# jirsat/wavenets

Hardware: AMD Instinct MI355X
Metric: audio samples/sec (training step, 16 kHz mu-law) (higher is better)
Workload: dtype f32 (fp16 hi|lo split operands, fp32 accumulate)

## Files before the change

wavenets_amd/csrc/wn_bwd_pair.hip:

```cpp
#include "wn_split16.h"

using namespace wn_split16;

namespace {

constexpr int BP_NK1 = 16;
constexpr int BP_NKR = 4;
constexpr int BP_NKF = 8;
constexpr int BP_NKM = BP_NK1 + BP_NKF;
constexpr int BP_W1 = BP_NK1 * 2 * 2048, BP_W2 = (BP_NKR + BP_NKF) * 2 * 2048;
constexpr int BP_PITCH = 36;
constexpr int BP_STAGE = 32 * BP_PITCH * 4;
constexpr int BP_LDS = BP_W1 + BP_W2 + 8 * BP_STAGE;
constexpr int BP_PF = 4;

__device__ __forceinline__ void bp_store32(const f32x16& v, float* stage, float* dst, int64_t ld, int rows_valid, int lane) {
  const int tl = lane & 31, h = lane >> 5;
#pragma unroll
  for (int rq = 0; rq < 4; ++rq) {
    f32x4 o;
    o.x = v[4 * rq + 0]; o.y = v[4 * rq + 1]; o.z = v[4 * rq + 2]; o.w = v[4 * rq + 3];
    *reinterpret_cast<f32x4*>(stage + tl * BP_PITCH + 8 * rq + 4 * h) = o;
  }
  asm volatile("s_waitcnt lgkmcnt(0)" ::: "memory");
#pragma unroll
  for (int i = 0; i < 4; ++i) {
    const int row = i * 8 + (lane >> 3);
    const int col = (lane & 7) * 4;
    const f32x4 o = *reinterpret_cast<const f32x4*>(stage + row * BP_PITCH + col);
    if (row < rows_valid) *reinterpret_cast<f32x4*>(dst + (int64_t)row * ld + col) = o;
  }
  asm volatile("s_waitcnt lgkmcnt(0)" ::: "memory");
}

}

__global__ __launch_bounds__(512, 2) void wn_bwd_pair_kernel(WnBwdPairArgs a) {
  __shared__ __attribute__((aligned(16))) unsigned char smem[BP_LDS];
  const int tid = threadIdx.x;
  const int lane = tid & 63, wave = tid >> 6;
  const int tl = lane & 31, h = lane >> 5;
  float* stage = reinterpret_cast<float*>(smem + BP_W1 + BP_W2 + wave * BP_STAGE);
  {
    wn_images_to_lds<512, BP_W1 / 16, BP_W2 / 16>(a.wx16, smem, BP_W1 / 16, a.wu16, smem + BP_W1, BP_W2 / 16, tid);
  }
  __syncthreads();
  const h8* w1 = reinterpret_cast<const h8*>(smem) + lane;
  const h8* w2 = reinterpret_cast<const h8*>(smem + BP_W1) + lane;

  float sc1, inv1;
  pow2_scale(a.am_gu_in ? *a.am_gu_in : 0.f, sc1, inv1);
  const float gfmax = a.am_gf ? *a.am_gf : 0.f;

  const int tiles_per_b = (a.T + 31) >> 5;
  const int64_t ntiles = (int64_t)a.B * tiles_per_b;
  struct TileCtx {
    int b, t, rows_valid;
    int64_t row0;
  };
  auto make_ctx = [&](int64_t tile, TileCtx& c) {
    c.b = (int)(tile / tiles_per_b);
    const int t0 = (int)(tile % tiles_per_b) * 32;
    c.t = t0 + tl;
    c.rows_valid = min(32, a.T - t0);
    c.row0 = (int64_t)c.b * a.T + t0;
  };
  auto load_x = [&](const TileCtx& c, int m, f32x4& q0, f32x4& q1, bool& okout) {
    const int seg = m >> 3;
    const int kk = m & 7;
    const int ts = c.t + (seg == 0 ? a.dil : 0);
    const bool ok = c.t < a.T && ts < a.T;
    const float* base = seg == 2 ? a.gf : a.gu_in;
    const float* src = base + ((int64_t)c.b * a.T + (ok ? ts : 0)) * 128 + 4 * h + 16 * kk;
    q0 = ldg4(src);
    q1 = ldg4(src + 8);
    okout = ok;
  };

  float wmax_x = 0.f, wmax_u = 0.f;
  const WnTileWalk walk = wn_tile_walk(ntiles, 8, wave);
  const int64_t tstride = walk.stride, tend = walk.end;
  int64_t tile = walk.first;
  TileCtx cur, nxt;
  f32x4 xr[BP_PF][2];
  bool okr[BP_PF];
  if (tile < tend) {
    make_ctx(tile, cur);
#pragma unroll
    for (int k = 0; k < BP_PF; ++k) load_x(cur, k, xr[k][0], xr[k][1], okr[k]);
  }
  for (; tile < tend; tile += tstride) {
    const bool has_next = tile + tstride < tend;
    if (has_next) make_ctx(tile + tstride, nxt);
    const bool tin = cur.t < a.T;
    const int64_t row = cur.row0 + (tin ? tl : 0);

    f32x4 addc[2][4];
#pragma unroll
    for (int j = 0; j < 2; ++j)
#pragma unroll
      for (int rq = 0; rq < 4; ++rq) addc[j][rq] = ldg4(a.gx_res + row * 64 + 32 * j + 8 * rq + 4 * h);

    f32x16 acc[2];
#pragma unroll
    for (int j = 0; j < 2; ++j)
#pragma unroll
      for (int r = 0; r < 16; ++r) acc[j][r] = 0.f;
    for (int m0 = 0; m0 < BP_NK1; m0 += BP_PF) {
      wn_static_for<BP_PF>([&](auto kc) {
        constexpr int k = decltype(kc)::value;
        h8 bh, bl;
        split8s(xr[k][0], xr[k][1], okr[k] ? sc1 : 0.f, bh, bl);
        __builtin_amdgcn_sched_barrier(0);
        load_x(cur, m0 + k + BP_PF, xr[k][0], xr[k][1], okr[k]);
#pragma unroll
        for (int j = 0; j < 2; ++j) {
          const h8 ah = w1[(((m0 + k) * 2 + j) * 2 + 0) * 64];
          const h8 al = w1[(((m0 + k) * 2 + j) * 2 + 1) * 64];
          mfma3(ah, al, bh, bl, acc[j]);
        }
        __builtin_amdgcn_sched_barrier(0);
      });
    }
    f32x16 gx[2];
    float tmax = 0.f;
#pragma unroll
    for (int j = 0; j < 2; ++j)
#pragma unroll
      for (int rq = 0; rq < 4; ++rq) {
        const float cv[4] = {addc[j][rq].x, addc[j][rq].y, addc[j][rq].z, addc[j][rq].w};
#pragma unroll
        for (int e = 0; e < 4; ++e) {
          const float v = tin ? acc[j][4 * rq + e] * inv1 + cv[e] : 0.f;
          gx[j][4 * rq + e] = v;
          tmax = fmaxf(tmax, fabsf(v));
        }
      }
    f32x4 sg[2][4], zz[2][4];
#pragma unroll
    for (int j = 0; j < 2; ++j)
#pragma unroll
      for (int rq = 0; rq < 4; ++rq) {
        sg[j][rq] = ldg4(a.ag + row * 64 + 32 * j + 8 * rq + 4 * h);
        zz[j][rq] = ldg4(a.z + row * a.ldz + 32 * j + 8 * rq + 4 * h);
      }
    if (cur.rows_valid > 0) {
      bp_store32(gx[0], stage, a.gx_out + cur.row0 * 64, 64, cur.rows_valid, lane);
      bp_store32(gx[1], stage, a.gx_out + cur.row0 * 64 + 32, 64, cur.rows_valid, lane);
    }
    wmax_x = fmaxf(wmax_x, tmax);
#pragma unroll
    for (int o = 32; o > 0; o >>= 1) tmax = fmaxf(tmax, __shfl_xor(tmax, o));
    float sc2, inv2;
    pow2_scale(fmaxf(tmax, gfmax), sc2, inv2);

#pragma unroll
    for (int j = 0; j < 2; ++j)
#pragma unroll
      for (int r = 0; r < 16; ++r) acc[j][r] = 0.f;
    wn_static_for<BP_NKR>([&](auto sc) {
      constexpr int ks = decltype(sc)::value;
      constexpr int jz = ks / 2, r0 = 8 * (ks % 2);
      f32x4 q0, q1;
      q0.x = gx[jz][r0 + 0]; q0.y = gx[jz][r0 + 1]; q0.z = gx[jz][r0 + 2]; q0.w = gx[jz][r0 + 3];
      q1.x = gx[jz][r0 + 4]; q1.y = gx[jz][r0 + 5]; q1.z = gx[jz][r0 + 6]; q1.w = gx[jz][r0 + 7];
      h8 bh, bl;
      split8s(q0, q1, sc2, bh, bl);
#pragma unroll
      for (int j = 0; j < 2; ++j) {
        const h8 ah = w2[((ks * 2 + j) * 2 + 0) * 64];
        const h8 al = w2[((ks * 2 + j) * 2 + 1) * 64];
        mfma3(ah, al, bh, bl, acc[j]);
      }
    });
    for (int m0 = BP_NK1; m0 < BP_NKM; m0 += BP_PF) {
      wn_static_for<BP_PF>([&](auto kc) {
        constexpr int k = decltype(kc)::value;
        h8 bh, bl;
        split8s(xr[k][0], xr[k][1], okr[k] ? sc2 : 0.f, bh, bl);
        __builtin_amdgcn_sched_barrier(0);
        const int mn = m0 + k + BP_PF;
        if (mn < BP_NKM) load_x(cur, mn, xr[k][0], xr[k][1], okr[k]);
        else if (has_next) load_x(nxt, mn - BP_NKM, xr[k][0], xr[k][1], okr[k]);
        const int ks2 = BP_NKR + (m0 + k - BP_NK1);
#pragma unroll
        for (int j = 0; j < 2; ++j) {
          const h8 ah = w2[((ks2 * 2 + j) * 2 + 0) * 64];
          const h8 al = w2[((ks2 * 2 + j) * 2 + 1) * 64];
          mfma3(ah, al, bh, bl, acc[j]);
        }
        __builtin_amdgcn_sched_barrier(0);
      });
    }
#pragma unroll
    for (int part = 0; part < 2; ++part)
#pragma unroll
      for (int j = 0; j < 2; ++j) {
        f32x16 o;
#pragma unroll
        for (int rq = 0; rq < 4; ++rq) {
          const float gv[4] = {sg[j][rq].x, sg[j][rq].y, sg[j][rq].z, sg[j][rq].w};
          const float zv[4] = {zz[j][rq].x, zz[j][rq].y, zz[j][rq].z, zz[j][rq].w};
#pragma unroll
          for (int e = 0; e < 4; ++e) {
            const float dz = acc[j][4 * rq + e] * inv2;
            const float v = tin ? (part == 0 ? wn_gate_bwd_f(dz, gv[e], zv[e]) : wn_gate_bwd_g(dz, gv[e], zv[e])) : 0.f;
            o[4 * rq + e] = v;
            wmax_u = fmaxf(wmax_u, fabsf(v));
          }
        }
        if (cur.rows_valid > 0) bp_store32(o, stage, a.gu_out + cur.row0 * 128 + 64 * part + 32 * j, 128, cur.rows_valid, lane);
      }
    if (has_next) cur = nxt;
  }
#pragma unroll
  for (int o = 32; o > 0; o >>= 1) {
    wmax_x = fmaxf(wmax_x, __shfl_xor(wmax_x, o));
    wmax_u = fmaxf(wmax_u, __shfl_xor(wmax_u, o));
  }
  if (lane == 0) {
    if (a.am_gx) wn_absmax_publish(a.am_gx, wmax_x);
    if (a.am_gu) wn_absmax_publish(a.am_gu, wmax_u);
  }
}

int wn_bwd_pair_supported(int R, int D, int KS, int F0) { return (R == 64 && D == 64 && KS == 2 && F0 == 128) ? 1 : 0; }

int wn_launch_bwd_pair(const WnBwdPairArgs& a, hipStream_t s) {
  const int64_t tiles = (int64_t)a.B * ((a.T + 31) / 32);
  if (tiles <= 0) return WN_OK;
  int64_t gx = (tiles + 7) / 8;
  if (gx > 256) gx = 256;
  hipLaunchKernelGGL(wn_bwd_pair_kernel, dim3((unsigned)gx), dim3(512), 0, s, a);
  WN_HIP_CHECK(hipGetLastError());
  return WN_OK;
}
```

wavenets_amd/csrc/wn_common.h:

```cpp
#pragma once
#include <hip/hip_runtime.h>
#include <stdint.h>

#include "../../include/wn_hip.h"

typedef float f32x16 __attribute__((ext_vector_type(16)));
typedef float f32x4 __attribute__((ext_vector_type(4)));

enum WnEpilogue : int {
  WN_EPI_PLAIN = 0,
  WN_EPI_DACT = 1,
  WN_EPI_GATE_BWD = 2,
  WN_EPI_GATE_FWD = 3,
};

__device__ __forceinline__ f32x16 wn_mfma(float a, float b, f32x16 c) {
  return __builtin_amdgcn_mfma_f32_32x32x2f32(a, b, c, 0, 0, 0);
}

__device__ __forceinline__ int wn_drow(int r, int h) { return (r & 3) + 8 * (r >> 2) + 4 * h; }

__device__ __forceinline__ float wn_sigmoid(float x) { return 1.0f / (1.0f + expf(-x)); }

__device__ __forceinline__ float wn_sigmoid_fast(float x) {
  return __builtin_amdgcn_rcpf(1.0f + __builtin_amdgcn_exp2f(-1.4426950408889634f * x));
}
__device__ __forceinline__ float wn_tanh_fast(float x) {
  return __builtin_fmaf(-2.0f, __builtin_amdgcn_rcpf(1.0f + __builtin_amdgcn_exp2f(2.8853900817779268f * x)), 1.0f);
}

__device__ __forceinline__ float wn_act(float x, int act) {
  switch (act) {
    case WN_ACT_RELU: return x > 0.f ? x : 0.f;
    case WN_ACT_LEAKY_RELU: return x >= 0.f ? x : 0.2f * x;
    case WN_ACT_TANH: return tanhf(x);
    case WN_ACT_SIGMOID: return wn_sigmoid(x);
    case WN_ACT_ELU: return x > 0.f ? x : expm1f(x);
    default: return x;
  }
}

__device__ __forceinline__ float wn_dact_from_y(float y, int act) {
  switch (act) {
    case WN_ACT_RELU: return y > 0.f ? 1.f : 0.f;
    case WN_ACT_LEAKY_RELU: return y >= 0.f ? 1.f : 0.2f;
    case WN_ACT_TANH: return 1.f - y * y;
    case WN_ACT_SIGMOID: return y * (1.f - y);
    case WN_ACT_ELU: return y > 0.f ? 1.f : y + 1.f;
    default: return 1.f;
  }
}

__host__ __device__ __forceinline__ size_t wn_frag_floats(int I, int KK) {
  return (size_t)((KK + 7) / 8) * ((I + 31) / 32) * 256;
}

#ifdef __cplusplus
#include <type_traits>
template <int N, class F>
__device__ __forceinline__ void wn_static_for(F&& f) {
  if constexpr (N > 0) {
    wn_static_for<N - 1>(f);
    f(std::integral_constant<int, N - 1>{});
  }
}
#endif

#define WN_HIP_CHECK(expr)                                   \
  do {                                                       \
    hipError_t _e = (expr);                                  \
    if (_e != hipSuccess) {                                  \
      wn_set_error("%s:%d: %s -> %s", __FILE__, __LINE__, #expr, hipGetErrorString(_e)); \
      return WN_E_HIP;                                       \
    }                                                        \
  } while (0)

__device__ __forceinline__ void wn_gate_bwd(float dz, float g, float z, float& duf, float& dug) {
  const float a = g > 1e-30f ? z / g : 0.f;
  duf = dz * g * (1.f - a * a);
  dug = dz * z * (1.f - g);
}

__device__ __forceinline__ float wn_gate_bwd_f(float dz, float g, float z) {
  const float a = g > 1e-30f ? z / g : 0.f;
  return dz * g * (1.f - a * a);
}
__device__ __forceinline__ float wn_gate_bwd_g(float dz, float g, float z) { return dz * z * (1.f - g); }

__device__ __forceinline__ void wn_absmax_publish(float* slot, float v) {
  if (v > 0.f && v < 3.0e38f && v > *reinterpret_cast<volatile float*>(slot))
    atomicMax(reinterpret_cast<int*>(slot), __float_as_int(v));
}

__device__ __forceinline__ void wn_absmax_publish_any(float* slot, float v) {
  if (v > 0.f && v > *reinterpret_cast<volatile float*>(slot))
    atomicMax(reinterpret_cast<int*>(slot), __float_as_int(v));
}

__device__ __forceinline__ float wn_absmax_acc(float wmax, float a, float b, float c, float d) {
  const unsigned m0 = max(__float_as_uint(a) & 0x7fffffffu, __float_as_uint(b) & 0x7fffffffu);
  const unsigned m1 = max(__float_as_uint(c) & 0x7fffffffu, __float_as_uint(d) & 0x7fffffffu);
  return __uint_as_float(max(__float_as_uint(wmax), max(m0, m1)));
}
__device__ __forceinline__ float wn_wave_absmax_bits(float wmax) {
  unsigned m = __float_as_uint(wmax);
#pragma unroll
  for (int o = 32; o > 0; o >>= 1) m = max(m, (unsigned)__shfl_xor((int)m, o));
  const float v = __uint_as_float(m);
  return v < 3.0e38f ? v : 3.0e38f;
}

template <int THREADS, int MAX1, int MAX2 = 0>
__device__ __forceinline__ void wn_images_to_lds(const void* src1, void* dst1, int n16_1, const void* src2, void* dst2, int n16_2,
                                                 int tid) {
  constexpr int K1 = (MAX1 + THREADS - 1) / THREADS, K2 = (MAX2 + THREADS - 1) / THREADS;
  const f32x4* s1 = reinterpret_cast<const f32x4*>(src1);
  const f32x4* s2 = reinterpret_cast<const f32x4*>(src2);
  f32x4 v1[K1 > 0 ? K1 : 1], v2[K2 > 0 ? K2 : 1];
#pragma unroll
  for (int k = 0; k < K1; ++k) { const int i = tid + k * THREADS; if (i < n16_1) v1[k] = s1[i]; }
#pragma unroll
  for (int k = 0; k < K2; ++k) { const int i = tid + k * THREADS; if (i < n16_2) v2[k] = s2[i]; }
  __builtin_amdgcn_sched_barrier(0);
  f32x4* d1 = reinterpret_cast<f32x4*>(dst1);
  f32x4* d2 = reinterpret_cast<f32x4*>(dst2);
#pragma unroll
  for (int k = 0; k < K1; ++k) { const int i = tid + k * THREADS; if (i < n16_1) d1[i] = v1[k]; }
#pragma unroll
  for (int k = 0; k < K2; ++k) { const int i = tid + k * THREADS; if (i < n16_2) d2[i] = v2[k]; }
}

#define WN_KERAS_EPS 1e-7f

#define WN_RANGE_LIMIT 30000.0f

__device__ __forceinline__ void wn_guard_publish_over(float* slot, float wmax) {
  const unsigned m = __float_as_uint(wmax);
  if (m >= __float_as_uint(WN_RANGE_LIMIT)) {
    const float v = __uint_as_float(m);
    atomicMax(reinterpret_cast<int*>(slot), __float_as_int(v < 3.0e38f ? v : 3.0e38f));
  }
}

static inline int wn_blocks(int64_t n, int per = 256, int cap = 4096) {
  int64_t b = (n + per - 1) / per;
  if (b > cap) b = cap;
  if (b < 1) b = 1;
  return (int)b;
}

void wn_set_error(const char* fmt, ...);
int wn_debug_get(int key);

struct WnTileWalk { int64_t first, end, stride; };
__device__ __forceinline__ WnTileWalk wn_tile_walk(int64_t ntiles, int waves, int wave) {
  WnTileWalk w;
  if ((gridDim.x & 7u) == 0u) {
    const int64_t n8 = (ntiles + 7) >> 3;
    const int64_t x = blockIdx.x & 7u;
    w.first = x * n8 + (int64_t)(blockIdx.x >> 3) * waves + wave;
    w.end = (x + 1) * n8 < ntiles ? (x + 1) * n8 : ntiles;
    w.stride = (int64_t)(gridDim.x >> 3) * waves;
  } else {
    w.first = (int64_t)blockIdx.x * waves + wave;
    w.end = ntiles;
    w.stride = (int64_t)gridDim.x * waves;
  }
  return w;
}
```

wavenets_amd/csrc/wn_elem.hip:

```cpp
#include <algorithm>

#include "wn_kernels.h"
#include "wn_sample.h"

__global__ void wn_add_kernel(const float* a, const float* b, float* out, int64_t n) {
  for (int64_t i = (int64_t)blockIdx.x * blockDim.x + threadIdx.x; i < n;
       i += (int64_t)gridDim.x * blockDim.x)
    out[i] = a[i] + b[i];
}
int wn_launch_add(const float* a, const float* b, float* out, int64_t n, hipStream_t s) {
  if (n <= 0) return WN_OK;
  hipLaunchKernelGGL(wn_add_kernel, dim3(wn_blocks(n)), dim3(256), 0, s, a, b, out, n);
  WN_HIP_CHECK(hipGetLastError());
  return WN_OK;
}

__global__ void wn_fill_kernel(float* p, float v, int64_t n) {
  for (int64_t i = (int64_t)blockIdx.x * blockDim.x + threadIdx.x; i < n;
       i += (int64_t)gridDim.x * blockDim.x)
    p[i] = v;
}
int wn_launch_fill(float* p, float v, int64_t n, hipStream_t s) {
  if (n <= 0) return WN_OK;
  hipLaunchKernelGGL(wn_fill_kernel, dim3(wn_blocks(n)), dim3(256), 0, s, p, v, n);
// ... 307 lines not shown
__global__ void wn_dact_mul_kernel(const float* g, const float* y, float* out, int64_t n, int act) {
  for (int64_t i = (int64_t)blockIdx.x * blockDim.x + threadIdx.x; i < n;
       i += (int64_t)gridDim.x * blockDim.x)
    out[i] = g[i] * wn_dact_from_y(y[i], act);
}
int wn_launch_dact_mul(const float* g, const float* y, float* out, int64_t n, int act, hipStream_t s) {
  if (n <= 0) return WN_OK;
  hipLaunchKernelGGL(wn_dact_mul_kernel, dim3(wn_blocks(n)), dim3(256), 0, s, g, y, out, n, act);
  WN_HIP_CHECK(hipGetLastError());
  return WN_OK;
}

__device__ __forceinline__ uint32_t wn_hash32(uint32_t x) {
  x ^= x >> 16; x *= 0x7feb352dU; x ^= x >> 15; x *= 0x846ca68bU; x ^= x >> 16;
  return x;
}
__device__ __forceinline__ bool wn_drop_keep(int64_t idx, uint32_t key, float rate) {
  const uint32_t lo = (uint32_t)idx, hi = (uint32_t)((uint64_t)idx >> 32);
  const uint32_t hsh = wn_hash32(lo ^ wn_hash32(hi + key));
  return (float)(hsh >> 8) * (1.0f / 16777216.0f) >= rate;
}
__global__ void wn_dropout_kernel(const float* x, const float* g_res, float* out, int64_t n, float rate, float scale,
                                  uint32_t key, float* absmax_out) {
  float m = 0.f;
  for (int64_t i = (int64_t)blockIdx.x * blockDim.x + threadIdx.x; i < n; i += (int64_t)gridDim.x * blockDim.x) {
    float v = wn_drop_keep(i, key, rate) ? x[i] * scale : 0.f;
    if (g_res) v += g_res[i];
    out[i] = v;
    m = fmaxf(m, fabsf(v));
  }
  if (absmax_out) {
    m = wn_wave_max(m);
    if ((threadIdx.x & 63) == 0) wn_absmax_publish(absmax_out, m);
  }
}
uint32_t wn_dropout_key(uint64_t seed, int block, uint64_t step) {
  uint32_t k = (uint32_t)seed * 0x9E3779B9U + (uint32_t)(seed >> 32);
  k ^= (uint32_t)block * 0x85EBCA6BU + 0x1234567U;
  k ^= (uint32_t)step * 0xC2B2AE35U + (uint32_t)(step >> 32) * 0x27D4EB2FU;
  return k;
}
int wn_launch_dropout(const float* x, const float* g_res, float* out, int64_t n, float rate, uint32_t key,
                      float* absmax_out, hipStream_t s) {
  if (n <= 0) return WN_OK;
  hipLaunchKernelGGL(wn_dropout_kernel, dim3(wn_blocks(n)), dim3(256), 0, s, x, g_res, out, n, rate, 1.0f / (1.0f - rate),
                     key, absmax_out);
  WN_HIP_CHECK(hipGetLastError());
  return WN_OK;
}

__global__ void wn_cond_scatter_kernel(const float* tmp, const float* params, int64_t b_off0, int64_t b_stride, int B,
                                       int N, int D2, float* cb) {
  const int64_t total = (int64_t)N * B * D2;
  for (int64_t i = (int64_t)blockIdx.x * blockDim.x + threadIdx.x; i < total; i += (int64_t)gridDim.x * blockDim.x) {
    const int n = (int)(i % D2);
    const int u = (int)((i / D2) % B);
    const int b = (int)(i / ((int64_t)D2 * B));
    cb[i] = tmp[((int64_t)u * N + b) * D2 + n] + params[b_off0 + (int64_t)b * b_stride + n];
  }
}
__global__ void wn_cond_gather_kernel(const float* slab, int64_t P, int spb, int64_t bd_off0, int64_t bd_stride, int B,
                                      int N, int D2, float* dcb) {
  const int64_t total = (int64_t)B * N * D2;
  for (int64_t i = (int64_t)blockIdx.x * blockDim.x + threadIdx.x; i < total; i += (int64_t)gridDim.x * blockDim.x) {
    const int n = (int)(i % D2);
    const int b = (int)((i / D2) % N);
    const int u = (int)(i / ((int64_t)D2 * N));
    float acc = 0.f;
    for (int sp = 0; sp < spb; ++sp) acc += slab[(int64_t)(u * spb + sp) * P + bd_off0 + (int64_t)b * bd_stride + n];
    dcb[i] = acc;
  }
}
__global__ void wn_cond_wgrad_kernel(const float* m, const float* dcb, int B, int Cc, int N, int D2, float* grads,
                                     int64_t w_off0, int64_t w_stride, int64_t b_off0, int64_t b_stride) {
  const int64_t total = (int64_t)N * (Cc + 1) * D2;
  for (int64_t i = (int64_t)blockIdx.x * blockDim.x + threadIdx.x; i < total; i += (int64_t)gridDim.x * blockDim.x) {
    const int n = (int)(i % D2);
    const int c = (int)((i / D2) % (Cc + 1));
    const int b = (int)(i / ((int64_t)D2 * (Cc + 1)));
    float acc = 0.f;
    for (int u = 0; u < B; ++u) {
      const float g = dcb[((int64_t)u * N + b) * D2 + n];
      acc += c < Cc ? m[(int64_t)u * Cc + c] * g : g;
    }
    if (c < Cc) grads[w_off0 + (int64_t)b * w_stride + (int64_t)c * D2 + n] = acc;
    else grads[b_off0 + (int64_t)b * b_stride + n] = acc;
  }
}
int wn_launch_cond_scatter(const float* tmp, const float* params, int64_t b_off0, int64_t b_stride, int B, int N, int D2,
                           float* cb, hipStream_t s) {
  const int64_t total = (int64_t)N * B * D2;
  hipLaunchKernelGGL(wn_cond_scatter_kernel, dim3((unsigned)std::min<int64_t>((total + 255) / 256, 1024)), dim3(256), 0, s, tmp,
                     params, b_off0, b_stride, B, N, D2, cb);
  WN_HIP_CHECK(hipGetLastError());
  return WN_OK;
}
int wn_launch_cond_gather(const float* slab, int64_t P, int spb, int64_t bd_off0, int64_t bd_stride, int B, int N, int D2,
                          float* dcb, hipStream_t s) {
  const int64_t total = (int64_t)B * N * D2;
  hipLaunchKernelGGL(wn_cond_gather_kernel, dim3((unsigned)std::min<int64_t>((total + 255) / 256, 1024)), dim3(256), 0, s, slab, P,
                     spb, bd_off0, bd_stride, B, N, D2, dcb);
  WN_HIP_CHECK(hipGetLastError());
  return WN_OK;
}
int wn_launch_cond_wgrad(const float* m, const float* dcb, int B, int Cc, int N, int D2, float* grads, int64_t w_off0,
                         int64_t w_stride, int64_t b_off0, int64_t b_stride, hipStream_t s) {
  const int64_t total = (int64_t)N * (Cc + 1) * D2;
  hipLaunchKernelGGL(wn_cond_wgrad_kernel, dim3((unsigned)std::min<int64_t>((total + 255) / 256, 1024)), dim3(256), 0, s, m, dcb, B,
                     Cc, N, D2, grads, w_off0, w_stride, b_off0, b_stride);
  WN_HIP_CHECK(hipGetLastError());
  return WN_OK;
}

__global__ __launch_bounds__(256) void wn_inconv_fwd_kernel(const float* x, const float* w, const float* bias, int B, int T,
                                                            int R, int KS, float* y, float* absmax_out) {
  const int q = R / 4;
  const int64_t total = (int64_t)B * T * q;
  float wmax = 0.f;
  for (int64_t i = (int64_t)blockIdx.x * blockDim.x + threadIdx.x; i < total; i += (int64_t)gridDim.x * blockDim.x) {
    const int c = (int)(i % q) * 4;
    const int64_t row = i / q;
    const int t = (int)(row % T);
    float a0 = 0.f, a1 = 0.f, a2 = 0.f, a3 = 0.f;
    for (int tap = 0; tap < KS; ++tap) {
      const int ts = t - (KS - 1 - tap);
      const float xv = ts >= 0 ? x[row - (KS - 1 - tap)] : 0.f;
      const f32x4 wv = *reinterpret_cast<const f32x4*>(w + (int64_t)tap * R + c);
      a0 = fmaf(wv.x, xv, a0); a1 = fmaf(wv.y, xv, a1); a2 = fmaf(wv.z, xv, a2); a3 = fmaf(wv.w, xv, a3);
    }
    const f32x4 bv = *reinterpret_cast<const f32x4*>(bias + c);
    const f32x4 o = f32x4{a0 + bv.x, a1 + bv.y, a2 + bv.z, a3 + bv.w};
    *reinterpret_cast<f32x4*>(y + row * R + c) = o;
    wmax = fmaxf(wmax, fmaxf(fmaxf(fabsf(o.x), fabsf(o.y)), fmaxf(fabsf(o.z), fabsf(o.w))));
  }
  if (absmax_out) {
    __shared__ float wm[4];
    if (!(wmax < 3.0e38f)) wmax = 3.0e38f;
    wmax = wn_wave_max(wmax);
    if ((threadIdx.x & 63) == 0) wm[threadIdx.x >> 6] = wmax;
    __syncthreads();
    if (threadIdx.x == 0) wn_absmax_publish_any(absmax_out, fmaxf(fmaxf(wm[0], wm[1]), fmaxf(wm[2], wm[3])));
  }
}
int wn_launch_inconv_fwd(const float* x, const float* w, const float* bias, int B, int T, int R, int KS, float* y,
                         float* absmax_out, hipStream_t s) {
  const int64_t total = (int64_t)B * T * (R / 4);
  if (total <= 0) return WN_OK;
  hipLaunchKernelGGL(wn_inconv_fwd_kernel, dim3((unsigned)std::min<int64_t>((total + 255) / 256, 1024)), dim3(256), 0, s, x, w, bias,
                     B, T, R, KS, y, absmax_out);
  WN_HIP_CHECK(hipGetLastError());
  return WN_OK;
}

__global__ __launch_bounds__(256) void wn_sgemm_small32_kernel(const float* A, int64_t sai, int64_t sak, const float* B, int64_t sbk,
                                                               int64_t sbj, float* C, int ldc, int M, int N, int K,
                                                               int64_t za, int64_t zb, int64_t zc, const float* bias, int act,
                                                               int zk) {
  constexpr int KC = 128;
  __shared__ float As[KC][32 + 1], Bs[KC][32 + 1];
  A += (int64_t)blockIdx.z * za; B += (int64_t)blockIdx.z * zb; C += (int64_t)blockIdx.z * zc;
  if (zk > 0) K = max(0, min(K - (int)blockIdx.z * zk, zk));
  const int i0 = blockIdx.y * 32, j0 = blockIdx.x * 32;
  const int tx = threadIdx.x & 31, ty = threadIdx.x >> 5;
  float acc[4] = {0.f, 0.f, 0.f, 0.f};
  for (int k0 = 0; k0 < K; k0 += KC) {
    float ra[16], rb[16];
#pragma unroll
    for (int q = 0; q < 16; ++q) {
      const int e = threadIdx.x + 256 * q;
      const int ka = sak == 1 ? e % KC : e / 32, ia = sak == 1 ? e / KC : e % 32;
      ra[q] = (i0 + ia < M && k0 + ka < K) ? A[(int64_t)(i0 + ia) * sai + (int64_t)(k0 + ka) * sak] : 0.f;
      const int kb = sbk == 1 ? e % KC : e / 32, jb = sbk == 1 ? e / KC : e % 32;
      rb[q] = (j0 + jb < N && k0 + kb < K) ? B[(int64_t)(k0 + kb) * sbk + (int64_t)(j0 + jb) * sbj] : 0.f;
    }
    if (k0 > 0) __syncthreads();
#pragma unroll
    for (int q = 0; q < 16; ++q) {
      const int e = threadIdx.x + 256 * q;
      const int ka = sak == 1 ? e % KC : e / 32, ia = sak == 1 ? e / KC : e % 32;
      As[ka][ia] = ra[q];
      const int kb = sbk == 1 ? e % KC : e / 32, jb = sbk == 1 ? e / KC : e % 32;
      Bs[kb][jb] = rb[q];
    }
    __syncthreads();
#pragma unroll 8
    for (int k = 0; k < KC; ++k) {
      const float bv = Bs[k][tx];
#pragma unroll
      for (int a = 0; a < 4; ++a) acc[a] = fmaf(As[k][ty + 8 * a], bv, acc[a]);
    }
  }
#pragma unroll
  for (int a = 0; a < 4; ++a) {
    const int i = i0 + ty + 8 * a, j = j0 + tx;
    if (i < M && j < N) {
      float v = acc[a];
      if (bias) v = wn_act(v + bias[j], act);
      C[(int64_t)i * ldc + j] = v;
    }
  }
}
int wn_launch_sgemm_small(const float* A, int64_t sai, int64_t sak, const float* B, int64_t sbk, int64_t sbj, float* C, int ldc,
                          int M, int N, int K, hipStream_t s) {
  if (M <= 0 || N <= 0) return WN_OK;
  hipLaunchKernelGGL(wn_sgemm_small32_kernel, dim3((N + 31) / 32, (M + 31) / 32), dim3(256), 0, s, A, sai, sak, B, sbk, sbj, C,
                     ldc, M, N, K, (int64_t)0, (int64_t)0, (int64_t)0, (const float*)nullptr, 0, 0);
  WN_HIP_CHECK(hipGetLastError());
  return WN_OK;
}

int wn_launch_sgemm_small_batched(const float* A, int64_t sai, int64_t sak, int64_t za, const float* B, int64_t sbk, int64_t sbj,
                                  int64_t zb, float* C, int ldc, int64_t zc, int M, int N, int K, int nz, const float* bias,
                                  int act, hipStream_t s, int zk) {
  if (M <= 0 || N <= 0 || nz <= 0) return WN_OK;
  if (nz > 65535) { wn_set_error("sgemm_small_batched: too many products"); return WN_E_UNSUPPORTED; }
  hipLaunchKernelGGL(wn_sgemm_small32_kernel, dim3((N + 31) / 32, (M + 31) / 32, nz), dim3(256), 0, s, A, sai, sak, B, sbk, sbj, C,
                     ldc, M, N, K, za, zb, zc, bias, act, zk);
  WN_HIP_CHECK(hipGetLastError());
  return WN_OK;
}

__global__ void wn_skip_gather_kernel(const float* params, int64_t ws_off0, int64_t ws_stride, const float* bsum, int N, int D,
                                      int S, float* wsall) {
  for (int64_t i = (int64_t)blockIdx.x * blockDim.x + threadIdx.x; i < (int64_t)(N * D + 1) * S; i += (int64_t)gridDim.x * blockDim.x) {
    const int k = (int)(i / S), sidx = (int)(i % S);
    wsall[i] = k < N * D ? params[ws_off0 + (int64_t)(k / D) * ws_stride + (int64_t)(k % D) * S + sidx] : bsum[sidx];
  }
}
__global__ void wn_vec_add_kernel(const float* a, const float* b, int n, float* out) {
  const int i = blockIdx.x * blockDim.x + threadIdx.x;
  if (i < n) out[i] = a[i] + b[i];
}
int wn_launch_skip_fold(const float* params, int64_t ws_off0, int64_t ws_stride, int64_t wf0_off, int64_t bf0_off,
                        const float* bsum, int N, int D, int S, int F0, float* V, float* bfold, float* wsall, hipStream_t s) {
  const int64_t total = (int64_t)(N * D + 1) * S;
  hipLaunchKernelGGL(wn_skip_gather_kernel, dim3((unsigned)std::min<int64_t>((total + 255) / 256, 2048)), dim3(256), 0, s, params,
                     ws_off0, ws_stride, bsum, N, D, S, wsall);
  WN_HIP_CHECK(hipGetLastError());
  int rc = wn_launch_sgemm_small(wsall, S, 1, params + wf0_off, F0, 1, V, F0, N * D + 1, F0, S, s);
  if (rc) return rc;
  hipLaunchKernelGGL(wn_vec_add_kernel, dim3((F0 + 255) / 256), dim3(256), 0, s, V + (int64_t)N * D * F0, params + bf0_off, F0, bfold);
  WN_HIP_CHECK(hipGetLastError());
  return WN_OK;
}

__global__ void wn_skip_scatter_kernel(const float* Y, const float* colsum, int64_t ws_off0, int64_t ws_stride, int64_t bs_off0,
                                       int64_t bs_stride, int64_t bf0_off, int N, int D, int S, int F0, float* grads) {
  const int64_t n_ws = (int64_t)N * D * S, n_bs = (int64_t)N * S;
  const int64_t total = n_ws + n_bs + F0;
  for (int64_t i = (int64_t)blockIdx.x * blockDim.x + threadIdx.x; i < total; i += (int64_t)gridDim.x * blockDim.x) {
    if (i < n_ws) {
      const int k = (int)(i / S), sidx = (int)(i % S);
      grads[ws_off0 + (int64_t)(k / D) * ws_stride + (int64_t)(k % D) * S + sidx] = Y[i];
    } else if (i < n_ws + n_bs) {
      const int64_t j = i - n_ws;
      grads[bs_off0 + (j / S) * bs_stride + (j % S)] = Y[n_ws + (j % S)];
    } else {
      grads[bf0_off + (i - n_ws - n_bs)] = colsum[i - n_ws - n_bs];
    }
  }
}
int wn_launch_skip_scatter(const float* Y, const float* colsum, int64_t ws_off0, int64_t ws_stride, int64_t bs_off0,
                           int64_t bs_stride, int64_t bf0_off, int N, int D, int S, int F0, float* grads, hipStream_t s) {
  const int64_t total = (int64_t)N * D * S + (int64_t)N * S + F0;
  hipLaunchKernelGGL(wn_skip_scatter_kernel, dim3((unsigned)std::min<int64_t>((total + 255) / 256, 4096)), dim3(256), 0, s, Y, colsum,
                     ws_off0, ws_stride, bs_off0, bs_stride, bf0_off, N, D, S, F0, grads);
  WN_HIP_CHECK(hipGetLastError());
  return WN_OK;
}

__global__ void wn_guard_flag_kernel(const float* absmax, float limit, int enabled, float* out) {
  const float m = absmax ? *absmax : 0.f;
  out[0] = (enabled && !(m < limit)) ? 1.0f : 0.0f;
}
__global__ void wn_guard_accumulate_kernel(const float* src, float* dst) {
  const unsigned a = __float_as_uint(src[0]) & 0x7fffffffu, b = __float_as_uint(dst[0]) & 0x7fffffffu;
  dst[0] = __uint_as_float(a > b ? a : b);
}
int wn_launch_guard_accumulate(const float* src, float* dst, hipStream_t s) {
  hipLaunchKernelGGL(wn_guard_accumulate_kernel, dim3(1), dim3(1), 0, s, src, dst);
  WN_HIP_CHECK(hipGetLastError());
  return WN_OK;
}
int wn_launch_guard_flag(const float* absmax, float limit, int enabled, float* out, hipStream_t s) {
  hipLaunchKernelGGL(wn_guard_flag_kernel, dim3(1), dim3(1), 0, s, absmax, limit, enabled, out);
  WN_HIP_CHECK(hipGetLastError());
  return WN_OK;
}

template <int KS>
__global__ __launch_bounds__(256) void wn_inconv_wgrad_kernel(const float* x, const float* g, int T, int R, int spb,
                                                              float* slab, int64_t P, int64_t w_off, int64_t b_off) {
  __shared__ float red[256 * (KS + 1) * 4];
  const int split = blockIdx.x, ub = split / spb, sp = split % spb;
  int len = (T + spb - 1) / spb;
  const int r0 = sp * len, r1 = min(T, r0 + len);
  const int ng = R / 4, nrl = 256 / ng;
  const int cg = threadIdx.x % ng, rl = threadIdx.x / ng;
  float acc[KS + 1][4];
#pragma unroll
  for (int i = 0; i <= KS; ++i)
#pragma unroll
    for (int e = 0; e < 4; ++e) acc[i][e] = 0.f;
  const float* xb = x + (int64_t)ub * T;
  const float* gb = g + (int64_t)ub * T * R + 4 * cg;
  for (int t = r0 + rl; t < r1; t += nrl) {
    const f32x4 gv = *reinterpret_cast<const f32x4*>(gb + (int64_t)t * R);
    const float ge[4] = {gv.x, gv.y, gv.z, gv.w};
#pragma unroll
    for (int tap = 0; tap < KS; ++tap) {
      const int ts = t - (KS - 1 - tap);
      const float xv = ts >= 0 ? xb[ts] : 0.f;
#pragma unroll
      for (int e = 0; e < 4; ++e) acc[tap][e] = fmaf(xv, ge[e], acc[tap][e]);
    }
#pragma unroll
    for (int e = 0; e < 4; ++e) acc[KS][e] += ge[e];
  }
#pragma unroll
  for (int i = 0; i <= KS; ++i)
#pragma unroll
    for (int e = 0; e < 4; ++e) red[(i * 4 + e) * 256 + rl * ng + cg] = acc[i][e];
  __syncthreads();
  float* row = slab + (int64_t)split * P;
  for (int o = threadIdx.x; o < (KS + 1) * R; o += 256) {
    const int i = o / R, c = o % R;
    float sum = 0.f;
    for (int l = 0; l < nrl; ++l) sum += red[(i * 4 + (c & 3)) * 256 + l * ng + (c >> 2)];
    if (i < KS) row[w_off + (int64_t)i * R + c] = sum;
    else row[b_off + c] = sum;
  }
}

int wn_inconv_wgrad_supported(int R, int KS) { return (R % 4 == 0 && R >= 4 && R <= 1024 && 256 % (R / 4) == 0 && (KS == 2 || KS == 3)) ? 1 : 0; }

int wn_launch_inconv_wgrad(const float* x, const float* g, int B, int T, int R, int KS, int splits_per_b, float* slab,
                           int64_t P, int64_t w_off, int64_t b_off, hipStream_t s) {
  if (!wn_inconv_wgrad_supported(R, KS)) { wn_set_error("inconv_wgrad: unsupported shape R=%d KS=%d", R, KS); return WN_E_UNSUPPORTED; }
  const dim3 grid((unsigned)(B * splits_per_b));
  if (KS == 2) hipLaunchKernelGGL(wn_inconv_wgrad_kernel<2>, grid, dim3(256), 0, s, x, g, T, R, splits_per_b, slab, P, w_off, b_off);
  else hipLaunchKernelGGL(wn_inconv_wgrad_kernel<3>, grid, dim3(256), 0, s, x, g, T, R, splits_per_b, slab, P, w_off, b_off);
  WN_HIP_CHECK(hipGetLastError());
  return WN_OK;
}
```

wavenets_amd/csrc/wn_forward.hip:

```cpp
#include "wn_plan_internal.h"

namespace {

__global__ void wn_ring_capture_kernel(const float* src, int B, int T, int C, int nslots, float* ring) {
  const int64_t n = (int64_t)nslots * B * C;
  for (int64_t i = (int64_t)blockIdx.x * blockDim.x + threadIdx.x; i < n; i += (int64_t)gridDim.x * blockDim.x) {
    const int c = (int)(i % C);
    const int b = (int)((i / C) % B);
    const int k = (int)(i / ((int64_t)C * B));
    const int t = T - nslots + k;
    if (t >= 0) ring[((int64_t)(t % nslots) * B + b) * C + c] = src[((int64_t)b * T + t) * C + c];
  }
}

__global__ void wn_shift_split_kernel(const float* x_full, int B, int T, float* inputs, float* y_true) {
  const int64_t n = (int64_t)B * T;
  for (int64_t i = (int64_t)blockIdx.x * blockDim.x + threadIdx.x; i < n; i += (int64_t)gridDim.x * blockDim.x) {
    const int64_t b = i / T, t = i % T;
    inputs[i] = x_full[b * (T + 1) + t];
    y_true[i] = x_full[b * (T + 1) + t + 1];
  }
}

}

namespace wnp {

BlockPtrs block_ptrs(const wn_plan* p, int b, const float* params, const float* fragbase, int B, int T) {
  BlockPtrs k;
  memset(&k, 0, sizeof(k));
  const BlockInfo& bi = p->blocks[b];
  k.B = B; k.T = T; k.KS = p->KS; k.R = p->R; k.D = p->D; k.S = p->S; k.Cin = p->R; k.depth = p->LPB;
  k.act = p->c.activation; k.residual = p->c.use_residual;
  for (int i = 0; i < p->LPB; ++i) {
    const ConvInfo& c = bi.dil[i];
    k.dil[i] = c.dil;
    k.Wd[i] = params + p->tensors[c.kernel_t].off;
    k.bd[i] = params + p->tensors[c.bias_t].off;
    k.Fd[i] = fragbase + c.fragF; k.Fd_stride[i] = c.fragF_stride;
    k.Bd[i] = fragbase + c.fragB; k.Bd_stride[i] = c.fragB_stride;
  }
  k.br = params + p->tensors[bi.conv1.bias_t].off;
  k.Fr = fragbase + bi.conv1.fragF; k.Br_ = fragbase + bi.conv1.fragB;
  if (bi.has_skip) { k.bs = params + p->tensors[bi.conv_skip.bias_t].off; k.Bs = fragbase + bi.conv_skip.fragB; }
  k.Cc = 0; k.cond = nullptr; k.cb = nullptr;
  k.fused = p->fused_ok;
  if (p->fused16_ok && p->LPB == 1) { k.F16d = fragbase + bi.dil.back().frag16; k.F16r = fragbase + bi.conv1.frag16; }
  if (bi.f16gate >= 0) { k.F16g = fragbase + bi.f16gate; k.F16r = fragbase + bi.conv1.frag16; }
  if (bi.f16nat >= 0) k.F16n = fragbase + bi.f16nat;
  if (bi.g16u >= 0 && p->LPB == 1) k.G16u = fragbase + bi.g16u;
  if (bi.g16uf >= 0) k.G16uf = fragbase + bi.g16uf;
  if (p->LPB == 1 && bi.dil[0].frag16B >= 0) k.G16x = fragbase + bi.dil[0].frag16B;
  return k;
}

void deep16_ptrs(const wn_plan* p, int b, const float* fragbase, BlockPtrs& k) {
  if (!deep16(p)) return;
  const BlockInfo& bi = p->blocks[b];
  k.F16d = fragbase + bi.dil.back().frag16; k.F16r = fragbase + bi.conv1.frag16;
  for (int i = 0; i < p->LPB; ++i) {
    const ConvInfo& c = bi.dil[i];
    if (bi.d16F[i] >= 0) { k.F16i[i] = fragbase + bi.d16F[i]; k.JTi[i] = std::max(2, ceil32(c.cout)); }
    if (bi.d16B[i] >= 0) { k.G16i[i] = fragbase + bi.d16B[i]; k.JTb[i] = std::max(2, ceil32(c.cin)); }
  }
  if (bi.g16u >= 0) { k.G16u = fragbase + bi.g16u; k.JTu = std::max(2, ceil32(p->D)); }
}

int ring_capture(const float* src, int B, int T, int C, int nslots, float* ring, hipStream_t s) {
  const int64_t n = (int64_t)nslots * B * C;
  hipLaunchKernelGGL(wn_ring_capture_kernel, dim3((unsigned)std::min<int64_t>((n + 255) / 256, 4096)), dim3(256), 0, s,
                     src, B, T, C, nslots, ring);
  WN_HIP_CHECK(hipGetLastError());
  return WN_OK;
}

int forward_core(wn_plan* p, const float* params, const float* x, bool prep, const float* cond, int B,
                 int T, bool training, float* ws, const WsLayout& L, hipStream_t s, const GenRings* rings, LossFuse* lf) {
  int rc = ensure_device_tables(p);
  if (rc) return rc;
  const int64_t rows = (int64_t)B * T;
  float* fragbase = ws + L.frag;
  if (prep) {
    rc = wn_launch_prep_table(p->d_prep, (int)p->prep.size(), params, fragbase, s);
    if (rc) return rc;
  }
  wn_exec& exs = wnp::ex(p);
  const bool fold = fold_ok(p);
  const bool fork_prep = prep && fold && p->c.use_skip && wn_debug_get(9) == 0;
  bool prep_forked = false;
  auto fold_prep = [&](hipStream_t sp) -> int {
    const bool fp_prof = prep && fold && exs.foldprep_used + 2 <= (int)exs.foldprep_ev.size();
    if (fp_prof) (void)hipEventRecord(exs.foldprep_ev[exs.foldprep_used], sp);
    if (prep && p->c.use_skip) {
      const ConvInfo& c0 = p->blocks[0].has_skip ? p->blocks[0].conv_skip : p->blocks[0].conv1;
      WnVecSumArgs v;
      v.base = params; v.off0 = p->tensors[c0.bias_t].off;
      v.stride = p->N > 1 ? (p->tensors[(p->blocks[1].has_skip ? p->blocks[1].conv_skip : p->blocks[1].conv1).bias_t].off - v.off0) : 0;
      v.count = p->N; v.len = p->Sh; v.out = ws + L.bias_sum;
      const int r = wn_launch_vecsum(v, sp);
      if (r) return r;
    }
    if (fold && prep) {
      const BlockInfo& b0 = p->blocks[0];
      const int64_t wst = p->N > 1 ? p->tensors[p->blocks[1].conv_skip.kernel_t].off - p->tensors[b0.conv_skip.kernel_t].off : 0;
      int r = wn_launch_skip_fold(params, p->tensors[b0.conv_skip.kernel_t].off, wst, p->tensors[p->finals[0].kernel_t].off,
                                  p->tensors[p->finals[0].bias_t].off, ws + L.bias_sum, p->N, p->D, p->S, p->fold_F0, ws + L.vfold,
                                  ws + L.bfold, ws + L.wsall, sp);
      if (r) return r;
      r = wn_launch_prep_table(p->d_prep2, (int)p->prep2.size(), ws, fragbase, sp, 64);
      if (r) return r;
    }
    if (fp_prof) { (void)hipEventRecord(exs.foldprep_ev[exs.foldprep_used + 1], sp); exs.foldprep_used += 2; }
    return WN_OK;
  };
  if (!fork_prep) {
    rc = fold_prep(s);
    if (rc) return rc;
  }
  const float* m = cond;
  if (p->c.cond_inputs > 0) {
    if (!cond) { wn_set_error("Conditioning must be provided."); return WN_E_INVALID; }
    int mc = p->c.cond_inputs;
    for (size_t j = 0; j < p->mapping.size(); ++j) {
      const ConvInfo& c = p->mapping[j];
      if (cond_small(p))
        rc = wn_launch_sgemm_small_batched(m, mc, 1, 0, params + p->tensors[c.kernel_t].off, c.cout, 1, 0, ws + L.M[j], c.cout, 0,
                                           B, c.cout, mc, 1, params + p->tensors[c.bias_t].off, p->c.mapping_activation, s);
      else
      rc = Gemm(1, B, c.cout, ceil32(c.cout)).seg(m, mc, mc, 0, fragbase + c.fragF)
               .bias(params + p->tensors[c.bias_t].off).act(p->c.mapping_activation).run(ws + L.M[j], c.cout, s);
      if (rc) return rc;
      m = ws + L.M[j]; mc = c.cout;
    }
    if (p->frag_condF >= 0) {
      const int D2 = 2 * p->D;
      const ConvInfo& c0 = p->blocks[0].conv_cond;
      const int64_t bst = p->N > 1 ? p->tensors[p->blocks[1].conv_cond.bias_t].off - p->tensors[c0.bias_t].off : 0;
      if (cond_small(p)) {
        const int64_t wst = p->N > 1 ? p->tensors[p->blocks[1].conv_cond.kernel_t].off - p->tensors[c0.kernel_t].off : 0;
        rc = wn_launch_sgemm_small_batched(m, p->Cc, 1, 0, params + p->tensors[c0.kernel_t].off, D2, 1, wst, ws + L.cbt, p->N * D2, D2,
                                           B, D2, p->Cc, p->N, nullptr, 0, s);
      } else
      rc = Gemm(1, B, p->N * D2, ceil32(p->N * D2)).seg(m, p->Cc, p->Cc, 0, fragbase + p->frag_condF).run(ws + L.cbt, p->N * D2, s);
      if (rc) return rc;
      rc = wn_launch_cond_scatter(ws + L.cbt, params, p->tensors[c0.bias_t].off, bst, B, p->N, D2, ws + L.cb, s);
      if (rc) return rc;
    } else {
    for (int b = 0; b < p->N; ++b) {
      const ConvInfo& c = p->blocks[b].conv_cond;
      rc = Gemm(1, B, 2 * p->D, ceil32(2 * p->D)).seg(m, p->Cc, p->Cc, 0, fragbase + c.fragF)
               .bias(params + p->tensors[c.bias_t].off).run(ws + L.cb + (int64_t)b * B * 2 * p->D, 2 * p->D, s);
      if (rc) return rc;
    }
    }
  }
  float* const fam = ws + L.fwd_absmax;
  WN_HIP_CHECK(hipMemsetAsync(fam, 0, sizeof(float), s));
  {
    if (p->R % 4 == 0 && wn_debug_get(1) != 1) {
      rc = wn_launch_inconv_fwd(x, params + p->tensors[p->causal.kernel_t].off, params + p->tensors[p->causal.bias_t].off, B, T,
                                p->R, p->KS, ws + L.H[0], fam, s);
    } else {
      Gemm g(B, T, p->R, ceil32(p->R));
      for (int t = 0; t < p->KS; ++t)
        g.seg(x, 1, 1, (p->KS - 1 - t), fragbase + p->causal.fragF + t * p->causal.fragF_stride);
      rc = g.bias(params + p->tensors[p->causal.bias_t].off).run(ws + L.H[0], p->R, s);
    }
    if (rc) return rc;
    if (rings) {
      rc = ring_capture(x, B, T, 1, p->KS, rings->xin, s);
      if (!rc) rc = ring_capture(ws + L.H[0], B, T, p->R, rings->nslots[0], rings->h[0], s);
      if (rc) return rc;
    }
  }
  if (p->Dp != p->D) {
    rc = wn_launch_fill(ws + L.Z, 0.f, rows * p->N * p->Dp, s);
    if (rc) return rc;
  }
  const bool prof_chain = wnp::ex(p).prof_on && !rings && p->LPB == 1 && p->c.cond_inputs == 0 && p->R == p->D &&
                          !(training && wnp::ex(p).drop_rate > 0.f) && block_ptrs(p, 0, params, fragbase, B, T).fused;
  const bool stack_prof = !rings && wnp::ex(p).stack_used + 2 <= (int)wnp::ex(p).stack_ev.size();
  if (stack_prof) (void)hipEventRecord(wnp::ex(p).stack_ev[wnp::ex(p).stack_used], s);
  if (fork_prep) {
    if (!exs.side) {
      WN_HIP_CHECK(hipStreamCreateWithFlags(&exs.side, hipStreamNonBlocking));
      WN_HIP_CHECK(hipEventCreateWithFlags(&exs.ev_fork, hipEventDisableTiming));
      WN_HIP_CHECK(hipEventCreateWithFlags(&exs.ev_join, hipEventDisableTiming));
    }
    if (!exs.ev_ffork) {
      WN_HIP_CHECK(hipEventCreateWithFlags(&exs.ev_ffork, hipEventDisableTiming));
      WN_HIP_CHECK(hipEventCreateWithFlags(&exs.ev_fjoin, hipEventDisableTiming));
    }
    WN_HIP_CHECK(hipEventRecord(exs.ev_ffork, s));
    WN_HIP_CHECK(hipStreamWaitEvent(exs.side, exs.ev_ffork, 0));
    rc = fold_prep(exs.side);
    if (rc) return rc;
    WN_HIP_CHECK(hipEventRecord(exs.ev_fjoin, exs.side));
    prep_forked = true;
  }
  for (int b = 0; b < p->N; ++b) {
    BlockPtrs k = block_ptrs(p, b, params, fragbase, B, T);
    if (training && !rings) deep16_ptrs(p, b, fragbase, k);
    if (p->c.cond_inputs > 0) k.cb = ws + L.cb + (int64_t)b * B * 2 * p->D;
    BlockBufs f;
    memset(&f, 0, sizeof(f));
    const int hi = training ? b : (b & 1), ho = training ? b + 1 : ((b + 1) & 1);
    f.x = ws + L.H[hi];
    if (training && wnp::ex(p).drop_rate > 0.f) {
      rc = wn_launch_dropout(ws + L.H[hi], nullptr, ws + L.XD[b], rows * p->R, wnp::ex(p).drop_rate,
                             wn_dropout_key(wnp::ex(p).drop_seed, b, wnp::ex(p).drop_step), nullptr, s);
      if (rc) return rc;
      f.x = ws + L.XD[b];
      f.res = ws + L.H[hi];
    }
    for (int i = 0; i + 1 < p->LPB; ++i) f.P[i] = ws + L.P[b][i];
    f.U = ws + L.U;
    f.AG = training ? ws + L.AG[b] : nullptr;
    f.Z = ws + L.Z + (int64_t)b * rows * p->Dp; f.ldz = p->Dp;
    f.O = nullptr;
    f.x_out = ws + L.H[ho];
    f.fwd_absmax = fam;
    const bool prof = wnp::ex(p).prof_on && wnp::ex(p).prof_used + 2 <= (int)wnp::ex(p).prof_ev.size();
    const bool ev0 = prof && (!prof_chain || b == 0), ev1 = prof && (!prof_chain || b == p->N - 1);
    if (ev0) (void)hipEventRecord(wnp::ex(p).prof_ev[wnp::ex(p).prof_used], s);
    rc = block_forward(k, f, s);
    if (rc) return rc;
    if (ev1) {
      (void)hipEventRecord(wnp::ex(p).prof_ev[wnp::ex(p).prof_used + 1], s);
      wnp::ex(p).prof_cnt[wnp::ex(p).prof_used / 2] = prof_chain ? p->N : 1;
      wnp::ex(p).prof_used += 2;
    }
    if (rings && b + 1 < p->N) {
      rc = ring_capture(f.x_out, B, T, p->R, rings->nslots[b + 1], rings->h[b + 1], s);
      if (rc) return rc;
    }
    if (rings)
      for (int i = 0; i + 1 < p->LPB; ++i) {
        rc = ring_capture(f.P[i], B, T, p->D, rings->nslots_p[b][i], rings->hp[b][i], s);
        if (rc) return rc;
      }
  }
  if (prep_forked) WN_HIP_CHECK(hipStreamWaitEvent(s, exs.ev_fjoin, 0));
  const float* hin;
  size_t first_final = 0;
  if (fold) {
    const ConvInfo& c0 = p->finals[0];
    if (p->Dp == p->D && wn_gemm_planes16s_supported(c0.cout, p->D, p->N, p->Dp, c0.cout) &&
        (int64_t)rows * p->Dp * 4 < ((int64_t)1 << 32) && (int64_t)rows * c0.cout * 4 < ((int64_t)1 << 32)) {
      WnGemmPlanesArgs ga;
      memset(&ga, 0, sizeof(ga));
      ga.z = ws + L.Z; ga.plane_stride = rows * p->Dp; ga.ld = p->Dp; ga.plane_k = p->D; ga.nplanes = p->N;
      ga.w16 = fragbase + p->frag16_foldF; ga.bias = ws + L.bfold; ga.act = p->c.activation;
      ga.y = ws + L.HA[0]; ga.ldy = c0.cout; ga.N = c0.cout; ga.B = B; ga.T = T; ga.absmax_out = fam;
      rc = wn_launch_gemm_planes16s(ga, s);
    } else
    rc = Gemm(B, T, c0.cout, ceil32(c0.cout)).seg_planes(ws + L.Z, p->Dp, rows * p->Dp, p->N * p->Dp, nullptr)
             .w16(fragbase + p->frag16_foldF).bias(ws + L.bfold).act(p->c.activation).absmax_fwd(fam)
             .run(ws + L.HA[0], c0.cout, s);
    if (rc) return rc;
    hin = ws + L.HA[0];
    first_final = 1;
  } else if (p->c.use_skip) {
    rc = Gemm(B, T, p->Sh, ceil32(p->Sh)).seg_planes(ws + L.Z, p->Dp, rows * p->Dp, p->N * p->Dp, fragbase + p->frag_skipF)
             .w16(p->frag16_skipF >= 0 ? fragbase + p->frag16_skipF : nullptr)
             .bias(ws + L.bias_sum).absmax_fwd(fam).run(ws + L.skipsum, p->Sh, s);
    if (rc) return rc;
    hin = ws + L.skipsum;
  } else {
    hin = ws + L.H[training ? p->N : (p->N & 1)];
  }
  if (stack_prof) { (void)hipEventRecord(wnp::ex(p).stack_ev[wnp::ex(p).stack_used + 1], s); wnp::ex(p).stack_used += 2; }
  int hc = fold ? p->finals[0].cout : p->Hin;
  for (size_t i = first_final; i < p->finals.size(); ++i) {
    const ConvInfo& c = p->finals[i];
    const bool last = (i + 1 == p->finals.size());
    float* dst = last ? ws + L.logits : ws + L.HA[i];
    if (last && lf && loss_fusable(p, rows) && wn_gemm_planes16s_supported(c.cout, hc, 1, hc, c.cout) &&
        (int64_t)rows * hc * 4 < ((int64_t)1 << 32)) {
      WnGemmPlanesArgs ga;
      memset(&ga, 0, sizeof(ga));
      ga.z = hin; ga.plane_stride = 0; ga.ld = hc; ga.plane_k = hc; ga.nplanes = 1;
      ga.w16 = fragbase + c.frag16; ga.bias = params + p->tensors[c.bias_t].off; ga.act = WN_ACT_LINEAR;
      ga.y = lf->g_logits; ga.ldy = c.cout; ga.N = c.cout; ga.B = B; ga.T = T; ga.absmax_out = lf->absmax_out;
      ga.cat_loss = 1; ga.target = lf->target; ga.gscale = lf->gscale; ga.loss_rows = lf->loss_rows;
      ga.sample_out = lf->sample_out; ga.inv_lv = lf->inv_lv; ga.seed = lf->seed; ga.offset = lf->offset;
      rc = wn_launch_gemm_planes16s(ga, s);
      if (rc) return rc;
      lf->done = true;
      break;
    }
    if (c.frag16 >= 0 && wn_debug_get(1) != 1 && wn_gemm_planes16s_supported(c.cout, hc, 1, hc, c.cout) &&
        (int64_t)rows * hc * 4 < ((int64_t)1 << 32)) {
      WnGemmPlanesArgs ga;
      memset(&ga, 0, sizeof(ga));
      ga.z = hin; ga.plane_stride = 0; ga.ld = hc; ga.plane_k = hc; ga.nplanes = 1;
      ga.w16 = fragbase + c.frag16; ga.bias = params + p->tensors[c.bias_t].off; ga.act = last ? WN_ACT_LINEAR : p->c.activation;
      ga.y = dst; ga.ldy = c.cout; ga.N = c.cout; ga.B = B; ga.T = T; ga.absmax_out = last ? nullptr : fam;
      rc = wn_launch_gemm_planes16s(ga, s);
      if (rc) return rc;
      hin = dst; hc = c.cout;
      continue;
    }
    rc = Gemm(B, T, c.cout, ceil32(c.cout)).seg(hin, hc, hc, 0, fragbase + c.fragF)
             .w16(c.frag16 >= 0 ? fragbase + c.frag16 : nullptr)
             .bias(params + p->tensors[c.bias_t].off).act(last ? WN_ACT_LINEAR : p->c.activation)
             .absmax_fwd(last ? nullptr : fam).run(dst, c.cout, s);
    if (rc) return rc;
    hin = dst; hc = c.cout;
  }
  return WN_OK;
}

int shift_split(const float* x_full, int B, int T, float* inputs, float* y_true, hipStream_t s) {
  const int64_t rows = (int64_t)B * T;
  hipLaunchKernelGGL(wn_shift_split_kernel, dim3((unsigned)std::min<int64_t>((rows + 255) / 256, 4096)), dim3(256), 0, s,
                     x_full, B, T, inputs, y_true);
  WN_HIP_CHECK(hipGetLastError());
  return WN_OK;
}

bool loss_fusable(const wn_plan* p, int64_t rows) {
  if (p->c.head != WN_HEAD_CATEGORICAL || p->Cout != 256 || wn_debug_get(1) == 1 || p->finals.empty()) return false;
  const ConvInfo& c = p->finals.back();
  return c.frag16 >= 0 && c.cout == 256 && rows > 0;
}

int loss_stage(wn_plan* p, int B, int T, int global_batch, bool want_grad, float* ws, const WsLayout& L,
               float* loss_out, float* absmax_out, hipStream_t s, bool fused_done) {
  const int64_t rows = (int64_t)B * T;
  const float gscale = 1.0f / (float)global_batch;
  int rc;
  if (fused_done) return wn_launch_sum(ws + L.loss_rows, rows, gscale, loss_out, ws + L.sum_scratch, s);
  float* g_logits = want_grad ? ws + L.GF.back() : nullptr;
  if (p->c.head == WN_HEAD_CATEGORICAL) {
    rc = wn_launch_quantize(ws + L.yt, reinterpret_cast<int32_t*>(ws + L.target), rows, p->c.bits, s);
    if (rc) return rc;
    float* so = nullptr;
    if (want_grad && wnp::ex(p).step_sample && !wnp::ex(p).step_sample_det && p->Cout <= 256) { so = wnp::ex(p).step_sample; wnp::ex(p).step_sample = nullptr; }
    rc = wn_launch_cat_loss(ws + L.logits, reinterpret_cast<const int32_t*>(ws + L.target), rows, p->Cout,
                            gscale, ws + L.loss_rows, g_logits, absmax_out, s, so, p->c.bits, wnp::ex(p).step_sample_seed,
                            wnp::ex(p).step_sample_off);
  } else {
    rc = wn_launch_mix_loss(ws + L.logits, ws + L.yt, rows, p->c.num_mixtures, p->c.bits,
                            p->c.head == WN_HEAD_LOGISTIC ? 1 : 2, gscale, ws + L.loss_rows, g_logits, absmax_out, s);
  }
  if (rc) return rc;
  return wn_launch_sum(ws + L.loss_rows, rows, gscale, loss_out, ws + L.sum_scratch, s);
}

}

using namespace wnp;

extern "C" int wn_forward(wn_plan* p, const float* params, const float* x, const float* cond, int32_t B,
                          int32_t T, float* out, float* logits_out, float* workspace, int64_t ws_floats,
                          void* stream) {
  if (!p || !params || !x || !workspace || B < 1 || T < 1) { wn_set_error("forward: bad arguments"); return WN_E_INVALID; }
  hipStream_t s = (hipStream_t)stream;
  const WsLayout L = make_layout(p, B, T, false);
  if (ws_floats < L.total) { wn_set_error("forward: workspace too small (%lld < %lld floats)", (long long)ws_floats, (long long)L.total); return WN_E_INVALID; }
  int rc = forward_core(p, params, x, true, cond, B, T, false, workspace, L, s);
  if (rc) return rc;
  const int64_t rows = (int64_t)B * T;
  if (logits_out) WN_HIP_CHECK(hipMemcpyAsync(logits_out, workspace + L.logits, rows * p->Cout * sizeof(float), hipMemcpyDeviceToDevice, s));
  if (out) {
    if (p->c.head == WN_HEAD_CATEGORICAL) return wn_launch_softmax(workspace + L.logits, out, rows, p->Cout, s);
    WN_HIP_CHECK(hipMemcpyAsync(out, workspace + L.logits, rows * p->Cout * sizeof(float), hipMemcpyDeviceToDevice, s));
  }
  return WN_OK;
}

extern "C" int wn_forward_training(wn_plan* p, const float* params, const float* x, const float* cond, int32_t B,
                                   int32_t T, float* out, float* logits_out, float* workspace, int64_t ws_floats,
                                   void* stream) {
  if (!p || !params || !x || !workspace || B < 1 || T < 1) { wn_set_error("forward_training: bad arguments"); return WN_E_INVALID; }
  hipStream_t s = (hipStream_t)stream;
  const WsLayout L = make_layout(p, B, T, true);
  if (ws_floats < L.total) { wn_set_error("forward_training: workspace too small (%lld < %lld floats)", (long long)ws_floats, (long long)L.total); return WN_E_INVALID; }
  int rc = forward_core(p, params, x, true, cond, B, T, true, workspace, L, s);
  if (rc) return rc;
  const int64_t rows = (int64_t)B * T;
  if (logits_out) WN_HIP_CHECK(hipMemcpyAsync(logits_out, workspace + L.logits, rows * p->Cout * sizeof(float), hipMemcpyDeviceToDevice, s));
  if (out) {
    if (p->c.head == WN_HEAD_CATEGORICAL) return wn_launch_softmax(workspace + L.logits, out, rows, p->Cout, s);
    WN_HIP_CHECK(hipMemcpyAsync(out, workspace + L.logits, rows * p->Cout * sizeof(float), hipMemcpyDeviceToDevice, s));
  }
  return WN_OK;
}

extern "C" int wn_eval_loss(wn_plan* p, const float* params, const float* x_full, const float* cond,
                            int32_t B, int32_t T, int32_t global_batch, float* loss_out, float* pred_out,
                            float* workspace, int64_t ws_floats, void* stream) {
  if (!p || !params || !x_full || !workspace || !loss_out || B < 1 || T < 1) { wn_set_error("eval_loss: bad arguments"); return WN_E_INVALID; }
  hipStream_t s = (hipStream_t)stream;
  const WsLayout L = make_layout(p, B, T, false);
  if (ws_floats < L.total) { wn_set_error("eval_loss: workspace too small"); return WN_E_INVALID; }
  const int64_t rows = (int64_t)B * T;
  float* inputs = workspace + L.probs;
  { const int rcs = shift_split(x_full, B, T, inputs, workspace + L.yt, s); if (rcs) return rcs; }
  int rc = forward_core(p, params, inputs, true, cond, B, T, false, workspace, L, s);
  if (rc) return rc;
  rc = loss_stage(p, B, T, global_batch > 0 ? global_batch : B, false, workspace, L, loss_out, nullptr, s);
  if (rc) return rc;
  rc = wn_launch_guard_flag(workspace + L.fwd_absmax, WN_RANGE_LIMIT, wn_debug_get(1) != 1, loss_out + 2, s);
  if (rc) return rc;
  if (pred_out) {
    if (p->c.head == WN_HEAD_CATEGORICAL) return wn_launch_softmax(workspace + L.logits, pred_out, rows, p->Cout, s);
    WN_HIP_CHECK(hipMemcpyAsync(pred_out, workspace + L.logits, rows * p->Cout * sizeof(float), hipMemcpyDeviceToDevice, s));
  }
  return WN_OK;
}
```

wavenets_amd/csrc/wn_gemm.hip:

```cpp
#include "wn_split16.h"

using namespace wn_split16;

__device__ __forceinline__ void wn_prep16_body(const WnPrepDesc& d, const float* params, float* ws,
                                               int64_t start, int64_t stride) {
  const int JI = (d.I + 31) / 32;
  const int nks = (d.KK + 15) / 16;
  const int64_t total = (int64_t)nks * JI * 64 * 8;
  const float* src = params + d.src_off;
  __half* dst = reinterpret_cast<__half*>(ws + d.dst_off);
  for (int64_t idx = start; idx < total; idx += stride) {
    const int jj = idx & 7;
    const int lane = (idx >> 3) & 63;
    const int64_t blk = idx >> 9;
    const int j = blk % JI;
    const int ks = blk / JI;
    const int i = 32 * j + (lane & 31);
    const int kk = 16 * ks + 8 * (jj >> 2) + 4 * (lane >> 5) + (jj & 3);
    float v = 0.f;
    if (i < d.I && kk < d.KK) v = d.transpose ? src[(int64_t)kk * d.ld + i] : src[(int64_t)i * d.ld + kk];
    const __half hi = __float2half_rn(v);
    const __half lo = __float2half_rn(v - __half2float(hi));
    const int64_t base = (((int64_t)(ks + d.q_off) * d.JT + (j + d.j_off)) * 2) * 512 + lane * 8 + jj;
    dst[base] = hi;
// ... 409 lines not shown
        for (int i = 0; i < WG_TM; ++i) av[i][e] = px[(int64_t)e * a.ldx + 32 * i];
#pragma unroll
        for (int j = 0; j < WG_TN; ++j) bv[j][e] = pg[(int64_t)e * a.ldg + 32 * j];
      }
      return;
    }
#pragma unroll
    for (int e = 0; e < 8; ++e) {
      const int t = tb + e;
      const int ts = t - a.shift;
      const bool tv = t < r1;
      const bool xv = tv && ts >= 0 && ts < a.T;
#pragma unroll
      for (int i = 0; i < WG_TM; ++i) av[i][e] = (xv && kin[i]) ? px[(int64_t)e * a.ldx + 32 * i] : 0.f;
#pragma unroll
      for (int j = 0; j < WG_TN; ++j) bv[j][e] = (tv && nin[j]) ? pg[(int64_t)e * a.ldg + 32 * j] : 0.f;
    }
  };
  auto compute_chunk = [&](const float (&av)[WG_TM][8], const float (&bv)[WG_TN][8]) {
    h8 ah[WG_TM], al[WG_TM];
#pragma unroll
    for (int i = 0; i < WG_TM; ++i) split8(av[i], ah[i], al[i]);
#pragma unroll
    for (int j = 0; j < WG_TN; ++j) {
      h8 bh, bl;
      float sv[8];
#pragma unroll
      for (int e = 0; e < 8; ++e) {
        bsum[j] += bv[j][e];
        sv[e] = bv[j][e] * gsc;
      }
      split8(sv, bh, bl);
#pragma unroll
      for (int i = 0; i < WG_TM; ++i) {
        mfma3(ah[i], al[i], bh, bl, acc[i][j]);
      }
    }
  };
  {
    float av0[WG_TM][8], bv0[WG_TN][8], av1[WG_TM][8], bv1[WG_TN][8];
    int tt = r0;
    if (tt < r1) load_chunk(tt, av0, bv0);
    for (; tt < r1; tt += 32) {
      if (tt + 16 < r1) load_chunk(tt + 16, av1, bv1);
      compute_chunk(av0, bv0);
      if (tt + 16 < r1) {
        if (tt + 32 < r1) load_chunk(tt + 32, av0, bv0);
        compute_chunk(av1, bv1);
      }
    }
  }

#pragma unroll
  for (int i = 0; i < WG_TM; ++i)
#pragma unroll
    for (int j = 0; j < WG_TN; ++j) {
      const int n = n0 + 32 * j + tl;
#pragma unroll
      for (int r = 0; r < 16; ++r) {
        const int k = k0 + 32 * i + wn_drow(r, h);
        if (k < a.K && n < a.N) a.out[(int64_t)k * a.out_ld + n] = acc[i][j][r] * inv_gsc;
      }
    }
  if (a.bias) {
#pragma unroll
    for (int j = 0; j < WG_TN; ++j) {
      const float tot = bsum[j] + __shfl_xor(bsum[j], 32);
      const int n = n0 + 32 * j + tl;
      if (h == 0 && n < a.N) a.bias[n] = tot;
    }
  }
}

__global__ __launch_bounds__(256, 2) void wn_wgrad_kernel(WnWgradArgs a, int nkb, int nnb) {
  const int wave = threadIdx.x >> 6;
  const int nsplit = a.B * a.splits_per_b;
  const int split = blockIdx.x * 4 + wave;
  if (split >= nsplit) return;
  const int kb = blockIdx.y / nnb, nb = blockIdx.y % nnb;
  const int sp = split % a.splits_per_b;
  int len = (a.T + a.splits_per_b - 1) / a.splits_per_b;
  len = (len + 1) & ~1;
  WnWgUnit u;
  u.x = a.x; u.ldx = a.ldx; u.K = a.K; u.shift = a.shift; u.g = a.g; u.ldg = a.ldg; u.N = a.N;
  u.T = a.T; u.b = split / a.splits_per_b; u.r0 = sp * len; u.r1 = min(a.T, u.r0 + len);
  u.k0 = kb * 32 * WG_TM; u.n0 = nb * 32 * WG_TN;
  u.out = a.slab + (int64_t)split * a.K * a.N; u.out_ld = a.N;
  u.bias = (a.slab_bias && kb == 0) ? a.slab_bias + (int64_t)split * a.N : nullptr;
  wn_wgrad_body(u);
}

template <bool F16>
__global__ __launch_bounds__(256, 2) void wn_wgrad_batched_kernel(const WnWgJob* jobs, float* ws, float* slab,
                                                                  int64_t P, int B, int T, int splits_per_b) {
  const int wave = threadIdx.x >> 6;
  const int nsplit = B * splits_per_b;
  const int split = blockIdx.x * 4 + wave;
  if (split >= nsplit) return;
  const WnWgJob j = jobs[blockIdx.y];
  const int sp = split % splits_per_b;
  int len = (T + splits_per_b - 1) / splits_per_b;
  len = (len + 1) & ~1;
  WnWgUnit u;
  u.x = ws + j.x_off; u.ldx = j.ldx; u.K = j.K; u.shift = j.shift; u.g = ws + j.g_off; u.ldg = j.ldg; u.N = j.N;
  u.T = T; u.b = split / splits_per_b; u.r0 = sp * len; u.r1 = min(T, u.r0 + len);
  u.k0 = j.k0; u.n0 = j.n0;
  float* row = slab + (int64_t)split * P;
  u.out = row + j.out_off; u.out_ld = j.N;
  u.bias = j.bias_off >= 0 ? row + j.bias_off : nullptr;
  if constexpr (F16) {
    float gsc = 1.0f, inv = 1.0f;
    if (j.gmax_off >= 0) pow2_scale(ws[j.gmax_off], gsc, inv);
    wn_wgrad_body16(u, gsc, inv);
  } else {
    wn_wgrad_body(u);
  }
}

int wn_launch_wgrad_batched(const WnWgJob* d_jobs, int njobs, float* ws, float* slab, int64_t P, int B, int T,
                            int splits_per_b, hipStream_t s, bool exact_fp32) {
  if (njobs <= 0) return WN_OK;
  const int nsplit = B * splits_per_b;
  if (exact_fp32 || wn_debug_get(1) == 1 || wn_debug_get(3) == 1)
    hipLaunchKernelGGL(wn_wgrad_batched_kernel<false>, dim3((nsplit + 3) / 4, njobs), dim3(256), 0, s, d_jobs, ws, slab, P,
                       B, T, splits_per_b);
  else
    hipLaunchKernelGGL(wn_wgrad_batched_kernel<true>, dim3((nsplit + 3) / 4, njobs), dim3(256), 0, s, d_jobs, ws, slab, P,
                       B, T, splits_per_b);
  WN_HIP_CHECK(hipGetLastError());
  return WN_OK;
}

__global__ void wn_reduce_table_kernel(const float* slab, int nsplit, int64_t P, float* out,
                                       const WnTensorDesc* table) {
  const WnTensorDesc d = table[blockIdx.y];
  for (int64_t i = (int64_t)blockIdx.x * blockDim.x + threadIdx.x; i < d.len;
       i += (int64_t)gridDim.x * blockDim.x) {
    float acc = 0.f;
    const float* col = slab + d.off + i;
    int s = 0;
    for (; s + 8 <= nsplit; s += 8) {
      float v[8];
#pragma unroll
      for (int e = 0; e < 8; ++e) v[e] = col[(int64_t)(s + e) * P];
#pragma unroll
      for (int e = 0; e < 8; ++e) acc += v[e];
    }
    for (; s < nsplit; ++s) acc += col[(int64_t)s * P];
    out[d.off + i] = acc;
  }
}

struct WnBlkFirst { int v[257]; };
__global__ __launch_bounds__(256) void wn_reduce_flat_kernel(const float* slab, int nsplit, int64_t P, float* out,
                                                             const WnTensorDesc* table, WnBlkFirst bf, int n) {
  int lo = 0, hi = n;
  while (hi - lo > 1) {
    const int mid = (lo + hi) >> 1;
    if (bf.v[mid] <= (int)blockIdx.x) lo = mid; else hi = mid;
  }
  const WnTensorDesc d = table[lo];
  const int64_t i = (int64_t)((int)blockIdx.x - bf.v[lo]) * 256 + threadIdx.x;
  if (i >= d.len) return;
  float acc = 0.f;
  const float* col = slab + d.off + i;
  int s = 0;
  for (; s + 16 <= nsplit; s += 16) {
    float v[16];
#pragma unroll
    for (int e = 0; e < 16; ++e) v[e] = col[(int64_t)(s + e) * P];
#pragma unroll
    for (int e = 0; e < 16; ++e) acc += v[e];
  }
  for (; s < nsplit; ++s) acc += col[(int64_t)s * P];
  out[d.off + i] = acc;
}

int wn_launch_reduce_table(const float* slab, int nsplit, int64_t P, float* out, const WnTensorDesc* d_table,
                           int n, hipStream_t s, const WnTensorDesc* h_table) {
  if (n <= 0) return WN_OK;
  if (h_table && n <= 256) {
    WnBlkFirst bf;
    int64_t nblk = 0;
    for (int t = 0; t < n; ++t) { bf.v[t] = (int)nblk; nblk += (h_table[t].len + 255) / 256; }
    for (int t = n; t <= 256; ++t) bf.v[t] = (int)nblk;
    if (nblk <= 0) return WN_OK;
    if (nblk < (int64_t)1 << 30) {
      hipLaunchKernelGGL(wn_reduce_flat_kernel, dim3((unsigned)nblk), dim3(256), 0, s, slab, nsplit, P, out, d_table, bf, n);
      WN_HIP_CHECK(hipGetLastError());
      return WN_OK;
    }
  }
  hipLaunchKernelGGL(wn_reduce_table_kernel, dim3(64, n), dim3(256), 0, s, slab, nsplit, P, out, d_table);
  WN_HIP_CHECK(hipGetLastError());
  return WN_OK;
}

int wn_wgrad_tile_k() { return 32 * WG_TM; }
int wn_wgrad_tile_n() { return 32 * WG_TN; }

int wn_wgrad_choose_splits(int B, int T, int K, int N) {
  const int jobs = ((K + 32 * WG_TM - 1) / (32 * WG_TM)) * ((N + 32 * WG_TN - 1) / (32 * WG_TN));
  int want = (1024 + jobs - 1) / jobs;
  int per_b = (want + B - 1) / B;
  const int max_per_b = (T + 255) / 256;
  if (per_b > max_per_b) per_b = max_per_b;
  if (per_b < 1) per_b = 1;
  return per_b;
}

int wn_launch_wgrad(const WnWgradArgs& a, hipStream_t s) {
  if (a.K <= 0 || a.N <= 0 || a.B <= 0 || a.T <= 0) return WN_OK;
  const int nkb = (a.K + 32 * WG_TM - 1) / (32 * WG_TM);
  const int nnb = (a.N + 32 * WG_TN - 1) / (32 * WG_TN);
  const int nsplit = a.B * a.splits_per_b;
  dim3 grid((nsplit + 3) / 4, nkb * nnb);
  hipLaunchKernelGGL(wn_wgrad_kernel, grid, dim3(256), 0, s, a, nkb, nnb);
  WN_HIP_CHECK(hipGetLastError());
  return WN_OK;
}

#define WN_RED_GROUP 16
__global__ void wn_reduce_stageA_kernel(float* slab, int nsplit, int64_t total) {
  const int g = blockIdx.y;
  const int s0 = g * WN_RED_GROUP;
  const int s1 = min(nsplit, s0 + WN_RED_GROUP);
  for (int64_t i = (int64_t)blockIdx.x * blockDim.x + threadIdx.x; i < total;
       i += (int64_t)gridDim.x * blockDim.x) {
    float acc = 0.f;
    for (int s = s0; s < s1; ++s) acc += slab[(int64_t)s * total + i];
    slab[(int64_t)s0 * total + i] = acc;
  }
}

__global__ void wn_reduce_kernel(WnReduceArgs a, int stride) {
  const int64_t total = (int64_t)a.K * a.N;
  for (int64_t i = (int64_t)blockIdx.x * blockDim.x + threadIdx.x; i < total;
       i += (int64_t)gridDim.x * blockDim.x) {
    float acc = 0.f;
    for (int s = 0; s < a.nsplit; s += stride) acc += a.slab[(int64_t)s * total + i];
    const int k = (int)(i / a.N), n = (int)(i % a.N);
    float* dst = a.out + (int64_t)(k / a.seg_len) * a.seg_stride + (int64_t)(k % a.seg_len) * a.N + n;
    for (int r = 0; r < a.replicate; ++r) {
      float* d = dst + (int64_t)r * a.rep_stride;
      *d = a.accumulate ? (*d + acc) : acc;
    }
  }
}

int wn_launch_reduce(const WnReduceArgs& a, hipStream_t s) {
  const int64_t total = (int64_t)a.K * a.N;
  if (total <= 0) return WN_OK;
  int blocks = (int)((total + 255) / 256);
  if (blocks > 2048) blocks = 2048;
  int stride = 1;
  if (a.nsplit > 2 * WN_RED_GROUP) {
    const int groups = (a.nsplit + WN_RED_GROUP - 1) / WN_RED_GROUP;
    hipLaunchKernelGGL(wn_reduce_stageA_kernel, dim3(blocks, groups), dim3(256), 0, s,
                       const_cast<float*>(a.slab), a.nsplit, total);
    stride = WN_RED_GROUP;
  }
  hipLaunchKernelGGL(wn_reduce_kernel, dim3(blocks), dim3(256), 0, s, a, stride);
  WN_HIP_CHECK(hipGetLastError());
  return WN_OK;
}
```

wavenets_amd/csrc/wn_kernels.h:

```cpp
#pragma once
#include "wn_common.h"

struct WnTensorDesc { int64_t off; int64_t len; };

struct WnPrepDesc {
  int64_t src_off;
  int64_t dst_off;
  int32_t I;
  int32_t KK;
  int32_t ld;
  int32_t transpose;
  int32_t q_off;
  int32_t j_off;
  int32_t JT;
  int32_t kind;
};
int wn_launch_prep_table(const WnPrepDesc* d_table, int n, const float* params, float* ws,
                         hipStream_t s, int gx = 16);
int wn_launch_prep_one(WnPrepDesc d, const float* params, float* ws, hipStream_t s);
struct WnVecSumArgs { const float* base; int64_t off0; int64_t stride; int32_t count; int32_t len; float* out; };
int wn_launch_vecsum(WnVecSumArgs a, hipStream_t s);

#define WN_MAXSEG 4
struct WnSeg {
  const float* x;
  const float* frag;
  int32_t ldx;
  int32_t K;
  int32_t shift;
  int32_t vec;
  int32_t plane_k;
  int64_t plane_stride;
};
struct WnGemmArgs {
  WnSeg seg[WN_MAXSEG];
  int32_t nseg;
  int32_t B, T;
  int32_t N;
  int32_t JTtot;
  const float* bias;
  const float* rowbias;
  int32_t ld_rowbias;
  const float* addc;
  int32_t ld_addc;
  int32_t act;
  int32_t epi;
  const float* aux;
  int32_t ld_aux;
  const float* aux2;
  int32_t ld_aux2;
  float* y;
  int32_t ldy;
  int32_t vec_out;
  float* y2;
  int32_t ld_y2;
  int32_t absmax_any;
};
int wn_launch_gemm_rows(const WnGemmArgs& a, hipStream_t s);
int wn_gemm_rows16_ok(const WnGemmArgs& a);
int wn_launch_gemm_rows16(const WnGemmArgs& a, const float* w16, const float* absmax_in0,
                          const float* absmax_in1, float* absmax_out, hipStream_t s);

struct WnGemmPlanesArgs {
  const float* z;
  int64_t plane_stride;
  int32_t ld, plane_k, nplanes;
  const float* w16;
  const float* bias;
  int32_t act;
  float* y; int32_t ldy;
  int32_t N;
  int32_t B, T;
  float* absmax_out;
  int32_t bwd;
  const float* absmax_in;
  const float* aux; int32_t ld_aux;
  int32_t nshift; int32_t shift[4];
  int32_t cat_loss;
  const int32_t* target;
  float gscale;
  float* loss_rows;
  float* sample_out;
  float inv_lv;
  uint64_t seed, offset;
};
int wn_gemm_planes16s_supported(int N, int plane_k, int nplanes, int ld, int ldy);
int wn_gemm_taps16s_supported(int N, int plane_k, int ntaps, int ld, int ldy);
int wn_launch_gemm_planes16s(const WnGemmPlanesArgs& a, hipStream_t s);

struct WnWgradArgs {
  const float* x; int32_t ldx; int32_t K; int32_t shift;
  const float* g; int32_t ldg; int32_t N;
  int32_t B, T;
  int32_t splits_per_b;
  float* slab;
  float* slab_bias;
};
int wn_wgrad_choose_splits(int B, int T, int K, int N);
int wn_launch_wgrad(const WnWgradArgs& a, hipStream_t s);
struct WnWgJob {
  int64_t x_off, g_off, out_off, bias_off;
  int64_t gmax_off;
  int32_t ldx, ldg, K, N, shift, k0, n0, pad_;
};
struct WnWgLayer {
  int64_t x_off, du_off, z_off, go_off;
  int64_t dwd_off, dbd_off, dwr_off, dbr_off;
  int64_t gmax_u_off, gmax_h_off;
  int32_t dilation, ldz;
};
int wn_wgrad_layer_supported(int R, int D, int KS);
int wn_launch_wgrad_layers(const WnWgLayer* d_layers, int nlayers, int R, float* ws, float* slab, int64_t P, int B,
                           int T, int splits_per_b, hipStream_t s, int inner = 0);
struct WnWgPair {
  int64_t x_off, g_off;
  int64_t w_off, b_off;
  int64_t gmax_off;
  int32_t shift;
  union { int32_t pad_; int32_t nseg; };
  union { int64_t g2_off; int64_t seg_stride; };
  int64_t w2_off, b2_off, gmax2_off;
};
int wn_wgrad_pair_kind(int K, int N);
int wn_launch_wgrad_pairs(int kind, const WnWgPair* d_jobs, int njobs, float* ws, float* slab, int64_t P, int B, int T,
                          int splits_per_b, hipStream_t s);
int wn_wgrad_tr_kind(int K, int N, int taps);
int wn_launch_wgrad_tr(int kind, const WnWgPair* d_jobs, int njobs, float* ws, float* slab, int64_t P, int B, int T,
                       int splits_per_b, hipStream_t s, float* slab2 = nullptr, int64_t P2 = 0);
struct WnBwdPairArgs {
  const float* gu_in;
  const float* gx_res;
  const float* gf;
  const float* ag;
  const float* z; int32_t ldz;
  float* gx_out;
  float* gu_out;
  const float* wx16;
  const float* wu16;
  const float* am_gu_in; const float* am_gf;
  float* am_gx; float* am_gu;
  int32_t B, T, dil;
};
int wn_bwd_pair_supported(int R, int D, int KS, int F0);
int wn_launch_bwd_pair(const WnBwdPairArgs& a, hipStream_t s);
int wn_bwd_s128_supported(int R, int D, int KS, int F0);
int wn_launch_bwd_s128(const WnBwdPairArgs& a, hipStream_t s);
int wn_wgrad_skip_supported(int D, int S, int KZ);
int wn_launch_wgrad_skip(const float* z, int ldz, const float* g, int ldg, int64_t rows, int KZ, int S, int D,
                         int nsplit, float* slab, int64_t P, int64_t w_off0, int64_t w_stride, int64_t b_off0,
                         int64_t b_stride, int nblocks, const float* gmax, hipStream_t s);
int wn_wgrad_tile_k();
int wn_wgrad_tile_n();
int wn_launch_wgrad_batched(const WnWgJob* d_jobs, int njobs, float* ws, float* slab, int64_t P, int B, int T,
                            int splits_per_b, hipStream_t s, bool exact_fp32 = false);
int wn_launch_reduce_table(const float* slab, int nsplit, int64_t P, float* out, const WnTensorDesc* d_table,
                           int n, hipStream_t s, const WnTensorDesc* h_table = nullptr);
struct WnReduceArgs {
  const float* slab; int32_t nsplit; int32_t K; int32_t N;
  float* out; int32_t seg_len; int64_t seg_stride; int32_t accumulate;
  int32_t replicate; int64_t rep_stride;
};
int wn_launch_reduce(const WnReduceArgs& a, hipStream_t s);

struct WnLayerFwdArgs {
  const float* x;
  const float* frag_d;
  const float* frag_r;
  const float* bias_d;
  const float* bias_r;
  const float* cb;
  float* x_out;
  float* o_out;
  float* z_out; int32_t ldz;
  float* ag_out;
  const float* res;
  const float* xt[3];
  int32_t B, T, R, D, KS, dilation, residual;
  float* absmax_out;
};
int wn_layer_fwd_supported(int R, int D, int KS);
int wn_layer_fwd_f16_supported(int R, int D, int KS);
int wn_launch_layer_fwd_f16(const WnLayerFwdArgs& a, hipStream_t s);
size_t wn_frag16_floats(int I, int KK);
int wn_layer_fwd_s128_supported(int R, int D, int KS);
int wn_launch_layer_fwd_s128(const WnLayerFwdArgs& a, hipStream_t s);
int wn_launch_layer_fwd(const WnLayerFwdArgs& a, hipStream_t s);
int wn_gen_block128_supported(int R, int D, int KS);
int wn_launch_gen_block128(const WnLayerFwdArgs& a, hipStream_t s);

struct WnGenBlock {
  int64_t ring_off;
  int64_t w16d_off;
  int64_t w16r_off;
  int64_t bias_d_off;
  int64_t bias_r_off;
  int64_t cb_off;
  int32_t nslots, dilation;
};
struct WnGenStepArgs {
  const float* params;
  float* ws;
  const WnGenBlock* blocks;
  const float* xin;
  const float* causal_w;
  const float* causal_b;
  int64_t zrow_off;
  int64_t hrow_off;
  int64_t skip_w16_off;
  int64_t skip_bias_off;
  int64_t skiprow_off;
  int32_t skip_tiles, skip_ld;
  int32_t skip_act, pad1_;
  int64_t u0_off;
  int64_t tau;
  int32_t B, nblocks, residual;
  int32_t ntiles;
  unsigned long long* ts;
  int64_t bias_r_off0, bias_r_stride;
  WnGenBlock blk0[3];
  float* guard;
};
struct WnGen128Args {
  const float* params;
  float* ws;
  const WnGenBlock* blocks;
  int64_t zrow_off;
  int64_t hrow_off;
  int64_t tau;
  int32_t B, nblocks, residual;
  float* guard;
  int64_t skip_w16_off, skip_bias_off, skiprow_off;
  int32_t skip_act;
  const float* xin; const float* causal_w; const float* causal_b;
  int32_t ntiles; uint32_t epoch; int64_t relay_off; unsigned* tmo;
  unsigned long long* ts;
  int32_t mute_block;
};
int wn_launch_gen_chain128(const WnGen128Args& a, hipStream_t s);
int wn_launch_gen_relay128(const WnGen128Args& a, hipStream_t s);
int64_t wn_gen_relay128_floats(int B, int nblocks);
struct WnEmit { float* out; int length; int step; float* xin_slot; };
#define WN_EMIT_NONE (WnEmit{nullptr, 0, 0, nullptr})
struct WnSampleCtl {
  float T, inv_T;
  int32_t top_k;
  float top_p;
  __host__ __device__ bool on() const { return T != 1.0f || top_k > 0 || top_p > 0.f; }
};
#define WN_SAMPLE_CTL_OFF (WnSampleCtl{1.0f, 1.0f, 0, 0.f})
#define WN_GEN_HEAD_MAX 4
struct WnGenHeadArgs {
  const float* params;
  float* ws;
  int64_t in_off;
  int64_t out_off;
  int64_t w16_off[WN_GEN_HEAD_MAX];
  int64_t bias_off[WN_GEN_HEAD_MAX];
  int32_t K[WN_GEN_HEAD_MAX], N[WN_GEN_HEAD_MAX], act[WN_GEN_HEAD_MAX];
  int32_t in_ld, nlayers, B;
  int64_t f32_w_off, f32_bias_off;
  int32_t f32_K, f32_N;
  int32_t tail, mix_M, mix_kind;
  float inv_lv;
  uint64_t seed, offset;
  float* samp;
  WnEmit em;
  float* guard;
  WnSampleCtl ctl;
};
int wn_launch_gen_head(const WnGenHeadArgs& a, hipStream_t s);
int wn_gen_blocks_supported(int R, int D, int KS);
int wn_gen_chain_max_blocks();
int64_t wn_gen_u0_floats(int B, int nblocks, int D);
int wn_gen_skip_fusable(int S);
int wn_launch_gen_blocks(const WnGenStepArgs& a, int R, int KS, int what, hipStream_t s);
int wn_launch_gen_head_pre(const WnGenHeadArgs& a, const WnGenStepArgs& g, int R, int KS, hipStream_t s);

int wn_launch_add(const float* a, const float* b, float* out, int64_t n, hipStream_t s);
int wn_launch_fill(float* p, float v, int64_t n, hipStream_t s);
int wn_launch_dact_mul(const float* g, const float* y, float* out, int64_t n, int act, hipStream_t s);
uint32_t wn_dropout_key(uint64_t seed, int block, uint64_t step);
int wn_launch_dropout(const float* x, const float* g_res, float* out, int64_t n, float rate, uint32_t key,
                      float* absmax_out, hipStream_t s);
int wn_launch_gate(const float* u, int64_t rows, int D, float* ag, float* z, int ldz, hipStream_t s);
int wn_launch_cond_scatter(const float* tmp, const float* params, int64_t b_off0, int64_t b_stride, int B, int N, int D2,
                           float* cb, hipStream_t s);
int wn_launch_cond_gather(const float* slab, int64_t P, int spb, int64_t bd_off0, int64_t bd_stride, int B, int N, int D2,
                          float* dcb, hipStream_t s);
int wn_launch_cond_wgrad(const float* m, const float* dcb, int B, int Cc, int N, int D2, float* grads, int64_t w_off0,
                         int64_t w_stride, int64_t b_off0, int64_t b_stride, hipStream_t s);
int wn_launch_skip_fold(const float* params, int64_t ws_off0, int64_t ws_stride, int64_t wf0_off, int64_t bf0_off,
                        const float* bsum, int N, int D, int S, int F0, float* V, float* bfold, float* wsall, hipStream_t s);
int wn_launch_sgemm_small(const float* A, int64_t sai, int64_t sak, const float* B, int64_t sbk, int64_t sbj, float* C, int ldc,
                          int M, int N, int K, hipStream_t s);
int wn_launch_sgemm_small_batched(const float* A, int64_t sai, int64_t sak, int64_t za, const float* B, int64_t sbk, int64_t sbj,
                                  int64_t zb, float* C, int ldc, int64_t zc, int M, int N, int K, int nz, const float* bias,
                                  int act, hipStream_t s, int zk = 0);
int wn_launch_skip_scatter(const float* Y, const float* colsum, int64_t ws_off0, int64_t ws_stride, int64_t bs_off0,
                           int64_t bs_stride, int64_t bf0_off, int N, int D, int S, int F0, float* grads, hipStream_t s);
int wn_inconv_wgrad_supported(int R, int KS);
int wn_launch_inconv_wgrad(const float* x, const float* g, int B, int T, int R, int KS, int splits_per_b, float* slab,
                           int64_t P, int64_t w_off, int64_t b_off, hipStream_t s);
int wn_launch_inconv_fwd(const float* x, const float* w, const float* bias, int B, int T, int R, int KS, float* y,
                         float* absmax_out, hipStream_t s);
int wn_launch_guard_flag(const float* absmax, float limit, int enabled, float* out, hipStream_t s);
int wn_launch_guard_accumulate(const float* src, float* dst, hipStream_t s);
int wn_launch_batch_reduce(const float* slab, int B, int splits, int N, float* out, hipStream_t s);
int64_t wn_colsum_scratch_floats(int B, int C);
int wn_launch_colsum_per_batch(const float* g, int B, int T, int C, float* out, float* scratch, hipStream_t s);
int wn_launch_quantize(const float* x, int32_t* idx, int64_t n, int bits, hipStream_t s);
int wn_launch_dequantize(const int32_t* idx, float* x, int64_t n, int bits, hipStream_t s);
int wn_launch_mulaw(const float* x, float* y, int64_t n, hipStream_t s);
int wn_launch_inv_mulaw(const float* y, float* x, int64_t n, hipStream_t s);

int wn_launch_softmax(const float* logits, float* probs, int64_t rows, int C, hipStream_t s);
int wn_launch_cat_loss(const float* logits, const int32_t* target, int64_t rows, int C,
                       float gscale, float* loss_rows, float* g_logits, float* absmax_out, hipStream_t s,
                       float* sample_out = nullptr, int bits = 8, uint64_t seed = 0, uint64_t offset = 0);
int wn_launch_cat_loss_probs(const float* probs, const int32_t* target, int64_t rows, int C,
                             float* loss_rows, hipStream_t s);
int wn_launch_mix_loss(const float* pred, const float* y, int64_t rows, int M, int bits, int kind,
                       float gscale, float* loss_rows, float* g_pred, float* absmax_out, hipStream_t s);
int wn_launch_sum(const float* v, int64_t n, float scale, float* out, float* scratch, hipStream_t s);
int wn_launch_sqdiff_sum(const float* a, const float* b, int64_t n, float scale, float* out, float* scratch, hipStream_t s);

int wn_launch_sample_det(const float* pred, int64_t rows, int C, int M, int bits, float* out, hipStream_t s,
                         WnEmit em = WN_EMIT_NONE);
int wn_launch_sample_rand(const float* pred, int64_t rows, int C, int M, int bits, int kind, uint64_t seed, uint64_t offset,
                          float* out, hipStream_t s, WnSampleCtl ctl = WN_SAMPLE_CTL_OFF, WnEmit em = WN_EMIT_NONE);
int wn_sample_from_logits_supported(int C);
int wn_launch_sample_rand_cat_logits(const float* logits, int64_t rows, int C, int bits, uint64_t seed, uint64_t offset,
                                     float* out, hipStream_t s, WnSampleCtl ctl = WN_SAMPLE_CTL_OFF, WnEmit em = WN_EMIT_NONE);
int wn_sample_top_k_max_classes();

int wn_launch_sumsq(const float* g, const WnTensorDesc* d_table, int n, float* norms2, hipStream_t s);
int wn_launch_clip(float* g, const WnTensorDesc* d_table, int n, float clipnorm, float* norms2, hipStream_t s);
int wn_launch_axpy_table(float* y, const float* x, const WnTensorDesc* d_table, int n, float coef,
                         hipStream_t s);
int wn_launch_adam(float* p, const float* g, float* m, float* v, const WnTensorDesc* d_table, int n,
                   const float* norms2, float clipnorm, float alpha, float beta1, float beta2,
                   float eps, const float* skip_flag, hipStream_t s);
int wn_launch_adam_ema(float* p, const float* g, float* m, float* v, float* a, const WnTensorDesc* d_table, int n,
                       const float* norms2, float clipnorm, float alpha, float beta1, float beta2,
                       float eps, float momentum, int first, int overwrite, const float* skip_flag, hipStream_t s);
```

wavenets_amd/csrc/wn_layer16.hip:

```cpp
#include "wn_split16.h"

using namespace wn_split16;

template <int R32, int D32, int KS>
struct WnL16 {
  static constexpr int R = 32 * R32, D = 32 * D32, JU = 2 * D32;
  static constexpr int KS1 = KS * R / 16;
  static constexpr int KS2 = D / 16;
  static constexpr int WD_BYTES = KS1 * JU * 2048;
  static constexpr int WR_BYTES = KS2 * R32 * 2048;
  static constexpr int CMAX = (R > D ? R : D);
  static constexpr int PITCH = CMAX + 4;
  static constexpr int STAGE_BYTES = 32 * PITCH * 4;
  static constexpr int WAVES = 8;
  static constexpr int BIAS_BYTES = (2 * D + R) * 4;
  static constexpr int LDS_BYTES = WD_BYTES + WR_BYTES + WAVES * STAGE_BYTES + BIAS_BYTES;
};

typedef unsigned u32x4 __attribute__((ext_vector_type(4)));
template <int C32, int PITCH>
__device__ __forceinline__ void wn_store_tile(const f32x16 (&v)[C32], float* stage, float* dst, int ld, int rows_valid, int lane) {
  const int tl = lane & 31, h = lane >> 5;
#pragma unroll
  for (int j = 0; j < C32; ++j)
#pragma unroll
    for (int rq = 0; rq < 4; ++rq) {
      f32x4 o;
      o.x = v[j][4 * rq + 0]; o.y = v[j][4 * rq + 1]; o.z = v[j][4 * rq + 2]; o.w = v[j][4 * rq + 3];
      *reinterpret_cast<f32x4*>(stage + tl * PITCH + 32 * j + 8 * rq + 4 * h) = o;
    }
  asm volatile("s_waitcnt lgkmcnt(0)" ::: "memory");
  constexpr int LPR = C32 * 8;
  constexpr int RPI = 64 / LPR;
  const __amdgpu_buffer_rsrc_t rs = __builtin_amdgcn_make_buffer_rsrc(dst, 0, rows_valid * ld * 4, 0x00020000);
#pragma unroll
  for (int i = 0; i < 32 / RPI; ++i) {
    const int row = i * RPI + lane / LPR;
    const int col = (lane % LPR) * 4;
    const f32x4 o = *reinterpret_cast<const f32x4*>(stage + row * PITCH + col);
    __builtin_amdgcn_raw_buffer_store_b128(__builtin_bit_cast(u32x4, o), rs, (row * ld + col) * 4, 0, 0);
  }
  asm volatile("" ::: "memory");
}

template <int R32, int D32, int KS, int FAST>
__global__ __launch_bounds__(512, 2) void wn_layer_fwd_f16_kernel(WnLayerFwdArgs a_in) {
  WnLayerFwdArgs a = a_in;
  if constexpr (FAST > 0) {
    a.xt[0] = a.xt[1] = a.xt[2] = nullptr; a.res = nullptr; a.o_out = nullptr; a.residual = 1;
    if constexpr (FAST != 3) a.cb = nullptr;
    if constexpr (FAST == 1) a.ag_out = nullptr;
  }
  using G = WnL16<R32, D32, KS>;
  constexpr int R = G::R, D = G::D, JU = G::JU, KS1 = G::KS1, KS2 = G::KS2, PITCH = G::PITCH;
  constexpr int QR = R / 8;
  __shared__ __attribute__((aligned(16))) unsigned char smem[G::LDS_BYTES];
  const int tid = threadIdx.x;
  const int lane = tid & 63, wave = __builtin_amdgcn_readfirstlane(tid >> 6);
  const int tl = lane & 31, h = lane >> 5;

  {
    float* sb = reinterpret_cast<float*>(smem + G::WD_BYTES + G::WR_BYTES + G::WAVES * G::STAGE_BYTES);
    static_assert(2 * D + R <= 512, "one bias element per thread");
    const float bval = tid < 2 * D ? a.bias_d[tid] : (tid < 2 * D + R ? a.bias_r[tid - 2 * D] : 0.f);
    wn_images_to_lds<512, G::WD_BYTES / 16, G::WR_BYTES / 16>(a.frag_d, smem, G::WD_BYTES / 16, a.frag_r, smem + G::WD_BYTES,
                                                               G::WR_BYTES / 16, tid);
    if (tid < 2 * D + R) sb[tid] = bval;
  }
  __syncthreads();
  const float* lbias_d = reinterpret_cast<const float*>(smem + G::WD_BYTES + G::WR_BYTES + G::WAVES * G::STAGE_BYTES);
  const float* lbias_r = lbias_d + 2 * D;
  const h8* wd = reinterpret_cast<const h8*>(smem) + lane;
  const h8* wr = reinterpret_cast<const h8*>(smem + G::WD_BYTES) + lane;
  float* stage = reinterpret_cast<float*>(smem + G::WD_BYTES + G::WR_BYTES + wave * G::STAGE_BYTES);

  const int tiles_per_b = (a.T + 31) >> 5;
  const int64_t ntiles = (int64_t)a.B * tiles_per_b;
  float wmax = 0.f;
  const WnTileWalk walk = wn_tile_walk(ntiles, G::WAVES, wave);

  struct Tile {
    int b, rows_valid;
    bool tin, xvalid[KS];
    int64_t row0;
    const float* xrow[KS];
  };
  auto tile_at = [&](int64_t tile) {
    Tile s;
    s.b = (int)(tile / tiles_per_b);
    const int t0 = (int)(tile % tiles_per_b) * 32;
    const int t = t0 + tl;
    s.tin = t < a.T;
    s.rows_valid = min(32, a.T - t0);
    s.row0 = (int64_t)s.b * a.T + t0;
#pragma unroll
    for (int tap = 0; tap < KS; ++tap) {
      const int ts = a.xt[tap] ? t : t - (KS - 1 - tap) * a.dilation;
      s.xvalid[tap] = s.tin && ts >= 0;
      s.xrow[tap] = (a.xt[tap] ? a.xt[tap] : a.x) + ((int64_t)s.b * a.T + (s.xvalid[tap] ? ts : 0)) * R + 4 * h;
    }
    return s;
  };
  f32x4 xq[KS][QR];
  f32x4 cbv = {0.f, 0.f, 0.f, 0.f};
  auto request_tap = [&](const Tile& s, auto tapc) {
    constexpr int tap = decltype(tapc)::value;
#pragma unroll
    for (int q = 0; q < QR; ++q) xq[tap][q] = *reinterpret_cast<const f32x4*>(s.xrow[tap] + 8 * q);
  };
  auto request_cb = [&](const Tile& s) {
    if (a.cb && 4 * lane < 2 * D) cbv = *reinterpret_cast<const f32x4*>(a.cb + (int64_t)s.b * 2 * D + 4 * lane);
  };

  constexpr bool ROT = FAST >= 2;
  Tile cur, nxt;
  auto do_tile = [&](int64_t tile, auto nextc, auto firstc) __attribute__((always_inline)) {
    constexpr bool has_next = ROT && decltype(nextc)::value;
    constexpr bool first = !ROT || decltype(firstc)::value;
    asm volatile("; tile body %0" ::"n"(2 * (int)has_next + (int)first) : "memory");
    if constexpr (first) {
      cur = tile_at(tile);
      wn_static_for<KS>([&](auto tapc) { request_tap(cur, tapc); });
      request_cb(cur);
    }
    if constexpr (has_next) nxt = tile_at(tile + walk.stride);
    const bool tin = cur.tin;
    const int rows_valid = cur.rows_valid;
    const int64_t row0 = cur.row0;
    __builtin_amdgcn_sched_barrier(0);
    f32x16 u[JU];
#pragma unroll
    for (int j = 0; j < JU; ++j)
#pragma unroll
      for (int rq = 0; rq < 4; ++rq) {
        const f32x4 bv = *reinterpret_cast<const f32x4*>(lbias_d + 32 * j + 8 * rq + 4 * h);
        u[j][4 * rq + 0] = bv.x; u[j][4 * rq + 1] = bv.y; u[j][4 * rq + 2] = bv.z; u[j][4 * rq + 3] = bv.w;
      }
    if (a.cb) {
      f32x4* cbl = reinterpret_cast<f32x4*>(stage);
      if (4 * lane < 2 * D) cbl[lane] = cbv;
      if constexpr (ROT) {
        if constexpr (has_next) request_cb(nxt);
      }
#pragma unroll
      for (int j = 0; j < JU; ++j)
#pragma unroll
        for (int rq = 0; rq < 4; ++rq) {
          const f32x4 cv = cbl[8 * j + 2 * rq + h];
          u[j][4 * rq + 0] += cv.x; u[j][4 * rq + 1] += cv.y; u[j][4 * rq + 2] += cv.z; u[j][4 * rq + 3] += cv.w;
        }
    }

    {
      constexpr int NB = KS1 * JU;
      h8 fr[3][2];
#pragma unroll
      for (int i = 0; i < 2; ++i) { fr[i][0] = wd[(i * 2 + 0) * 64]; fr[i][1] = wd[(i * 2 + 1) * 64]; }
      h8 bh, bl;
      wn_static_for<NB>([&](auto bc) {
        constexpr int blk = decltype(bc)::value;
        constexpr int ks = blk / JU, j = blk % JU;
        if constexpr (j == 0) {
          constexpr int tap = ks / (R / 16), kk = ks % (R / 16);
          f32x4 q0 = xq[tap][2 * kk], q1 = xq[tap][2 * kk + 1];
          if (!cur.xvalid[tap]) { q0 = f32x4{0.f, 0.f, 0.f, 0.f}; q1 = q0; }
          split8(q0, q1, bh, bl);
        }
        if constexpr (blk + 2 < NB) {
          fr[(blk + 2) % 3][0] = wd[((blk + 2) * 2 + 0) * 64];
          fr[(blk + 2) % 3][1] = wd[((blk + 2) * 2 + 1) * 64];
        }
        mfma3(fr[blk % 3][0], fr[blk % 3][1], bh, bl, u[j]);
        __builtin_amdgcn_sched_barrier(0);
        if constexpr (has_next && j == 0 && (ks + 1) % (R / 16) == 0 && ks / (R / 16) < KS - 1) {
          request_tap(nxt, std::integral_constant<int, ks / (R / 16)>{});
          __builtin_amdgcn_sched_barrier(0);
        }
      });
    }

    if (a.ag_out) {
#pragma unroll
      for (int j = 0; j < D32; ++j)
#pragma unroll
        for (int r = 0; r < 16; ++r) {
          u[j + D32][r] = wn_sigmoid_fast(u[j + D32][r]);
          u[j][r] = wn_tanh_fast(u[j][r]) * u[j + D32][r];
        }
      {
        f32x16 gv[D32];
#pragma unroll
        for (int j = 0; j < D32; ++j) gv[j] = u[j + D32];
        wn_store_tile<D32, PITCH>(gv, stage, a.ag_out + row0 * D, D, rows_valid, lane);
      }
    } else {
#pragma unroll
      for (int j = 0; j < D32; ++j)
#pragma unroll
        for (int r = 0; r < 16; ++r) u[j][r] = wn_tanh_fast(u[j][r]) * wn_sigmoid_fast(u[j + D32][r]);
    }
    if (a.z_out) {
      f32x16 zv[D32];
#pragma unroll
      for (int j = 0; j < D32; ++j) zv[j] = u[j];
      wn_store_tile<D32, PITCH>(zv, stage, a.z_out + row0 * a.ldz, a.ldz, rows_valid, lane);
    }

    f32x16 o[R32];
#pragma unroll
    for (int j = 0; j < R32; ++j)
#pragma unroll
      for (int rq = 0; rq < 4; ++rq) {
        const f32x4 bv = *reinterpret_cast<const f32x4*>(lbias_r + 32 * j + 8 * rq + 4 * h);
        o[j][4 * rq + 0] = bv.x; o[j][4 * rq + 1] = bv.y; o[j][4 * rq + 2] = bv.z; o[j][4 * rq + 3] = bv.w;
      }
    {
      constexpr int NB = KS2 * R32;
      h8 fr[3][2];
#pragma unroll
      for (int i = 0; i < 2 && i < NB; ++i) { fr[i][0] = wr[(i * 2 + 0) * 64]; fr[i][1] = wr[(i * 2 + 1) * 64]; }
      h8 bh, bl;
      wn_static_for<NB>([&](auto bc) {
        constexpr int blk = decltype(bc)::value;
        constexpr int ks = blk / R32, j = blk % R32;
        if constexpr (j == 0) {
          constexpr int jz = ks / 2, r0 = 8 * (ks % 2);
          f32x4 q0, q1;
          q0.x = u[jz][r0 + 0]; q0.y = u[jz][r0 + 1]; q0.z = u[jz][r0 + 2]; q0.w = u[jz][r0 + 3];
          q1.x = u[jz][r0 + 4]; q1.y = u[jz][r0 + 5]; q1.z = u[jz][r0 + 6]; q1.w = u[jz][r0 + 7];
          split8(q0, q1, bh, bl);
        }
        if constexpr (blk + 2 < NB) {
          fr[(blk + 2) % 3][0] = wr[((blk + 2) * 2 + 0) * 64];
          fr[(blk + 2) % 3][1] = wr[((blk + 2) * 2 + 1) * 64];
        }
        mfma3(fr[blk % 3][0], fr[blk % 3][1], bh, bl, o[j]);
        __builtin_amdgcn_sched_barrier(0);
      });
    }

    if (a.o_out) wn_store_tile<R32, PITCH>(o, stage, a.o_out + row0 * R, R, rows_valid, lane);
    if (a.residual) {
#pragma unroll
      for (int j = 0; j < R32; ++j)
#pragma unroll
        for (int rq = 0; rq < 4; ++rq) {
          f32x4 xr;
          if (a.res) xr = tin ? *reinterpret_cast<const f32x4*>(a.res + (row0 + tl) * R + 32 * j + 8 * rq + 4 * h)
                              : f32x4{0.f, 0.f, 0.f, 0.f};
          else xr = xq[KS - 1][j * 4 + rq];
          o[j][4 * rq + 0] += xr.x; o[j][4 * rq + 1] += xr.y; o[j][4 * rq + 2] += xr.z; o[j][4 * rq + 3] += xr.w;
        }
    }
    if constexpr (has_next) {
      __builtin_amdgcn_sched_barrier(0);
      request_tap(nxt, std::integral_constant<int, KS - 1>{});
      __builtin_amdgcn_sched_barrier(0);
    }
    if (tin) {
#pragma unroll
      for (int j = 0; j < R32; ++j)
#pragma unroll
        for (int r = 0; r < 16; ++r) wmax = fmaxf(wmax, fabsf(o[j][r]));
    }
    wn_store_tile<R32, PITCH>(o, stage, a.x_out + row0 * R, R, rows_valid, lane);
    if constexpr (has_next) cur = nxt;
  };
  using Next = std::true_type;
  using Last = std::false_type;
  using First = std::true_type;
  using Later = std::false_type;
  if constexpr (ROT) {
    if (walk.first < walk.end) {
// ... 50 lines not shown
```

wavenets_amd/csrc/wn_loss.hip:

```cpp
#include <algorithm>

#include "wn_kernels.h"
#include "wn_sample.h"

__global__ __launch_bounds__(256) void wn_softmax_kernel(const float* logits, float* probs,
                                                         int64_t rows, int C) {
  const int lane = threadIdx.x & 63;
  const int64_t row = (int64_t)blockIdx.x * 4 + (threadIdx.x >> 6);
  if (row >= rows) return;
  WnSoftmaxLoop(logits + row * C, C, lane).each([&](int j, float q) { probs[row * C + j] = q; });
}
int wn_launch_softmax(const float* logits, float* probs, int64_t rows, int C, hipStream_t s) {
  if (rows <= 0) return WN_OK;
  hipLaunchKernelGGL(wn_softmax_kernel, dim3((unsigned)((rows + 3) / 4)), dim3(256), 0, s, logits,
                     probs, rows, C);
  WN_HIP_CHECK(hipGetLastError());
  return WN_OK;
}

__global__ __launch_bounds__(256) void wn_cat_loss256_kernel(const float* logits, const int32_t* target,
                                                             int64_t rows, int C, float gscale,
                                                             float* loss_rows, float* g_logits, float* absmax_out,
                                                             float* sample_out, float inv_lv, uint64_t seed, uint64_t offset) {
  __shared__ float qs[4][256];
// ... 32 lines not shown
  }
}

__global__ __launch_bounds__(256) void wn_cat_loss_kernel(const float* logits, const int32_t* target,
                                                          int64_t rows, int C, float gscale,
                                                          float* loss_rows, float* g_logits, float* absmax_out) {
  const int lane = threadIdx.x & 63;
  const int64_t row = (int64_t)blockIdx.x * 4 + (threadIdx.x >> 6);
  if (row >= rows) return;
  float gmax = 0.f;
  wn_cat_ce_row(WnSoftmaxLoop(logits + row * C, C, lane), target[row], gscale, loss_rows + row, g_logits, row * C, gmax);
  if (g_logits && absmax_out) {
    gmax = wn_wave_max(gmax);
    if (lane == 0) wn_absmax_publish(absmax_out, gmax);
  }
}
int wn_launch_cat_loss(const float* logits, const int32_t* target, int64_t rows, int C,
                       float gscale, float* loss_rows, float* g_logits, float* absmax_out, hipStream_t s,
                       float* sample_out, int bits, uint64_t seed, uint64_t offset) {
  if (rows <= 0) return WN_OK;
  if (sample_out && C > 256) { wn_set_error("cat_loss: the in-kernel sample draw needs <= 256 classes"); return WN_E_UNSUPPORTED; }
  const float inv_lv = sample_out ? 1.0f / (float)(1 << (bits - 1)) : 0.f;
  if (C <= 256) {
    const int64_t wgs = std::min<int64_t>((rows + 3) / 4, 256 * 8);
    hipLaunchKernelGGL(wn_cat_loss256_kernel, dim3((unsigned)wgs), dim3(256), 0, s, logits, target, rows, C, gscale,
                       loss_rows, g_logits, absmax_out, sample_out, inv_lv, seed, offset);
  } else {
    hipLaunchKernelGGL(wn_cat_loss_kernel, dim3((unsigned)((rows + 3) / 4)), dim3(256), 0, s, logits,
                       target, rows, C, gscale, loss_rows, g_logits, absmax_out);
  }
  WN_HIP_CHECK(hipGetLastError());
  return WN_OK;
}

__global__ __launch_bounds__(256) void wn_cat_loss_probs_kernel(const float* probs,
                                                                const int32_t* target, int64_t rows,
                                                                int C, float* loss_rows) {
  const int lane = threadIdx.x & 63;
  const int64_t row = (int64_t)blockIdx.x * 4 + (threadIdx.x >> 6);
  if (row >= rows) return;
  const float* q = probs + row * C;
  float S = 0.f;
  for (int j = lane; j < C; j += 64) S += wn_ce_clip(q[j]);
  S = wn_wave_sum(S);
  const float pt = wn_ce_clip(q[wn_ce_target(target[row], C)]);
  if (lane == 0) loss_rows[row] = wn_ce_loss(pt, S);
}
int wn_launch_cat_loss_probs(const float* probs, const int32_t* target, int64_t rows, int C,
                             float* loss_rows, hipStream_t s) {
  if (rows <= 0) return WN_OK;
  hipLaunchKernelGGL(wn_cat_loss_probs_kernel, dim3((unsigned)((rows + 3) / 4)), dim3(256), 0, s,
                     probs, target, rows, C, loss_rows);
  WN_HIP_CHECK(hipGetLastError());
  return WN_OK;
}

#define WN_MAXMIX 32
__device__ __forceinline__ double wn_sigmoid_d(double x) { return 1.0 / (1.0 + exp(-x)); }
__device__ __forceinline__ double wn_dsigmoid_d(double x) { return wn_sigmoid_d(x) * wn_sigmoid_d(-x); }
__device__ __forceinline__ bool wn_logistic_bin(double a, double b, double& hi, double& lo) {
  const bool up = a + b > 0.0;
  hi = up ? -b : a;
  lo = up ? -a : b;
  return up;
}
__global__ void wn_mix_loss_kernel(const float* pred, const float* y, int64_t rows, int M, int bits,
                                   int kind, float gscale, float* loss_rows, float* g_pred, float* absmax_out) {
  const int64_t row = (int64_t)blockIdx.x * blockDim.x + threadIdx.x;
  if (row >= rows) return;
  const float* p = pred + row * 3 * M;
  const double yy = (double)y[row];
  double w[WN_MAXMIX], comp[WN_MAXMIX];
  double wm = -INFINITY;
  for (int k = 0; k < M; ++k) wm = fmax(wm, (double)p[k]);
  double wz = 0.0;
  for (int k = 0; k < M; ++k) { w[k] = exp((double)p[k] - wm); wz += w[k]; }
  const double winv = 1.0 / wz;
  const double halfbit = 0.5 / (double)(1 << bits);
  const double sqrt2pi = sqrt(2.0 * 3.14159265359);
  double lik = 0.0;
  for (int k = 0; k < M; ++k) {
    w[k] *= winv;
    const double mu = (double)p[M + k];
    const double ls = fmax((double)p[2 * M + k], -7.0);
    if (kind == 1) {
      const double inv = exp(-ls);
      double hi, lo;
      wn_logistic_bin((yy - mu + halfbit) * inv, (yy - mu - halfbit) * inv, hi, lo);
      comp[k] = wn_sigmoid_d(hi) - wn_sigmoid_d(lo);
    } else {
      const double sc = exp(ls);
      const double xx = fmin((yy - mu) / sc, 1e8);
      comp[k] = exp(-0.5 * xx * xx) / (sc * sqrt2pi);
    }
    lik += w[k] * comp[k];
  }
  loss_rows[row] = (float)(-log(lik));
  if (!g_pred) return;
  float* g = g_pred + row * 3 * M;
  const double dl = -(double)gscale / lik;
  for (int k = 0; k < M; ++k) {
    const double mu = (double)p[M + k];
    const double lsr = (double)p[2 * M + k];
    const double ls = fmax(lsr, -7.0);
    const double lsmask = lsr >= -7.0 ? 1.0 : 0.0;
    g[k] = (float)(dl * (w[k] * comp[k] - w[k] * lik));
    if (kind == 1) {
      const double inv = exp(-ls);
      double hi, lo;
      const bool up = wn_logistic_bin((yy - mu + halfbit) * inv, (yy - mu - halfbit) * inv, hi, lo);
      const double dhi = wn_dsigmoid_d(hi), dlo = wn_dsigmoid_d(lo);
      g[M + k] = (float)(dl * (-w[k] * inv * (up ? dlo - dhi : dhi - dlo)));
      g[2 * M + k] = (float)(dl * lsmask * (-w[k] * (hi * dhi - lo * dlo)));
    } else {
      const double sc = exp(ls);
      const double xr = (yy - mu) / sc;
      const double xx = fmin(xr, 1e8);
      const double xmask = xr <= 1e8 ? 1.0 : 0.0;
      const double pdf = comp[k];
      g[M + k] = (float)(dl * w[k] * pdf * xx / sc * xmask);
      g[2 * M + k] = (float)(dl * lsmask * w[k] * pdf * (xx * xx * xmask - 1.0));
    }
  }
  if (absmax_out) {
    float gmax = 0.f;
    for (int k = 0; k < 3 * M; ++k) gmax = fmaxf(gmax, fabsf(g[k]));
    wn_absmax_publish(absmax_out, gmax);
  }
}
int wn_launch_mix_loss(const float* pred, const float* y, int64_t rows, int M, int bits, int kind,
                       float gscale, float* loss_rows, float* g_pred, float* absmax_out, hipStream_t s) {
  if (rows <= 0) return WN_OK;
  if (M < 1 || M > WN_MAXMIX) { wn_set_error("mix_loss: num_mixtures %d unsupported (max %d)", M, WN_MAXMIX); return WN_E_UNSUPPORTED; }
  hipLaunchKernelGGL(wn_mix_loss_kernel, dim3((unsigned)((rows + 255) / 256)), dim3(256), 0, s, pred,
                     y, rows, M, bits, kind, gscale, loss_rows, g_pred, absmax_out);
  WN_HIP_CHECK(hipGetLastError());
  return WN_OK;
}

__global__ void wn_sum_stage1(const float* v, int64_t n, double* scratch) {
  __shared__ double sm[256];
  double acc = 0.0;
  for (int64_t i = (int64_t)blockIdx.x * blockDim.x + threadIdx.x; i < n;
       i += (int64_t)gridDim.x * blockDim.x)
    acc += (double)v[i];
  sm[threadIdx.x] = acc;
  __syncthreads();
  for (int o = 128; o > 0; o >>= 1) {
    if (threadIdx.x < o) sm[threadIdx.x] += sm[threadIdx.x + o];
    __syncthreads();
  }
  if (threadIdx.x == 0) scratch[blockIdx.x] = sm[0];
}
__global__ void wn_sum_stage2(const double* scratch, int nb, float scale, float* out) {
  __shared__ double sm[256];
  double acc = 0.0;
  for (int i = threadIdx.x; i < nb; i += blockDim.x) acc += scratch[i];
  sm[threadIdx.x] = acc;
  __syncthreads();
  for (int o = 128; o > 0; o >>= 1) {
    if (threadIdx.x < o) sm[threadIdx.x] += sm[threadIdx.x + o];
    __syncthreads();
  }
  if (threadIdx.x == 0) out[0] = (float)(sm[0] * (double)scale);
}
int wn_launch_sum(const float* v, int64_t n, float scale, float* out, float* scratch, hipStream_t s) {
  int nb = wn_blocks(n, 256, 1024);
  hipLaunchKernelGGL(wn_sum_stage1, dim3(nb), dim3(256), 0, s, v, n, reinterpret_cast<double*>(scratch));
  hipLaunchKernelGGL(wn_sum_stage2, dim3(1), dim3(256), 0, s, reinterpret_cast<const double*>(scratch), nb, scale, out);
  WN_HIP_CHECK(hipGetLastError());
  return WN_OK;
}

__global__ void wn_sqdiff_stage1(const float* a, const float* b, int64_t n, double* scratch) {
  __shared__ double sm[256];
  double acc = 0.0;
  for (int64_t i = (int64_t)blockIdx.x * blockDim.x + threadIdx.x; i < n;
       i += (int64_t)gridDim.x * blockDim.x) {
    const float d = a[i] - b[i];
    acc += (double)(d * d);
  }
  sm[threadIdx.x] = acc;
  __syncthreads();
  for (int o = 128; o > 0; o >>= 1) {
    if (threadIdx.x < o) sm[threadIdx.x] += sm[threadIdx.x + o];
    __syncthreads();
  }
  if (threadIdx.x == 0) scratch[blockIdx.x] = sm[0];
}
int wn_launch_sqdiff_sum(const float* a, const float* b, int64_t n, float scale, float* out, float* scratch, hipStream_t s) {
  int nb = wn_blocks(n, 256, 1024);
  hipLaunchKernelGGL(wn_sqdiff_stage1, dim3(nb), dim3(256), 0, s, a, b, n, reinterpret_cast<double*>(scratch));
  hipLaunchKernelGGL(wn_sum_stage2, dim3(1), dim3(256), 0, s, reinterpret_cast<const double*>(scratch), nb, scale, out);
  WN_HIP_CHECK(hipGetLastError());
  return WN_OK;
}
```

wavenets_amd/csrc/wn_plan_internal.h:

```cpp
#pragma once
#include <math.h>
#include <stdlib.h>
#include <string.h>

#include <algorithm>
#include <mutex>
#include <vector>

#include "../../include/wn_hip.h"
#include "wn_kernels.h"

namespace wnp {

inline int64_t align64(int64_t v) { return (v + 63) & ~(int64_t)63; }
inline int ceil32(int v) { return (v + 31) / 32; }
inline int ceil8(int v) { return (v + 7) / 8 * 8; }

struct TensorInfo {
  int64_t off, len;
  int ndim;
  int64_t shape[3];
  int is_kernel;
};

// ... 182 lines not shown
  int64_t sum_scratch;
  std::vector<int64_t> M;
  int64_t cb;
  int64_t dcb, g_m0, g_m1;
  int64_t cbt;
  int64_t total;
};

inline bool al16(const void* p) { return (((uintptr_t)p) & 15) == 0; }

struct Gemm {
  WnGemmArgs a;
  const float* w16_ = nullptr;
  const float* am0_ = nullptr;
  const float* am1_ = nullptr;
  float* amo_ = nullptr;
  Gemm& w16(const float* img) { w16_ = img; return *this; }
  Gemm& absmax(const float* in0, const float* in1, float* out) { am0_ = in0; am1_ = in1; amo_ = out; return *this; }
  Gemm& absmax_fwd(float* out) { amo_ = out; a.absmax_any = out ? 1 : 0; return *this; }
  Gemm(int B, int T, int N, int JTtot) {
    memset(&a, 0, sizeof(a));
    a.B = B; a.T = T; a.N = N; a.JTtot = JTtot; a.act = WN_ACT_LINEAR; a.epi = WN_EPI_PLAIN;
  }
  Gemm& seg(const float* x, int ldx, int K, int shift, const float* frag) {
    WnSeg& s = a.seg[a.nseg++];
    s.x = x; s.ldx = ldx; s.K = K; s.shift = shift; s.frag = frag;
    s.vec = (ldx % 4 == 0 && K % 4 == 0 && al16(x)) ? 1 : 0;
    s.plane_k = 0; s.plane_stride = 0;
    return *this;
  }
  Gemm& seg_planes(const float* x, int plane_k, int64_t plane_stride, int K, const float* frag) {
    seg(x, plane_k, K, 0, frag);
    WnSeg& s = a.seg[a.nseg - 1];
    s.plane_k = plane_k; s.plane_stride = plane_stride;
    s.vec = (plane_k % 4 == 0 && plane_stride % 4 == 0 && al16(x)) ? 1 : 0;
    return *this;
  }
  Gemm& bias(const float* b) { a.bias = b; return *this; }
  Gemm& rowbias(const float* b, int ld) { a.rowbias = b; a.ld_rowbias = ld; return *this; }
  Gemm& addc(const float* c, int ld) { a.addc = c; a.ld_addc = ld; return *this; }
  Gemm& act(int act) { a.act = act; return *this; }
  Gemm& dact(const float* ysaved, int ld, int act) { a.epi = WN_EPI_DACT; a.aux = ysaved; a.ld_aux = ld; a.act = act; return *this; }
  Gemm& gate_bwd(const float* g, int ldg, const float* z, int ldz) {
    a.epi = WN_EPI_GATE_BWD; a.aux = g; a.ld_aux = ldg; a.aux2 = z; a.ld_aux2 = ldz;
    return *this;
  }
  Gemm& gate_fwd(float* sig, int ld) { a.epi = WN_EPI_GATE_FWD; a.y2 = sig; a.ld_y2 = ld; return *this; }
  int run(float* y, int ldy, hipStream_t s) {
    a.y = y; a.ldy = ldy;
    bool v = (a.N % 4 == 0) && (ldy % 4 == 0) && al16(y);
    if (a.bias) v = v && al16(a.bias);
    if (a.addc) v = v && (a.ld_addc % 4 == 0) && al16(a.addc);
    if (a.aux) v = v && (a.ld_aux % 4 == 0) && al16(a.aux);
    if (a.aux2) v = v && (a.ld_aux2 % 4 == 0) && al16(a.aux2);
    if (a.y2) v = v && (a.ld_y2 % 4 == 0) && al16(a.y2);
    a.vec_out = v ? 1 : 0;
    if (w16_ && wn_debug_get(1) != 1 && wn_gemm_rows16_ok(a)) return wn_launch_gemm_rows16(a, w16_, am0_, am1_, amo_, s);
    if (a.epi == WN_EPI_GATE_FWD) { wn_set_error("gate-forward contraction needs the split-precision kernel (alignment / shape)"); return WN_E_UNSUPPORTED; }
    for (int i = 0; i < a.nseg; ++i)
      if (!a.seg[i].frag) { wn_set_error("contraction without an fp32 weight image needs the split-precision kernel"); return WN_E_UNSUPPORTED; }
    return wn_launch_gemm_rows(a, s);
  }
};

struct BlockPtrs {
  int B, T, KS, R, D, S, Cin, depth, act, residual;
  int dil[16];
  const float* Wd[16]; const float* bd[16];
  const float* br; const float* bs; const float* bc;
  const float* Fd[16]; const float* Bd[16]; int64_t Fd_stride[16], Bd_stride[16];
  const float* Fr; const float* Br_;
  const float* Fs; const float* Bs;
  const float* Fc; const float* Bc;
  int Cc;
  const float* cond;
  const float* cb;
  bool fused;
  const float* F16d; const float* F16r;
  const float* G16u; const float* G16x;
  const float* G16uf;
  const float* F16g;
  const float* F16n;
  const float* F16i[16]; const float* G16i[16];
  int JTi[16], JTb[16], JTu;
};

struct BlockBufs {
  const float* x;
  float* P[16];
  float* U;
  float* AG;
  float* Z; int ldz;
  float* O;
  float* x_out;
  const float* xt[3];
  const float* res;
  bool pre_done;
  float* fwd_absmax;
};

struct BlockGrads {
  const float* g_xout;
  const float* g_skip;
  float* g_o_tmp;
  float* g_u;
  float* g_p;
  float* g_pi[16];
  float* g_x;
  float* g_cond;
  float* dWd[16]; float* dbd[16];
  float* dWr; float* dbr; float* dWs; float* dbs; float* dWc; float* dbc;
  float* dcb;
  float* slab;
  bool defer;
  const float* am_gxout; const float* am_gskip;
  float* am_gu; float* am_gx;
  float* am_gp[16];
  const float* g_fold; int fold_F0; const float* am_gfold;
  float drop_rate; uint32_t drop_key; float* g_xd;
};

struct GenRings {
  float* xin;
  std::vector<float*> h;
  std::vector<int> nslots;
  std::vector<std::vector<float*>> hp;
  std::vector<std::vector<int>> nslots_p;
};

inline bool m16(int v) { return v > 0 && v % 16 == 0; }
inline bool m32(int v) { return v >= 64 && v % 32 == 0; }

int ensure_device_tables(wn_plan* p);
WsLayout make_layout(const wn_plan* p, int B, int T, bool training);
bool deep16(const wn_plan* p);
bool cond_small(const wn_plan* p);
bool fold_ok(const wn_plan* p);
bool head_pairs_ok(const wn_plan* p);
TrainPaths train_paths(const wn_plan* p);
TrainPaths train_paths(const wn_plan* p, const wn_exec& e, const WsLayout& L, int64_t rows);
int64_t slab_need(int B, int T, int K, int N);
int wgrad(const float* x, int ldx, int K, int shift, const float* g, int ldg, int N, int B, int T,
          float* dW, float* db, float* per_batch, float* slab, hipStream_t s);
int block_forward(const BlockPtrs& k, const BlockBufs& f, hipStream_t s);
int block_backward(const BlockPtrs& k, const BlockBufs& f, const BlockGrads& g, hipStream_t s);
struct LossFuse {
  const int32_t* target; float gscale; float* loss_rows; float* g_logits; float* absmax_out;
  float* sample_out; float inv_lv; uint64_t seed, offset;
  bool done;
};
bool loss_fusable(const wn_plan* p, int64_t rows);
BlockPtrs block_ptrs(const wn_plan* p, int b, const float* params, const float* fragbase, int B, int T);
void deep16_ptrs(const wn_plan* p, int b, const float* fragbase, BlockPtrs& k);
int forward_core(wn_plan* p, const float* params, const float* x, bool prep, const float* cond, int B,
                 int T, bool training, float* ws, const WsLayout& L, hipStream_t s, const GenRings* rings = nullptr,
                 LossFuse* lf = nullptr);
int shift_split(const float* x_full, int B, int T, float* inputs, float* y_true, hipStream_t s);
int loss_stage(wn_plan* p, int B, int T, int global_batch, bool want_grad, float* ws, const WsLayout& L,
               float* loss_out, float* absmax_out, hipStream_t s, bool fused_done = false);

}

int wn_sampling_check(const char* who, const wn_sampling* sp, int head, int classes, WnSampleCtl* ctl);
```

wavenets_amd/csrc/wn_train.hip:

```cpp
#include "wn_plan_internal.h"

namespace {
using namespace wnp;

void add_jobs(std::vector<WnWgJob>& jobs, int64_t x_off, int ldx, int K, int shift, int64_t g_off, int ldg, int N,
              int64_t out_off, int64_t bias_off, int64_t gmax_off) {
  const int tk = wn_wgrad_tile_k(), tn = wn_wgrad_tile_n();
  for (int k0 = 0; k0 < K; k0 += tk)
    for (int n0 = 0; n0 < N; n0 += tn) {
      WnWgJob j;
      memset(&j, 0, sizeof(j));
      j.x_off = x_off; j.g_off = g_off; j.out_off = out_off; j.bias_off = (k0 == 0) ? bias_off : -1;
      j.gmax_off = gmax_off;
      j.ldx = ldx; j.ldg = ldg; j.K = K; j.N = N; j.shift = shift; j.k0 = k0; j.n0 = n0;
      jobs.push_back(j);
    }
}

int ensure_schedule(const wn_plan* p, wn_exec& e, const WsLayout& L, int B, int T, const TrainPaths& tp) {
  WgSchedule& g = e.wg;
  if (g.valid && g.B == B && g.T == T && g.bsplits == L.bsplits && g.paths == tp) return WN_OK;
  const bool layerk = tp.layerk(), pairk = tp.pairk(), fold = tp.fold;
  std::vector<WnWgLayer> wgl, wgli;
  std::vector<WnWgPair> pairs[3];
// ... 40 lines not shown
      w.gmax_u_off = am_GU(b); w.gmax_h_off = p->S == 0 ? am_skip : am_GH(b + 1);
      w.dilation = c.dil;
      wgl.push_back(w);
    } else if (pairk) {
      const int64_t xoff = tp.drop ? L.XD[b] : L.H[b];
      {
        WnWgPair w;
        memset(&w, 0, sizeof(w));
        w.x_off = xoff; w.g_off = L.GU[b]; w.shift = c.dil;
        w.w_off = p->tensors[c.kernel_t].off;
        w.b_off = p->tensors[c.bias_t].off;
        w.gmax_off = am_GU(b);
        pairs[1].push_back(w);
      }
      WnWgPair w;
      memset(&w, 0, sizeof(w));
      w.x_off = zoff; w.g_off = p->S == 0 ? L.GO[b] : L.GH[b + 1]; w.shift = 0;
      w.w_off = p->tensors[bi.conv1.kernel_t].off; w.b_off = p->tensors[bi.conv1.bias_t].off;
      w.gmax_off = p->S == 0 ? am_skip : am_GH(b + 1);
      w.g2_off = w.w2_off = w.b2_off = w.gmax2_off = -1;
      if (tp.mfused) {
        w.g2_off = L.GF[0]; w.w2_off = (int64_t)b * p->D * p->fold_F0;
        w.b2_off = b == 0 ? (int64_t)p->N * p->D * p->fold_F0 : -1;
        w.gmax2_off = L.absmax + slot.gf(0);
      }
      pairs[2].push_back(w);
    } else {
    for (int i = 0; i < p->LPB; ++i) {
      const ConvInfo& ci = bi.dil[i];
      const bool lastc = i == p->LPB - 1;
      const int64_t xo = i == 0 ? (tp.drop ? L.XD[b] : L.H[b]) : L.P[b][i - 1];
      const int kc = i == 0 ? p->R : p->D, nc = lastc ? 2 * p->D : p->D;
      for (int t = 0; t < p->KS; ++t)
        add_jobs(jobs, xo, kc, kc, (p->KS - 1 - t) * ci.dil, lastc ? L.GU[b] : L.GP[b][i], nc, nc,
                 p->tensors[ci.kernel_t].off + (int64_t)t * kc * nc,
                 t == p->KS - 1 ? p->tensors[ci.bias_t].off : -1, lastc ? am_GU(b) : am_GP(b, i));
      if (!lastc) { cover(ci.kernel_t); cover(ci.bias_t); }
    }
    add_jobs(jobs, zoff, p->Dp, p->D, 0, p->S == 0 ? L.GO[b] : L.GH[b + 1], p->R, p->R,
             p->tensors[bi.conv1.kernel_t].off, p->tensors[bi.conv1.bias_t].off, p->S == 0 ? am_skip : am_GH(b + 1));
    }
    cover(bi.dil.back().kernel_t); cover(bi.dil.back().bias_t);
    cover(bi.conv1.kernel_t); cover(bi.conv1.bias_t);
    if (bi.has_skip && p->c.use_skip && !fold) {
      if (!tp.skipk)
        add_jobs(jobs, zoff, p->Dp, p->D, 0, L.g_skipsum, p->S, p->S,
                 p->tensors[bi.conv_skip.kernel_t].off, p->tensors[bi.conv_skip.bias_t].off, am_skip);
      cover(bi.conv_skip.kernel_t); cover(bi.conv_skip.bias_t);
    }
  }
  if (tp.mtr != 0) {
    const int per = 256 / p->D;
    for (int b0 = 0; b0 < p->N; b0 += per) {
      WnWgPair w;
      memset(&w, 0, sizeof(w));
      w.x_off = L.Z + (int64_t)b0 * B * T * p->Dp;
      w.seg_stride = (int64_t)B * T * p->Dp;
      w.nseg = std::min(per, p->N - b0);
      w.g_off = L.GF[0]; w.shift = 0;
      w.w_off = (int64_t)b0 * p->D * p->fold_F0;
      w.b_off = b0 == 0 ? (int64_t)p->N * p->D * p->fold_F0 : -1;
      w.gmax_off = L.absmax + slot.gf(0);
      w.w2_off = w.b2_off = w.gmax2_off = -1;
      pairs[0].push_back(w);
    }
  }
  const int head_first = (int)jobs.size(), cov_head = (int)cov.size();
  for (size_t i = fold ? 1 : 0; i < p->finals.size(); ++i) {
    const ConvInfo& c = p->finals[i];
    const int64_t xin = (i == 0) ? (p->c.use_skip ? L.skipsum : L.H[p->N]) : L.HA[i - 1];
    if (tp.headpairs() && wn_wgrad_pair_kind(c.cin, c.cout) != 0) {
      WnWgPair w;
      memset(&w, 0, sizeof(w));
      w.x_off = xin; w.g_off = L.GF[i]; w.shift = 0;
      w.w_off = p->tensors[c.kernel_t].off; w.b_off = p->tensors[c.bias_t].off;
      w.gmax_off = L.absmax + slot.gf((int)i);
      const int kind = wn_wgrad_pair_kind(c.cin, c.cout);
      hpairs[kind].push_back(w);
      if (kind == 5) {
        w.g_off += 128; w.w_off += 128; w.b_off += 128;
        hpairs[kind].push_back(w);
      }
    } else {
      add_jobs(jobs, xin, c.cin, c.cin, 0, L.GF[i], c.cout, c.cout, p->tensors[c.kernel_t].off,
               p->tensors[c.bias_t].off, L.absmax + slot.gf((int)i));
    }
    cover(c.kernel_t); cover(c.bias_t);
  }
  std::vector<WnWgPair> all;
  int pfirst[3], hfirst[6] = {0, 0, 0, 0, 0, 0};
  for (int kd = 0; kd <= 2; ++kd) { pfirst[kd] = (int)all.size(); all.insert(all.end(), pairs[kd].begin(), pairs[kd].end()); }
  for (int kd = 1; kd <= 5; ++kd) { hfirst[kd] = (int)all.size(); all.insert(all.end(), hpairs[kd].begin(), hpairs[kd].end()); }
  std::vector<WgSpan> spans;
  auto span = [&](WgSpan::Op op, WgSpan::Slab slab, int kind, int first, size_t count) {
    if (count > 0) spans.push_back(WgSpan{op, slab, kind, first, (int)count});
  };
  const int njobs = (int)jobs.size();
  const bool head_own = tp.head_split && (head_first < njobs || tp.headpairs());
  span(WgSpan::INCONV, WgSpan::BATCH, 0, 0, tp.in_split);
  span(WgSpan::JOBS, WgSpan::BATCH, tp.wg == WG_GENERIC_FP32, 0, head_own ? head_first : njobs);
  if (head_own) span(WgSpan::JOBS, WgSpan::HEAD, 0, head_first, njobs - head_first);
  for (int kd = 1; kd <= 5; ++kd) {
    const int trk = kd == 1 ? 3 : (kd == 3 ? 4 : (kd == 5 ? 5 : (kd == 2 ? 2 : 0)));
    if (trk != 0 && tp.pairk()) span(WgSpan::TR, WgSpan::HEAD, trk, hfirst[kd], hpairs[kd].size());
    else span(WgSpan::PAIRS, WgSpan::HEAD, kd, hfirst[kd], hpairs[kd].size());
  }
  const int n_side = (int)spans.size();
  span(WgSpan::TR, WgSpan::BATCH, 1, pfirst[1], pairs[1].size());
  span(WgSpan::TR, WgSpan::BATCH, tp.mfused ? 6 : 2, pfirst[2], pairs[2].size());
  span(WgSpan::LAYERS, WgSpan::BATCH, 0, 0, wgl.size());
  span(WgSpan::LAYERS, WgSpan::BATCH, 1, 0, wgli.size());
  if (tp.mtr != 0) span(WgSpan::TR, WgSpan::MFOLD, tp.mtr, pfirst[0], pairs[0].size());
  else if (tp.fold) span(WgSpan::SKIP, WgSpan::MFOLD, 0, 0, !tp.mfused);
  else span(WgSpan::SKIP, WgSpan::BATCH, 0, 0, tp.skipk);
  g.valid = false;
  int rc = g.jobs.upload(jobs, 1);
  if (!rc) rc = g.cov.upload(cov);
  if (!rc) rc = g.layers.upload(wgl);
  if (!rc) rc = g.inner.upload(wgli);
  if (!rc) rc = g.pairs.upload(all);
  if (rc) return rc;
  g.h_cov.swap(cov); g.spans.swap(spans);
  g.n_side = n_side; g.overlap = layerk || pairk; g.cov_head = head_own ? cov_head : (int)g.h_cov.size();
  g.B = B; g.T = T; g.bsplits = L.bsplits; g.paths = tp;
  g.valid = true;
  return WN_OK;
}

struct TrainCall {
  wn_exec& e;
  wn_plan* p; const float* params; const float* x_full; const float* cond;
  int B, T, global_batch, n_replicas;
  float* grads; float* loss_out; float* pred_out; float* ws; hipStream_t s;
  WsLayout L;
  int64_t rows;
  float* inputs;
  const float* fragbase; float* slab;
  float* am; AbsmaxSlots slot;
  int nf; float* am_gskip;
  const float* mlast = nullptr;
  TrainPaths tp;
  bool cond_batched = false;
  int64_t pm = 0;
  float* am_GF(int i) const { return am + slot.gf(i); }
  float* am_GU(int b) const { return am + slot.gu(b); }
  float* am_GH(int b) const { return am + slot.gh(b); }
  float* am_GP(int b, int i) const { return am + slot.gp(b, i); }
  struct Strided { int64_t off, stride; };
  Strided strided(int t0, int t1) const { return {p->tensors[t0].off, p->N > 1 ? p->tensors[t1].off - p->tensors[t0].off : 0}; }
  Strided skip_w{0, 0}, skip_b{0, 0};

  int forward_and_loss() {
    int rc;
    { const int rcs = shift_split(x_full, B, T, inputs, ws + L.yt, s); if (rcs) return rcs; }
    if (e.phase_on) (void)hipEventRecord(e.phase_ev[0], s);
    WN_HIP_CHECK(hipMemsetAsync(am, 0, L.n_absmax * sizeof(float), s));
    LossFuse lf;
    memset(&lf, 0, sizeof(lf));
    const bool fuse = !pred_out && loss_fusable(p, rows);
    if (fuse) {
      rc = wn_launch_quantize(ws + L.yt, reinterpret_cast<int32_t*>(ws + L.target), rows, p->c.bits, s);
      if (rc) return rc;
      lf.target = reinterpret_cast<const int32_t*>(ws + L.target);
      lf.gscale = 1.0f / (float)global_batch;
      lf.loss_rows = ws + L.loss_rows; lf.g_logits = ws + L.GF.back(); lf.absmax_out = am_GF(nf - 1);
      if (e.step_sample && !e.step_sample_det) {
        lf.sample_out = e.step_sample; lf.inv_lv = 1.0f / (float)(1 << (p->c.bits - 1));
        lf.seed = e.step_sample_seed; lf.offset = e.step_sample_off;
      }
    }
    rc = forward_core(p, params, inputs, true, cond, B, T, true, ws, L, s, nullptr, fuse ? &lf : nullptr);
    if (rc) return rc;
    if (lf.done && lf.sample_out) e.step_sample = nullptr;
    if (e.phase_on) (void)hipEventRecord(e.phase_ev[1], s);
    rc = loss_stage(p, B, T, global_batch, true, ws, L, loss_out, am_GF(nf - 1), s, lf.done);
    if (rc) return rc;
    if (pred_out) {
      if (p->c.head == WN_HEAD_CATEGORICAL) rc = wn_launch_softmax(ws + L.logits, pred_out, rows, p->Cout, s);
      else rc = hipMemcpyAsync(pred_out, ws + L.logits, rows * p->Cout * sizeof(float), hipMemcpyDeviceToDevice, s) == hipSuccess ? WN_OK : WN_E_HIP;
      if (rc) return rc;
    }
    if (e.step_sample) {
      float* so = e.step_sample;
      e.step_sample = nullptr;
      if (p->c.head == WN_HEAD_CATEGORICAL) {
        if (e.step_sample_det) {
          wn_set_error("step sample: deterministic categorical draws go through wn_sample_waveform");
          return WN_E_UNSUPPORTED;
        }
        rc = wn_launch_sample_rand_cat_logits(ws + L.logits, rows, p->Cout, p->c.bits, e.step_sample_seed, e.step_sample_off, so, s);
      } else {
        if (e.step_sample_det) rc = wn_launch_sample_det(ws + L.logits, rows, p->Cout, p->c.num_mixtures, p->c.bits, so, s);
        else rc = wn_launch_sample_rand(ws + L.logits, rows, p->Cout, p->c.num_mixtures, p->c.bits, p->c.head, e.step_sample_seed, e.step_sample_off, so, s);
      }
      if (rc) return rc;
    }
    if (p->c.l2_reg_factor > 0.f) {
      float* norms = ws + L.loss_rows;
      rc = wn_launch_sumsq(params, p->d_kdesc, (int)p->kdesc.size(), norms, s);
      if (rc) return rc;
      rc = wn_launch_sum(norms, (int64_t)p->kdesc.size(), p->c.l2_reg_factor / (float)n_replicas, loss_out + 1, ws + L.sum_scratch, s);
      if (rc) return rc;
    } else {
      rc = wn_launch_fill(loss_out + 1, 0.f, 1, s);
      if (rc) return rc;
    }
    rc = wn_launch_guard_flag(ws + L.fwd_absmax, WN_RANGE_LIMIT * (e.drop_rate > 0.f ? 1.f - e.drop_rate : 1.f),
                              wn_debug_get(1) != 1, loss_out + 2, s);
    if (rc) return rc;
    if (e.phase_on) (void)hipEventRecord(e.phase_ev[2], s);
    return WN_OK;
  }

  int cond_block_bwd(const BlockInfo& bi) {
    const ConvInfo& c = bi.conv_cond;
    int r = wgrad(mlast, p->Cc, p->Cc, 0, ws + L.dcb, 2 * p->D, 2 * p->D, 1, B, grads + p->tensors[c.kernel_t].off,
                  grads + p->tensors[c.bias_t].off, nullptr, slab, s);
    if (r) return r;
    return Gemm(1, B, p->Cc, ceil32(p->Cc)).seg(ws + L.dcb, 2 * p->D, 2 * p->D, 0, fragbase + c.fragB)
        .addc(ws + L.g_m0, p->Cc).run(ws + L.g_m0, p->Cc, s);
  }

  int head_backward() {
    int rc;
    float* head_out = p->c.use_skip ? ws + L.g_skipsum : ws + L.GH[p->N];
    for (int i = (int)p->finals.size() - 1; i >= (tp.fold ? 1 : 0); --i) {
      const ConvInfo& c = p->finals[i];
      float* dst = (i == 0) ? head_out : ws + L.GF[i - 1];
      if (c.frag16B >= 0 && wn_debug_get(1) != 1 && wn_gemm_planes16s_supported(c.cin, c.cout, 1, c.cout, c.cin) &&
          (int64_t)rows * c.cout * 4 < ((int64_t)1 << 32)) {
        WnGemmPlanesArgs ga;
        memset(&ga, 0, sizeof(ga));
        ga.z = ws + L.GF[i]; ga.ld = c.cout; ga.plane_k = c.cout; ga.nplanes = 1;
        ga.w16 = fragbase + c.frag16B; ga.act = p->c.activation;
        ga.y = dst; ga.ldy = c.cin; ga.N = c.cin; ga.B = B; ga.T = T;
        ga.bwd = 1; ga.absmax_in = am_GF(i);
        ga.absmax_out = i > 0 ? am_GF(i - 1) : (p->c.use_skip ? am_gskip : am_GH(p->N));
        if (i > 0) { ga.aux = ws + L.HA[i - 1]; ga.ld_aux = c.cin; }
        rc = wn_launch_gemm_planes16s(ga, s);
        if (rc) return rc;
        continue;
      }
      Gemm gm(B, T, c.cin, ceil32(c.cin));
      gm.seg(ws + L.GF[i], c.cout, c.cout, 0, fragbase + c.fragB);
      if (i > 0) gm.dact(ws + L.HA[i - 1], c.cin, p->c.activation);
      if (c.frag16B >= 0)
        gm.w16(fragbase + c.frag16B).absmax(am_GF(i), nullptr, i > 0 ? am_GF(i - 1) : (p->c.use_skip ? am_gskip : am_GH(p->N)));
      rc = gm.run(dst, c.cin, s);
      if (rc) return rc;
    }
    return WN_OK;
  }

  int chain_backward() {
    int rc;
    const float* g_skip = (p->c.use_skip && !tp.fold) ? ws + L.g_skipsum : nullptr;
    if (p->c.use_skip) {
      rc = wn_launch_fill(ws + L.GH[p->N], 0.f, rows * p->R, s);
      if (rc) return rc;
    }
    const bool pairk = tp.bwd_pairs();
    for (int b = p->N - 1; b >= 0; --b) {
      BlockPtrs k = block_ptrs(p, b, params, fragbase, B, T);
      deep16_ptrs(p, b, fragbase, k);
      const BlockInfo& bi = p->blocks[b];
      if (pairk && b < p->N - 1) {
        const BlockPtrs k1 = block_ptrs(p, b + 1, params, fragbase, B, T);
        WnBwdPairArgs a;
        memset(&a, 0, sizeof(a));
        a.gu_in = ws + L.GU[b + 1]; a.gx_res = ws + L.GH[b + 2]; a.gf = ws + L.GF[0];
        a.ag = ws + L.AG[b]; a.z = ws + L.Z + (int64_t)b * rows * p->Dp; a.ldz = p->Dp;
        a.gx_out = ws + L.GH[b + 1]; a.gu_out = ws + L.GU[b];
        a.wx16 = k1.G16x; a.wu16 = k.G16uf;
        a.am_gu_in = am_GU(b + 1); a.am_gf = am_GF(0); a.am_gx = am_GH(b + 1); a.am_gu = am_GU(b);
        a.B = B; a.T = T; a.dil = k1.dil[0];
        if (!a.wx16 || !a.wu16) { wn_set_error("bwd_pair: weight images missing"); return WN_E_UNSUPPORTED; }
        rc = tp.bwd == BWD_S128 ? wn_launch_bwd_s128(a, s) : wn_launch_bwd_pair(a, s);
        if (rc) return rc;
        if (b == 0) {
          Gemm gm(B, T, p->R, ceil32(p->R));
          for (int t = 0; t < p->KS; ++t)
            gm.seg(ws + L.GU[0], 2 * p->D, 2 * p->D, -(p->KS - 1 - t) * k.dil[0], k.Bd[0] + t * k.Bd_stride[0]);
          if (p->c.use_residual) gm.addc(ws + L.GH[1], p->R);
          gm.w16(k.G16x).absmax(am_GU(0), nullptr, am_GH(0));
          rc = gm.run(ws + L.GH[0], p->R, s);
          if (rc) return rc;
        }
        continue;
      }
      BlockBufs f;
      memset(&f, 0, sizeof(f));
      f.x = tp.drop ? ws + L.XD[b] : ws + L.H[b];
      for (int i = 0; i + 1 < p->LPB; ++i) f.P[i] = ws + L.P[b][i];
      f.AG = ws + L.AG[b];
      f.Z = ws + L.Z + (int64_t)b * rows * p->Dp; f.ldz = p->Dp;
      BlockGrads bg;
      memset(&bg, 0, sizeof(bg));
      bg.defer = true;
      for (int i = 0; i + 1 < p->LPB; ++i) bg.g_pi[i] = ws + L.GP[b][i];
      if (tp.deep16)
        for (int i = 0; i + 1 < p->LPB; ++i) bg.am_gp[i] = am_GP(b, i);
      if (tp.drop) {
        bg.drop_rate = e.drop_rate; bg.drop_key = wn_dropout_key(e.drop_seed, b, e.drop_step); bg.g_xd = ws + L.gxd;
      }
      bg.g_xout = (p->c.use_skip && b == p->N - 1 && p->S == 0) ? nullptr : ws + L.GH[b + 1];
      bg.g_skip = g_skip;
      bg.g_o_tmp = p->S == 0 ? ws + L.GO[b] : nullptr;
      bg.g_u = ws + L.GU[b];
      bg.g_x = pairk ? nullptr : ws + L.GH[b];
      bg.dcb = (bi.has_cond && !cond_batched) ? ws + L.dcb : nullptr;
      bg.slab = slab;
      bg.am_gxout = bg.g_xout ? am_GH(b + 1) : nullptr;
      bg.am_gskip = g_skip ? am_gskip : nullptr;
      bg.am_gu = am_GU(b); bg.am_gx = am_GH(b);
      if (tp.fold) { bg.g_fold = ws + L.GF[0]; bg.fold_F0 = p->fold_F0; bg.am_gfold = am_GF(0); }
      rc = block_backward(k, f, bg, s);
      if (rc) return rc;
      if (p->S == 0 && bg.g_xout == nullptr && g_skip) {
        WN_HIP_CHECK(hipMemcpyAsync(ws + L.GO[b], g_skip, rows * p->R * sizeof(float), hipMemcpyDeviceToDevice, s));
      }
      if (bi.has_cond && !cond_batched) {
        rc = cond_block_bwd(bi);
        if (rc) return rc;
      }
    }
    return WN_OK;
  }

  int fold_weight_gradients() {
    const int F0 = p->fold_F0;
    int rc = wn_launch_reduce_table(ws + L.mslab, B * L.bsplits, pm, ws + L.mtot, p->d_cov_fold, 1, s, &p->h_cov_fold);
    if (rc) return rc;
    const ConvInfo& c0 = p->finals[0];
    const int nd1 = p->N * p->D + 1;
    const float* wf0 = params + p->tensors[c0.kernel_t].off;
    rc = wn_launch_sgemm_small(ws + L.mtot, F0, 1, wf0, 1, F0, ws + L.ytmp, p->S, nd1, p->S, F0, s);
    if (rc) return rc;
    const int nzk = (nd1 + 127) / 128;
    if ((int64_t)nzk * p->S * F0 <= L.slab_floats) {
      rc = wn_launch_sgemm_small_batched(ws + L.wsall, 1, p->S, (int64_t)128 * p->S, ws + L.mtot, F0, 1, (int64_t)128 * F0, slab, F0,
                                         (int64_t)p->S * F0, p->S, F0, nd1, nzk, nullptr, 0, s, 128);
      if (rc) return rc;
      WnVecSumArgs v;
      v.base = slab; v.off0 = 0; v.stride = (int64_t)p->S * F0; v.count = nzk; v.len = p->S * F0;
      v.out = grads + p->tensors[c0.kernel_t].off;
      rc = wn_launch_vecsum(v, s);
    } else
    rc = wgrad(ws + L.wsall, p->S, p->S, 0, ws + L.mtot, F0, F0, 1, nd1, grads + p->tensors[c0.kernel_t].off, nullptr, nullptr,
               slab, s);
    if (rc) return rc;
    return wn_launch_skip_scatter(ws + L.ytmp, ws + L.mtot + (int64_t)p->N * p->D * F0, skip_w.off, skip_w.stride, skip_b.off,
                                  skip_b.stride, p->tensors[c0.bias_t].off, p->N, p->D, p->S, F0, grads, s);
  }

  int cond_weight_gradients() {
    int rc;
    const int D2 = 2 * p->D;
    const BlockInfo& b0 = p->blocks[0]; const BlockInfo& b1 = p->blocks[p->N > 1 ? 1 : 0];
    const Strided db = strided(b0.dil.back().bias_t, b1.dil.back().bias_t);
    const Strided cw = strided(b0.conv_cond.kernel_t, b1.conv_cond.kernel_t), cbi = strided(b0.conv_cond.bias_t, b1.conv_cond.bias_t);
    rc = wn_launch_cond_gather(ws + L.bslab, p->nparams, L.bsplits, db.off, db.stride, B, p->N, D2, ws + L.cbt, s);
    if (rc) return rc;
    if (cond_small(p) && (int64_t)p->N * B * p->Cc <= L.slab_floats) {
      rc = wn_launch_sgemm_small_batched(ws + L.cbt, p->N * D2, 1, D2, params + cw.off, 1, D2, cw.stride,
                                         slab, p->Cc, (int64_t)B * p->Cc, B, p->Cc, D2, p->N, nullptr, 0, s);
      if (rc) return rc;
      WnVecSumArgs v;
      v.base = slab; v.off0 = 0; v.stride = (int64_t)B * p->Cc; v.count = p->N; v.len = B * p->Cc; v.out = ws + L.g_m0;
      rc = wn_launch_vecsum(v, s);
    } else
    rc = Gemm(1, B, p->Cc, ceil32(p->Cc)).seg(ws + L.cbt, p->N * D2, p->N * D2, 0, fragbase + p->frag_condB).run(ws + L.g_m0, p->Cc, s);
    if (rc) return rc;
    return wn_launch_cond_wgrad(mlast, ws + L.cbt, B, p->Cc, p->N, D2, grads, cw.off, cw.stride, cbi.off, cbi.stride, s);
  }

  int launch(const WgSpan& sp, hipStream_t st) {
    const WgSchedule& g = e.wg;
    float* out = ws + L.bslab; int64_t pitch = p->nparams; int splits = L.bsplits;
    if (sp.slab == WgSpan::HEAD) { out = ws + L.hslab - L.head_base; pitch = L.head_span; splits = L.hsplits; }
    if (sp.slab == WgSpan::MFOLD) { out = ws + L.mslab; pitch = pm; }
    switch (sp.op) {
      case WgSpan::INCONV:
        return wn_launch_inconv_wgrad(inputs, ws + L.GH[0], B, T, p->R, p->KS, L.isplits, ws + L.islab, (int64_t)(p->KS + 1) * p->R,
                                      0, (int64_t)p->KS * p->R, st);
      case WgSpan::JOBS: return wn_launch_wgrad_batched(g.jobs.d + sp.first, sp.count, ws, out, pitch, B, T, splits, st, sp.kind != 0);
      case WgSpan::PAIRS: return wn_launch_wgrad_pairs(sp.kind, g.pairs.d + sp.first, sp.count, ws, out, pitch, B, T, splits, st);
      case WgSpan::TR:
        return wn_launch_wgrad_tr(sp.kind, g.pairs.d + sp.first, sp.count, ws, out, pitch, B, T, splits, st,
                                  sp.kind == 6 ? ws + L.mslab : nullptr, sp.kind == 6 ? pm : 0);
      case WgSpan::LAYERS: return wn_launch_wgrad_layers(sp.kind ? g.inner.d : g.layers.d, sp.count, p->R, ws, out, pitch, B, T, splits, st, sp.kind);
      case WgSpan::SKIP:
        if (sp.slab == WgSpan::MFOLD)
          return wn_launch_wgrad_skip(ws + L.Z, p->Dp, ws + L.GF[0], p->fold_F0, rows, p->N * p->D, p->fold_F0, p->D, B * splits, out, pitch,
                                      0, (int64_t)p->D * p->fold_F0, (int64_t)p->N * p->D * p->fold_F0, 0, 1, am_GF(0), st);
        return wn_launch_wgrad_skip(ws + L.Z, p->Dp, ws + L.g_skipsum, p->S, rows, p->N * p->D, p->S, p->D, B * splits, out, pitch,
                                    skip_w.off, skip_w.stride, skip_b.off, skip_b.stride, p->N, am_gskip, st);
    }
    return WN_E_INVALID;
  }

  int weight_gradients() {
    int rc;
    const WgSchedule& g = e.wg;
    if (e.phase_on) (void)hipEventRecord(e.phase_ev[3], s);
    const bool fork = g.overlap && wn_debug_get(9) != 1;
    if (fork && !e.side) {
      WN_HIP_CHECK(hipStreamCreateWithFlags(&e.side, hipStreamNonBlocking));
      WN_HIP_CHECK(hipEventCreateWithFlags(&e.ev_fork, hipEventDisableTiming));
      WN_HIP_CHECK(hipEventCreateWithFlags(&e.ev_join, hipEventDisableTiming));
    }
    struct SideJoin {
      wn_exec& e; hipStream_t s; bool armed;
      ~SideJoin() {
        if (!armed) return;
        if (hipEventRecord(e.ev_join, e.side) != hipSuccess || hipStreamWaitEvent(s, e.ev_join, 0) != hipSuccess)
          (void)hipStreamSynchronize(e.side);
      }
    } side_join{e, s, false};
    if (fork) {
      WN_HIP_CHECK(hipEventRecord(e.ev_fork, s));
      WN_HIP_CHECK(hipStreamWaitEvent(e.side, e.ev_fork, 0));
      side_join.armed = true;
    }
    size_t i = 0;
    for (; i < (size_t)g.n_side; ++i)
      if ((rc = launch(g.spans[i], fork ? e.side : s))) return rc;
    if (fork) WN_HIP_CHECK(hipEventRecord(e.ev_join, e.side));
    for (; i < g.spans.size(); ++i)
      if ((rc = launch(g.spans[i], s))) return rc;
    if (tp.fold && (rc = fold_weight_gradients())) return rc;
    if (fork) { WN_HIP_CHECK(hipStreamWaitEvent(s, e.ev_join, 0)); side_join.armed = false; }
    if (cond_batched && (rc = cond_weight_gradients())) return rc;
    const int cov0 = tp.in_split ? 2 : 0, ncov = (int)g.h_cov.size(), cov1 = g.cov_head;
    rc = wn_launch_reduce_table(ws + L.bslab, B * L.bsplits, p->nparams, grads, g.cov.d + cov0, cov1 - cov0, s, g.h_cov.data() + cov0);
    if (rc) return rc;
    if (tp.in_split && (rc = wn_launch_reduce_table(ws + L.islab, B * L.isplits, (int64_t)(p->KS + 1) * p->R, grads, g.cov.d, 2, s, g.h_cov.data())))
      return rc;
    if (cov1 < ncov && (rc = wn_launch_reduce_table(ws + L.hslab - L.head_base, B * L.hsplits, L.head_span, grads, g.cov.d + cov1, ncov - cov1,
                                                    s, g.h_cov.data() + cov1)))
      return rc;
    if (!p->c.use_skip && p->S > 0) {
      for (const BlockInfo& bi : p->blocks) {
        rc = wn_launch_fill(grads + p->tensors[bi.conv_skip.kernel_t].off, 0.f, p->tensors[bi.conv_skip.kernel_t].len, s);
        if (!rc) rc = wn_launch_fill(grads + p->tensors[bi.conv_skip.bias_t].off, 0.f, p->tensors[bi.conv_skip.bias_t].len, s);
        if (rc) return rc;
      }
    }
    return WN_OK;
  }

  int mapping_backward() {
    int rc;
    if (p->c.cond_inputs > 0) {
      const float* gm_cur = ws + L.g_m0;
      float* gm_other = ws + L.g_m1;
      for (int j = (int)p->mapping.size() - 1; j >= 0; --j) {
        const ConvInfo& c = p->mapping[j];
        const float* yin = (j == 0) ? cond : ws + L.M[j - 1];
        rc = wn_launch_dact_mul(gm_cur, ws + L.M[j], gm_other, (int64_t)B * c.cout, p->c.mapping_activation, s);
        if (rc) return rc;
        if (cond_small(p)) {
          rc = wn_launch_sgemm_small_batched(yin, 1, c.cin, 0, gm_other, c.cout, 1, 0, grads + p->tensors[c.kernel_t].off, c.cout, 0,
                                             c.cin, c.cout, B, 1, nullptr, 0, s);
          if (rc) return rc;
          WnVecSumArgs v;
          v.base = gm_other; v.off0 = 0; v.stride = c.cout; v.count = B; v.len = c.cout; v.out = grads + p->tensors[c.bias_t].off;
          rc = wn_launch_vecsum(v, s);
          if (rc) return rc;
          if (j > 0) {
            float* dst = const_cast<float*>(gm_cur);
            rc = wn_launch_sgemm_small_batched(gm_other, c.cout, 1, 0, params + p->tensors[c.kernel_t].off, 1, c.cout, 0, dst, c.cin, 0,
                                               B, c.cin, c.cout, 1, nullptr, 0, s);
            if (rc) return rc;
          }
          continue;
        }
        rc = wgrad(yin, c.cin, c.cin, 0, gm_other, c.cout, c.cout, 1, B, grads + p->tensors[c.kernel_t].off,
                   grads + p->tensors[c.bias_t].off, nullptr, slab, s);
        if (rc) return rc;
        if (j > 0) {
          float* dst = const_cast<float*>(gm_cur);
          rc = Gemm(1, B, c.cin, ceil32(c.cin)).seg(gm_other, c.cout, c.cout, 0, fragbase + c.fragB).run(dst, c.cin, s);
          if (rc) return rc;
        }
      }
    }
    return WN_OK;
  }

  int backward() {
    int rc;
    fragbase = ws + L.frag;
    slab = ws + L.slab;
    if (p->c.cond_inputs > 0) {
      mlast = p->mapping.empty() ? cond : ws + L.M.back();
      rc = wn_launch_fill(ws + L.g_m0, 0.f, (int64_t)B * p->Cc, s);
      if (rc) return rc;
    }
    cond_batched = p->frag_condB >= 0;
    tp = train_paths(p, e, L, rows);
    pm = (int64_t)p->N * p->D * p->fold_F0 + p->fold_F0;
    if (p->blocks[0].has_skip) {
      const BlockInfo& b0 = p->blocks[0]; const BlockInfo& b1 = p->blocks[p->N > 1 ? 1 : 0];
      skip_w = strided(b0.conv_skip.kernel_t, b1.conv_skip.kernel_t); skip_b = strided(b0.conv_skip.bias_t, b1.conv_skip.bias_t);
    }
    rc = ensure_schedule(p, e, L, B, T, tp);
    if (rc) return rc;
    if ((rc = head_backward())) return rc;
    if ((rc = chain_backward())) return rc;
    if ((rc = weight_gradients())) return rc;
    if ((rc = mapping_backward())) return rc;
    if (p->c.l2_reg_factor > 0.f) {
      rc = wn_launch_axpy_table(grads, params, p->d_kdesc, (int)p->kdesc.size(), 2.0f * p->c.l2_reg_factor / (float)n_replicas, s);
      if (rc) return rc;
    }
    if (e.phase_on) {
      (void)hipEventRecord(e.phase_ev[4], s);
    }

    return WN_OK;
  }
};

}

extern "C" int wn_plan_set_train_phases(wn_plan* p, int32_t phases) {
  if (!p || phases < 1 || phases > 3) { wn_set_error("set_train_phases: 1 (forward + loss), 2 (backward), 3 (both)"); return WN_E_INVALID; }
  wnp::ex(p).train_phases = phases;
  return WN_OK;
}

extern "C" int wn_train_fwd_bwd(wn_plan* p, const float* params, const float* x_full, const float* cond,
                                int32_t B, int32_t T, int32_t global_batch, int32_t n_replicas, float* grads,
                                float* loss_out, float* pred_out, float* workspace, int64_t ws_floats,
                                void* stream) {
  if (!p || !params || !x_full || !workspace || !loss_out || !grads || B < 1 || T < 1) { wn_set_error("train_fwd_bwd: bad arguments"); return WN_E_INVALID; }
  TrainCall c{wnp::ex(p)};
  c.p = p; c.params = params; c.x_full = x_full; c.cond = cond; c.B = B; c.T = T;
  c.global_batch = global_batch > 0 ? global_batch : B;
  c.n_replicas = n_replicas > 0 ? n_replicas : 1;
  c.grads = grads; c.loss_out = loss_out; c.pred_out = pred_out; c.ws = workspace; c.s = (hipStream_t)stream;
  c.L = make_layout(p, B, T, true);
  if (ws_floats < c.L.total) { wn_set_error("train_fwd_bwd: workspace too small (%lld < %lld floats)", (long long)ws_floats, (long long)c.L.total); return WN_E_INVALID; }
  c.rows = (int64_t)B * T;
  c.inputs = workspace + c.L.probs;
  c.am = workspace + c.L.absmax;
  c.nf = (int)p->finals.size();
  c.slot = AbsmaxSlots{c.nf, p->N, p->LPB};
  c.am_gskip = c.am + c.slot.gskip();
  const int phases = c.e.train_phases;
  int rc = WN_OK;
  if (phases & 1) rc = c.forward_and_loss();
  if (!rc && (phases & 2)) rc = c.backward();
  return rc;
}

extern "C" int wn_adam_step_guarded(wn_plan* p, float* params, const float* grads, float* m, float* v, int64_t step,
                                    float lr, float beta1, float beta2, float eps, float clipnorm, float* scratch,
                                    const float* skip_flag, void* stream) {
  if (!p || !params || !grads || !m || !v || !scratch || step < 1) { wn_set_error("adam_step: bad arguments"); return WN_E_INVALID; }
  hipStream_t s = (hipStream_t)stream;
  int rc = ensure_device_tables(p);
  if (rc) return rc;
  const int n = (int)p->tdesc.size();
  if (clipnorm > 0.f) {
    rc = wn_launch_sumsq(grads, p->d_tdesc, n, scratch, s);
    if (rc) return rc;
  }
  const double alpha = (double)lr * sqrt(1.0 - pow((double)beta2, (double)step)) / (1.0 - pow((double)beta1, (double)step));
  return wn_launch_adam(params, grads, m, v, p->d_tdesc, n, scratch, clipnorm, (float)alpha, beta1, beta2, eps, skip_flag, s);
}

extern "C" int wn_adam_step_ema(wn_plan* p, float* params, const float* grads, float* m, float* v, float* ema, int64_t step,
                                float lr, float beta1, float beta2, float eps, float clipnorm, float ema_momentum,
                                int32_t ema_overwrite, float* scratch, const float* skip_flag, void* stream) {
  if (!p || !params || !grads || !m || !v || !ema || !scratch || step < 1) { wn_set_error("adam_step_ema: bad arguments"); return WN_E_INVALID; }
  if (!std::isfinite(ema_momentum) || ema_momentum < 0.f || ema_momentum > 1.f) {
    wn_set_error("adam_step_ema: ema_momentum must be finite and in [0, 1] (got %g)", (double)ema_momentum);
    return WN_E_INVALID;
  }
  if (ema_overwrite != 0 && ema_overwrite != 1) { wn_set_error("adam_step_ema: ema_overwrite must be 0 or 1 (got %d)", (int)ema_overwrite); return WN_E_INVALID; }
  hipStream_t s = (hipStream_t)stream;
  int rc = ensure_device_tables(p);
  if (rc) return rc;
  const int n = (int)p->tdesc.size();
  if (clipnorm > 0.f) {
    rc = wn_launch_sumsq(grads, p->d_tdesc, n, scratch, s);
    if (rc) return rc;
  }
  const double alpha = (double)lr * sqrt(1.0 - pow((double)beta2, (double)step)) / (1.0 - pow((double)beta1, (double)step));
  return wn_launch_adam_ema(params, grads, m, v, ema, p->d_tdesc, n, scratch, clipnorm, (float)alpha, beta1, beta2, eps,
                            ema_momentum, step == 1 ? 1 : 0, (int)ema_overwrite, skip_flag, s);
}
// ... 15 lines not shown
```

Baseline: 22.80 million.

## Fuse step-entry kernels, merge reductions, and prefetch tiles before weight LDS load

Several launch-reduction changes land together. The shift/split, quantize and input conv are fused into one step-entry kernel. The absmax memsets are merged into one, and the guard flag and the zero fill are folded into the loss-sum stage2 kernel. The three gradient slab reductions become a single launch. Separately, the backward-pair and layer16 kernels now issue the first tile's global loads before staging weights into LDS, so load latency overlaps the weight copy.

```diff
diff --git a/wavenets_amd/csrc/wn_bwd_pair.hip b/wavenets_amd/csrc/wn_bwd_pair.hip
--- a/wavenets_amd/csrc/wn_bwd_pair.hip
+++ b/wavenets_amd/csrc/wn_bwd_pair.hip
@@ -41,16 +41,8 @@
   const int lane = tid & 63, wave = tid >> 6;
   const int tl = lane & 31, h = lane >> 5;
   float* stage = reinterpret_cast<float*>(smem + BP_W1 + BP_W2 + wave * BP_STAGE);
-  {
-    wn_images_to_lds<512, BP_W1 / 16, BP_W2 / 16>(a.wx16, smem, BP_W1 / 16, a.wu16, smem + BP_W1, BP_W2 / 16, tid);
-  }
-  __syncthreads();
   const h8* w1 = reinterpret_cast<const h8*>(smem) + lane;
   const h8* w2 = reinterpret_cast<const h8*>(smem + BP_W1) + lane;
-
-  float sc1, inv1;
-  pow2_scale(a.am_gu_in ? *a.am_gu_in : 0.f, sc1, inv1);
-  const float gfmax = a.am_gf ? *a.am_gf : 0.f;
 
   const int tiles_per_b = (a.T + 31) >> 5;
   const int64_t ntiles = (int64_t)a.B * tiles_per_b;
@@ -84,11 +76,18 @@
   TileCtx cur, nxt;
   f32x4 xr[BP_PF][2];
   bool okr[BP_PF];
-  if (tile < tend) {
-    make_ctx(tile, cur);
-#pragma unroll
-    for (int k = 0; k < BP_PF; ++k) load_x(cur, k, xr[k][0], xr[k][1], okr[k]);
-  }
+  make_ctx(tile < ntiles ? tile : ntiles - 1, cur);
+#pragma unroll
+  for (int k = 0; k < BP_PF; ++k) load_x(cur, k, xr[k][0], xr[k][1], okr[k]);
+  const float gumax = a.am_gu_in ? *a.am_gu_in : 0.f;
+  const float gfmax = a.am_gf ? *a.am_gf : 0.f;
+  __builtin_amdgcn_sched_barrier(0);
+  {
+    wn_images_to_lds<512, BP_W1 / 16, BP_W2 / 16>(a.wx16, smem, BP_W1 / 16, a.wu16, smem + BP_W1, BP_W2 / 16, tid);
+  }
+  __syncthreads();
+  float sc1, inv1;
+  pow2_scale(gumax, sc1, inv1);
   for (; tile < tend; tile += tstride) {
     const bool has_next = tile + tstride < tend;
     if (has_next) make_ctx(tile + tstride, nxt);
diff --git a/wavenets_amd/csrc/wn_common.h b/wavenets_amd/csrc/wn_common.h
--- a/wavenets_amd/csrc/wn_common.h
+++ b/wavenets_amd/csrc/wn_common.h
@@ -134,6 +134,11 @@
 
 #define WN_RANGE_LIMIT 30000.0f
 
+__device__ __forceinline__ float wn_guard_flag(const float* absmax, float limit, int enabled) {
+  const float m = absmax ? *absmax : 0.f;
+  return (enabled && !(m < limit)) ? 1.0f : 0.0f;
+}
+
 __device__ __forceinline__ void wn_guard_publish_over(float* slot, float wmax) {
   const unsigned m = __float_as_uint(wmax);
   if (m >= __float_as_uint(WN_RANGE_LIMIT)) {
diff --git a/wavenets_amd/csrc/wn_elem.hip b/wavenets_amd/csrc/wn_elem.hip
--- a/wavenets_amd/csrc/wn_elem.hip
+++ b/wavenets_amd/csrc/wn_elem.hip
@@ -483,6 +483,56 @@
   return WN_OK;
 }
 
+__global__ __launch_bounds__(256) void wn_step_entry_kernel(const float* x_full, const float* w, const float* bias, int B, int T,
+                                                            int R, int KS, int bits, float* inputs, float* y_true,
+                                                            int32_t* target, float* y, float* absmax_out) {
+  const int q = R / 4;
+  const int64_t total = (int64_t)B * T * q;
+  float wmax = 0.f;
+  for (int64_t i = (int64_t)blockIdx.x * blockDim.x + threadIdx.x; i < total; i += (int64_t)gridDim.x * blockDim.x) {
+    const int c = (int)(i % q) * 4;
+    const int64_t row = i / q;
+    const int t = (int)(row % T);
+    const float* xrow = x_full + row + row / T;
+    float a0 = 0.f, a1 = 0.f, a2 = 0.f, a3 = 0.f;
+    for (int tap = 0; tap < KS; ++tap) {
+      const int ts = t - (KS - 1 - tap);
+      const float xv = ts >= 0 ? xrow[-(KS - 1 - tap)] : 0.f;
+      const f32x4 wv = *reinterpret_cast<const f32x4*>(w + (int64_t)tap * R + c);
+      a0 = fmaf(wv.x, xv, a0); a1 = fmaf(wv.y, xv, a1); a2 = fmaf(wv.z, xv, a2); a3 = fmaf(wv.w, xv, a3);
+    }
+    const f32x4 bv = *reinterpret_cast<const f32x4*>(bias + c);
+    const f32x4 o = f32x4{a0 + bv.x, a1 + bv.y, a2 + bv.z, a3 + bv.w};
+    *reinterpret_cast<f32x4*>(y + row * R + c) = o;
+    wmax = fmaxf(wmax, fmaxf(fmaxf(fabsf(o.x), fabsf(o.y)), fmaxf(fabsf(o.z), fabsf(o.w))));
+    if (c == 0) {
+      const float yt = xrow[1];
+      inputs[row] = xrow[0];
+      y_true[row] = yt;
+      if (target) target[row] = wn_quantize_one(yt, bits);
+    }
+  }
+  if (absmax_out) {
+    __shared__ float wm[4];
+    if (!(wmax < 3.0e38f)) wmax = 3.0e38f;
+    wmax = wn_wave_max(wmax);
+    if ((threadIdx.x & 63) == 0) wm[threadIdx.x >> 6] = wmax;
+    __syncthreads();
+    if (threadIdx.x == 0) wn_absmax_publish_any(absmax_out, fmaxf(fmaxf(wm[0], wm[1]), fmaxf(wm[2], wm[3])));
+  }
+}
+int wn_launch_step_entry(const float* x_full, const float* w, const float* bias, int B, int T, int R, int KS, int bits,
+                         float* inputs, float* y_true, int32_t* target, float* y, float* absmax_out, hipStream_t s) {
+  const int64_t total = (int64_t)B * T * (R / 4);
+  if (total <= 0) return WN_OK;
+  if (R % 4 != 0) { wn_set_error("step_entry: R = %d is not a multiple of 4", R); return WN_E_UNSUPPORTED; }
+  if (target && (bits < 1 || bits > 16)) { wn_set_error("quantize: bits %d unsupported", bits); return WN_E_UNSUPPORTED; }
+  hipLaunchKernelGGL(wn_step_entry_kernel, dim3((unsigned)std::min<int64_t>((total + 255) / 256, 1024)), dim3(256), 0, s, x_full, w,
+                     bias, B, T, R, KS, bits, inputs, y_true, target, y, absmax_out);
+  WN_HIP_CHECK(hipGetLastError());
+  return WN_OK;
+}
+
 __global__ __launch_bounds__(256) void wn_sgemm_small32_kernel(const float* A, int64_t sai, int64_t sak, const float* B, int64_t sbk,
                                                                int64_t sbj, float* C, int ldc, int M, int N, int K,
                                                                int64_t za, int64_t zb, int64_t zc, const float* bias, int act,
@@ -601,8 +651,7 @@
 }
 
 __global__ void wn_guard_flag_kernel(const float* absmax, float limit, int enabled, float* out) {
-  const float m = absmax ? *absmax : 0.f;
-  out[0] = (enabled && !(m < limit)) ? 1.0f : 0.0f;
+  out[0] = wn_guard_flag(absmax, limit, enabled);
 }
 __global__ void wn_guard_accumulate_kernel(const float* src, float* dst) {
   const unsigned a = __float_as_uint(src[0]) & 0x7fffffffu, b = __float_as_uint(dst[0]) & 0x7fffffffu;
diff --git a/wavenets_amd/csrc/wn_forward.hip b/wavenets_amd/csrc/wn_forward.hip
--- a/wavenets_amd/csrc/wn_forward.hip
+++ b/wavenets_amd/csrc/wn_forward.hip
@@ -75,7 +75,8 @@
 }
 
 int forward_core(wn_plan* p, const float* params, const float* x, bool prep, const float* cond, int B,
-                 int T, bool training, float* ws, const WsLayout& L, hipStream_t s, const GenRings* rings, LossFuse* lf) {
+                 int T, bool training, float* ws, const WsLayout& L, hipStream_t s, const GenRings* rings, LossFuse* lf,
+                 const StepEntry* entry) {
   int rc = ensure_device_tables(p);
   if (rc) return rc;
   const int64_t rows = (int64_t)B * T;
@@ -155,9 +156,13 @@
     }
   }
   float* const fam = ws + L.fwd_absmax;
-  WN_HIP_CHECK(hipMemsetAsync(fam, 0, sizeof(float), s));
+  if (!(entry && entry->fam_cleared)) WN_HIP_CHECK(hipMemsetAsync(fam, 0, sizeof(float), s));
   {
-    if (p->R % 4 == 0 && wn_debug_get(1) != 1) {
+    if (entry && entry->x_full) {
+      if (!step_entry_fusable(p) || rings || x != entry->inputs) { wn_set_error("forward: step entry on a path without the elementwise input conv"); return WN_E_INVALID; }
+      rc = wn_launch_step_entry(entry->x_full, params + p->tensors[p->causal.kernel_t].off, params + p->tensors[p->causal.bias_t].off,
+                                B, T, p->R, p->KS, entry->bits, entry->inputs, entry->y_true, entry->target, ws + L.H[0], fam, s);
+    } else if (p->R % 4 == 0 && wn_debug_get(1) != 1) {
       rc = wn_launch_inconv_fwd(x, params + p->tensors[p->causal.kernel_t].off, params + p->tensors[p->causal.bias_t].off, B, T,
                                 p->R, p->KS, ws + L.H[0], fam, s);
     } else {
@@ -326,11 +331,16 @@
 }
 
 int loss_stage(wn_plan* p, int B, int T, int global_batch, bool want_grad, float* ws, const WsLayout& L,
-               float* loss_out, float* absmax_out, hipStream_t s, bool fused_done) {
+               float* loss_out, float* absmax_out, hipStream_t s, bool fused_done, const StepScalars* step) {
   const int64_t rows = (int64_t)B * T;
   const float gscale = 1.0f / (float)global_batch;
   int rc;
-  if (fused_done) return wn_launch_sum(ws + L.loss_rows, rows, gscale, loss_out, ws + L.sum_scratch, s);
+  auto sum_rows = [&]() {
+    if (step) return wn_launch_sum_step(ws + L.loss_rows, rows, gscale, loss_out, ws + L.sum_scratch, ws + L.fwd_absmax, step->limit,
+                                        step->enabled, s);
+    return wn_launch_sum(ws + L.loss_rows, rows, gscale, loss_out, ws + L.sum_scratch, s);
+  };
+  if (fused_done) return sum_rows();
   float* g_logits = want_grad ? ws + L.GF.back() : nullptr;
   if (p->c.head == WN_HEAD_CATEGORICAL) {
     rc = wn_launch_quantize(ws + L.yt, reinterpret_cast<int32_t*>(ws + L.target), rows, p->c.bits, s);
@@ -345,7 +355,7 @@
                             p->c.head == WN_HEAD_LOGISTIC ? 1 : 2, gscale, ws + L.loss_rows, g_logits, absmax_out, s);
   }
   if (rc) return rc;
-  return wn_launch_sum(ws + L.loss_rows, rows, gscale, loss_out, ws + L.sum_scratch, s);
+  return sum_rows();
 }
 
 }
diff --git a/wavenets_amd/csrc/wn_gemm.hip b/wavenets_amd/csrc/wn_gemm.hip
--- a/wavenets_amd/csrc/wn_gemm.hip
+++ b/wavenets_amd/csrc/wn_gemm.hip
@@ -585,8 +585,8 @@
 }
 
 struct WnBlkFirst { int v[257]; };
-__global__ __launch_bounds__(256) void wn_reduce_flat_kernel(const float* slab, int nsplit, int64_t P, float* out,
-                                                             const WnTensorDesc* table, WnBlkFirst bf, int n) {
+__global__ __launch_bounds__(256) void wn_reduce_flat_kernel(WnReduceSlabs sl, float* out, const WnTensorDesc* table,
+                                                             WnBlkFirst bf, int n) {
   int lo = 0, hi = n;
   while (hi - lo > 1) {
     const int mid = (lo + hi) >> 1;
@@ -595,6 +595,10 @@
   const WnTensorDesc d = table[lo];
   const int64_t i = (int64_t)((int)blockIdx.x - bf.v[lo]) * 256 + threadIdx.x;
   if (i >= d.len) return;
+  const int k = (lo >= sl.first[2]) ? 2 : (lo >= sl.first[1] ? 1 : 0);
+  const float* slab = sl.slab[k];
+  const int nsplit = sl.nsplit[k];
+  const int64_t P = sl.pitch[k];
   float acc = 0.f;
   const float* col = slab + d.off + i;
   int s = 0;
@@ -609,21 +613,29 @@
   out[d.off + i] = acc;
 }
 
+int wn_launch_reduce_slabs(const WnReduceSlabs& sl, float* out, const WnTensorDesc* d_table, int n, hipStream_t s,
+                           const WnTensorDesc* h_table) {
+  if (n <= 0) return WN_OK;
+  if (!h_table || n > 256) return WN_E_UNSUPPORTED;
+  WnBlkFirst bf;
+  int64_t nblk = 0;
+  for (int t = 0; t < n; ++t) { bf.v[t] = (int)nblk; nblk += (h_table[t].len + 255) / 256; }
+  for (int t = n; t <= 256; ++t) bf.v[t] = (int)nblk;
+  if (nblk <= 0) return WN_OK;
+  if (nblk >= (int64_t)1 << 30) return WN_E_UNSUPPORTED;
+  hipLaunchKernelGGL(wn_reduce_flat_kernel, dim3((unsigned)nblk), dim3(256), 0, s, sl, out, d_table, bf, n);
+  WN_HIP_CHECK(hipGetLastError());
+  return WN_OK;
+}
+
 int wn_launch_reduce_table(const float* slab, int nsplit, int64_t P, float* out, const WnTensorDesc* d_table,
                            int n, hipStream_t s, const WnTensorDesc* h_table) {
   if (n <= 0) return WN_OK;
-  if (h_table && n <= 256) {
-    WnBlkFirst bf;
-    int64_t nblk = 0;
-    for (int t = 0; t < n; ++t) { bf.v[t] = (int)nblk; nblk += (h_table[t].len + 255) / 256; }
-    for (int t = n; t <= 256; ++t) bf.v[t] = (int)nblk;
-    if (nblk <= 0) return WN_OK;
-    if (nblk < (int64_t)1 << 30) {
-      hipLaunchKernelGGL(wn_reduce_flat_kernel, dim3((unsigned)nblk), dim3(256), 0, s, slab, nsplit, P, out, d_table, bf, n);
-      WN_HIP_CHECK(hipGetLastError());
-      return WN_OK;
-    }
-  }
+  WnReduceSlabs sl;
+  sl.slab[0] = slab; sl.nsplit[0] = nsplit; sl.pitch[0] = P; sl.first[0] = 0;
+  for (int k = 1; k < 3; ++k) { sl.slab[k] = nullptr; sl.nsplit[k] = 0; sl.pitch[k] = 0; sl.first[k] = n; }
+  const int rc = wn_launch_reduce_slabs(sl, out, d_table, n, s, h_table);
+  if (rc != WN_E_UNSUPPORTED) return rc;
   hipLaunchKernelGGL(wn_reduce_table_kernel, dim3(64, n), dim3(256), 0, s, slab, nsplit, P, out, d_table);
   WN_HIP_CHECK(hipGetLastError());
   return WN_OK;
diff --git a/wavenets_amd/csrc/wn_kernels.h b/wavenets_amd/csrc/wn_kernels.h
--- a/wavenets_amd/csrc/wn_kernels.h
+++ b/wavenets_amd/csrc/wn_kernels.h
@@ -155,6 +155,9 @@
                             int splits_per_b, hipStream_t s, bool exact_fp32 = false);
 int wn_launch_reduce_table(const float* slab, int nsplit, int64_t P, float* out, const WnTensorDesc* d_table,
                            int n, hipStream_t s, const WnTensorDesc* h_table = nullptr);
+struct WnReduceSlabs { const float* slab[3]; int64_t pitch[3]; int32_t nsplit[3]; int32_t first[3]; };
+int wn_launch_reduce_slabs(const WnReduceSlabs& sl, float* out, const WnTensorDesc* d_table, int n, hipStream_t s,
+                           const WnTensorDesc* h_table);
 struct WnReduceArgs {
   const float* slab; int32_t nsplit; int32_t K; int32_t N;
   float* out; int32_t seg_len; int64_t seg_stride; int32_t accumulate;
@@ -303,6 +306,8 @@
                            int64_t P, int64_t w_off, int64_t b_off, hipStream_t s);
 int wn_launch_inconv_fwd(const float* x, const float* w, const float* bias, int B, int T, int R, int KS, float* y,
                          float* absmax_out, hipStream_t s);
+int wn_launch_step_entry(const float* x_full, const float* w, const float* bias, int B, int T, int R, int KS, int bits,
+                         float* inputs, float* y_true, int32_t* target, float* y, float* absmax_out, hipStream_t s);
 int wn_launch_guard_flag(const float* absmax, float limit, int enabled, float* out, hipStream_t s);
 int wn_launch_guard_accumulate(const float* src, float* dst, hipStream_t s);
 int wn_launch_batch_reduce(const float* slab, int B, int splits, int N, float* out, hipStream_t s);
@@ -322,6 +327,8 @@
 int wn_launch_mix_loss(const float* pred, const float* y, int64_t rows, int M, int bits, int kind,
                        float gscale, float* loss_rows, float* g_pred, float* absmax_out, hipStream_t s);
 int wn_launch_sum(const float* v, int64_t n, float scale, float* out, float* scratch, hipStream_t s);
+int wn_launch_sum_step(const float* v, int64_t n, float scale, float* out3, float* scratch, const float* absmax, float limit,
+                       int enabled, hipStream_t s);
 int wn_launch_sqdiff_sum(const float* a, const float* b, int64_t n, float scale, float* out, float* scratch, hipStream_t s);
 
 int wn_launch_sample_det(const float* pred, int64_t rows, int C, int M, int bits, float* out, hipStream_t s,
diff --git a/wavenets_amd/csrc/wn_layer16.hip b/wavenets_amd/csrc/wn_layer16.hip
--- a/wavenets_amd/csrc/wn_layer16.hip
+++ b/wavenets_amd/csrc/wn_layer16.hip
@@ -59,15 +59,6 @@
   const int lane = tid & 63, wave = __builtin_amdgcn_readfirstlane(tid >> 6);
   const int tl = lane & 31, h = lane >> 5;
 
-  {
-    float* sb = reinterpret_cast<float*>(smem + G::WD_BYTES + G::WR_BYTES + G::WAVES * G::STAGE_BYTES);
-    static_assert(2 * D + R <= 512, "one bias element per thread");
-    const float bval = tid < 2 * D ? a.bias_d[tid] : (tid < 2 * D + R ? a.bias_r[tid - 2 * D] : 0.f);
-    wn_images_to_lds<512, G::WD_BYTES / 16, G::WR_BYTES / 16>(a.frag_d, smem, G::WD_BYTES / 16, a.frag_r, smem + G::WD_BYTES,
-                                                               G::WR_BYTES / 16, tid);
-    if (tid < 2 * D + R) sb[tid] = bval;
-  }
-  __syncthreads();
   const float* lbias_d = reinterpret_cast<const float*>(smem + G::WD_BYTES + G::WR_BYTES + G::WAVES * G::STAGE_BYTES);
   const float* lbias_r = lbias_d + 2 * D;
   const h8* wd = reinterpret_cast<const h8*>(smem) + lane;
@@ -114,11 +105,28 @@
 
   constexpr bool ROT = FAST >= 2;
   Tile cur, nxt;
+  if constexpr (ROT) {
+    cur = tile_at(walk.first < ntiles ? walk.first : ntiles - 1);
+    wn_static_for<KS>([&](auto tapc) { request_tap(cur, tapc); });
+    request_cb(cur);
+    __builtin_amdgcn_sched_barrier(0);
+  }
+
+  {
+    float* sb = reinterpret_cast<float*>(smem + G::WD_BYTES + G::WR_BYTES + G::WAVES * G::STAGE_BYTES);
+    static_assert(2 * D + R <= 512, "one bias element per thread");
+    const float bval = tid < 2 * D ? a.bias_d[tid] : (tid < 2 * D + R ? a.bias_r[tid - 2 * D] : 0.f);
+    wn_images_to_lds<512, G::WD_BYTES / 16, G::WR_BYTES / 16>(a.frag_d, smem, G::WD_BYTES / 16, a.frag_r, smem + G::WD_BYTES,
+                                                               G::WR_BYTES / 16, tid);
+    if (tid < 2 * D + R) sb[tid] = bval;
+  }
+  __syncthreads();
+
   auto do_tile = [&](int64_t tile, auto nextc, auto firstc) __attribute__((always_inline)) {
     constexpr bool has_next = ROT && decltype(nextc)::value;
     constexpr bool first = !ROT || decltype(firstc)::value;
     asm volatile("; tile body %0" ::"n"(2 * (int)has_next + (int)first) : "memory");
-    if constexpr (first) {
+    if constexpr (!ROT) {
       cur = tile_at(tile);
       wn_static_for<KS>([&](auto tapc) { request_tap(cur, tapc); });
       request_cb(cur);
diff --git a/wavenets_amd/csrc/wn_loss.hip b/wavenets_amd/csrc/wn_loss.hip
--- a/wavenets_amd/csrc/wn_loss.hip
+++ b/wavenets_amd/csrc/wn_loss.hip
@@ -208,7 +208,7 @@
   }
   if (threadIdx.x == 0) scratch[blockIdx.x] = sm[0];
 }
-__global__ void wn_sum_stage2(const double* scratch, int nb, float scale, float* out) {
+__device__ __forceinline__ double wn_sum_partials(const double* scratch, int nb) {
   __shared__ double sm[256];
   double acc = 0.0;
   for (int i = threadIdx.x; i < nb; i += blockDim.x) acc += scratch[i];
@@ -218,12 +218,34 @@
     if (threadIdx.x < o) sm[threadIdx.x] += sm[threadIdx.x + o];
     __syncthreads();
   }
-  if (threadIdx.x == 0) out[0] = (float)(sm[0] * (double)scale);
+  return sm[0];
+}
+__global__ void wn_sum_stage2(const double* scratch, int nb, float scale, float* out) {
+  const double total = wn_sum_partials(scratch, nb);
+  if (threadIdx.x == 0) out[0] = (float)(total * (double)scale);
+}
+__global__ void wn_sum_stage2_step_kernel(const double* scratch, int nb, float scale, float* out, const float* absmax,
+                                          float limit, int enabled) {
+  const double total = wn_sum_partials(scratch, nb);
+  if (threadIdx.x == 0) {
+    out[0] = (float)(total * (double)scale);
+    out[1] = 0.f;
+    out[2] = wn_guard_flag(absmax, limit, enabled);
+  }
 }
 int wn_launch_sum(const float* v, int64_t n, float scale, float* out, float* scratch, hipStream_t s) {
   int nb = wn_blocks(n, 256, 1024);
   hipLaunchKernelGGL(wn_sum_stage1, dim3(nb), dim3(256), 0, s, v, n, reinterpret_cast<double*>(scratch));
   hipLaunchKernelGGL(wn_sum_stage2, dim3(1), dim3(256), 0, s, reinterpret_cast<const double*>(scratch), nb, scale, out);
+  WN_HIP_CHECK(hipGetLastError());
+  return WN_OK;
+}
+int wn_launch_sum_step(const float* v, int64_t n, float scale, float* out3, float* scratch, const float* absmax, float limit,
+                       int enabled, hipStream_t s) {
+  int nb = wn_blocks(n, 256, 1024);
+  hipLaunchKernelGGL(wn_sum_stage1, dim3(nb), dim3(256), 0, s, v, n, reinterpret_cast<double*>(scratch));
+  hipLaunchKernelGGL(wn_sum_stage2_step_kernel, dim3(1), dim3(256), 0, s, reinterpret_cast<const double*>(scratch), nb, scale, out3,
+                     absmax, limit, enabled);
   WN_HIP_CHECK(hipGetLastError());
   return WN_OK;
 }
diff --git a/wavenets_amd/csrc/wn_plan_internal.h b/wavenets_amd/csrc/wn_plan_internal.h
--- a/wavenets_amd/csrc/wn_plan_internal.h
+++ b/wavenets_amd/csrc/wn_plan_internal.h
@@ -358,12 +358,18 @@
 bool loss_fusable(const wn_plan* p, int64_t rows);
 BlockPtrs block_ptrs(const wn_plan* p, int b, const float* params, const float* fragbase, int B, int T);
 void deep16_ptrs(const wn_plan* p, int b, const float* fragbase, BlockPtrs& k);
+struct StepEntry {
+  bool fam_cleared;
+  const float* x_full; float* inputs; float* y_true; int32_t* target; int bits;
+};
+inline bool step_entry_fusable(const wn_plan* p) { return p->R % 4 == 0 && wn_debug_get(1) != 1; }
 int forward_core(wn_plan* p, const float* params, const float* x, bool prep, const float* cond, int B,
                  int T, bool training, float* ws, const WsLayout& L, hipStream_t s, const GenRings* rings = nullptr,
-                 LossFuse* lf = nullptr);
+                 LossFuse* lf = nullptr, const StepEntry* entry = nullptr);
 int shift_split(const float* x_full, int B, int T, float* inputs, float* y_true, hipStream_t s);
+struct StepScalars { float limit; int enabled; };
 int loss_stage(wn_plan* p, int B, int T, int global_batch, bool want_grad, float* ws, const WsLayout& L,
-               float* loss_out, float* absmax_out, hipStream_t s, bool fused_done = false);
+               float* loss_out, float* absmax_out, hipStream_t s, bool fused_done = false, const StepScalars* step = nullptr);
 
 }
 
diff --git a/wavenets_amd/csrc/wn_train.hip b/wavenets_amd/csrc/wn_train.hip
--- a/wavenets_amd/csrc/wn_train.hip
+++ b/wavenets_amd/csrc/wn_train.hip
@@ -216,15 +216,26 @@
 
   int forward_and_loss() {
     int rc;
-    { const int rcs = shift_split(x_full, B, T, inputs, ws + L.yt, s); if (rcs) return rcs; }
-    if (e.phase_on) (void)hipEventRecord(e.phase_ev[0], s);
-    WN_HIP_CHECK(hipMemsetAsync(am, 0, L.n_absmax * sizeof(float), s));
     LossFuse lf;
     memset(&lf, 0, sizeof(lf));
     const bool fuse = !pred_out && loss_fusable(p, rows);
+    StepEntry entry;
+    memset(&entry, 0, sizeof(entry));
+    if (step_entry_fusable(p)) {
+      entry.x_full = x_full; entry.inputs = inputs; entry.y_true = ws + L.yt; entry.bits = p->c.bits;
+      entry.target = fuse ? reinterpret_cast<int32_t*>(ws + L.target) : nullptr;
+    } else {
+      const int rcs = shift_split(x_full, B, T, inputs, ws + L.yt, s);
+      if (rcs) return rcs;
+    }
+    if (e.phase_on) (void)hipEventRecord(e.phase_ev[0], s);
+    entry.fam_cleared = L.fwd_absmax >= L.absmax + L.n_absmax && L.fwd_absmax - L.absmax <= (int64_t)L.n_absmax + 64;
+    WN_HIP_CHECK(hipMemsetAsync(am, 0, (entry.fam_cleared ? (size_t)(L.fwd_absmax + 64 - L.absmax) : (size_t)L.n_absmax) * sizeof(float), s));
     if (fuse) {
-      rc = wn_launch_quantize(ws + L.yt, reinterpret_cast<int32_t*>(ws + L.target), rows, p->c.bits, s);
-      if (rc) return rc;
+      if (!entry.x_full) {
+        rc = wn_launch_quantize(ws + L.yt, reinterpret_cast<int32_t*>(ws + L.target), rows, p->c.bits, s);
+        if (rc) return rc;
+      }
       lf.target = reinterpret_cast<const int32_t*>(ws + L.target);
       lf.gscale = 1.0f / (float)global_batch;
       lf.loss_rows = ws + L.loss_rows; lf.g_logits = ws + L.GF.back(); lf.absmax_out = am_GF(nf - 1);
@@ -233,11 +244,13 @@
         lf.seed = e.step_sample_seed; lf.offset = e.step_sample_off;
       }
     }
-    rc = forward_core(p, params, inputs, true, cond, B, T, true, ws, L, s, nullptr, fuse ? &lf : nullptr);
+    rc = forward_core(p, params, inputs, true, cond, B, T, true, ws, L, s, nullptr, fuse ? &lf : nullptr, &entry);
     if (rc) return rc;
     if (lf.done && lf.sample_out) e.step_sample = nullptr;
     if (e.phase_on) (void)hipEventRecord(e.phase_ev[1], s);
-    rc = loss_stage(p, B, T, global_batch, true, ws, L, loss_out, am_GF(nf - 1), s, lf.done);
+    const StepScalars flag{WN_RANGE_LIMIT * (e.drop_rate > 0.f ? 1.f - e.drop_rate : 1.f), wn_debug_get(1) != 1};
+    const bool one_launch = !(p->c.l2_reg_factor > 0.f);
+    rc = loss_stage(p, B, T, global_batch, true, ws, L, loss_out, am_GF(nf - 1), s, lf.done, one_launch ? &flag : nullptr);
     if (rc) return rc;
     if (pred_out) {
       if (p->c.head == WN_HEAD_CATEGORICAL) rc = wn_launch_softmax(ws + L.logits, pred_out, rows, p->Cout, s);
@@ -259,19 +272,15 @@
       }
       if (rc) return rc;
     }
-    if (p->c.l2_reg_factor > 0.f) {
+    if (!one_launch) {
       float* norms = ws + L.loss_rows;
       rc = wn_launch_sumsq(params, p->d_kdesc, (int)p->kdesc.size(), norms, s);
       if (rc) return rc;
       rc = wn_launch_sum(norms, (int64_t)p->kdesc.size(), p->c.l2_reg_factor / (float)n_replicas, loss_out + 1, ws + L.sum_scratch, s);
       if (rc) return rc;
-    } else {
-      rc = wn_launch_fill(loss_out + 1, 0.f, 1, s);
-      if (rc) return rc;
-    }
-    rc = wn_launch_guard_flag(ws + L.fwd_absmax, WN_RANGE_LIMIT * (e.drop_rate > 0.f ? 1.f - e.drop_rate : 1.f),
-                              wn_debug_get(1) != 1, loss_out + 2, s);
-    if (rc) return rc;
+      rc = wn_launch_guard_flag(ws + L.fwd_absmax, flag.limit, flag.enabled, loss_out + 2, s);
+      if (rc) return rc;
+    }
     if (e.phase_on) (void)hipEventRecord(e.phase_ev[2], s);
     return WN_OK;
   }
@@ -496,13 +505,25 @@
     if (fork) { WN_HIP_CHECK(hipStreamWaitEvent(s, e.ev_join, 0)); side_join.armed = false; }
     if (cond_batched && (rc = cond_weight_gradients())) return rc;
     const int cov0 = tp.in_split ? 2 : 0, ncov = (int)g.h_cov.size(), cov1 = g.cov_head;
-    rc = wn_launch_reduce_table(ws + L.bslab, B * L.bsplits, p->nparams, grads, g.cov.d + cov0, cov1 - cov0, s, g.h_cov.data() + cov0);
-    if (rc) return rc;
-    if (tp.in_split && (rc = wn_launch_reduce_table(ws + L.islab, B * L.isplits, (int64_t)(p->KS + 1) * p->R, grads, g.cov.d, 2, s, g.h_cov.data())))
-      return rc;
-    if (cov1 < ncov && (rc = wn_launch_reduce_table(ws + L.hslab - L.head_base, B * L.hsplits, L.head_span, grads, g.cov.d + cov1, ncov - cov1,
-                                                    s, g.h_cov.data() + cov1)))
-      return rc;
+    WnReduceSlabs sl;
+    int nsl = 0;
+    auto slab_of = [&](const float* base, int nsplit, int64_t pitch, int first) {
+      sl.slab[nsl] = base; sl.nsplit[nsl] = nsplit; sl.pitch[nsl] = pitch; sl.first[nsl] = first; ++nsl;
+    };
+    if (tp.in_split) slab_of(ws + L.islab, B * L.isplits, (int64_t)(p->KS + 1) * p->R, 0);
+    slab_of(ws + L.bslab, B * L.bsplits, p->nparams, cov0);
+    if (cov1 < ncov) slab_of(ws + L.hslab - L.head_base, B * L.hsplits, L.head_span, cov1);
+    while (nsl < 3) slab_of(nullptr, 0, 0, ncov);
+    rc = wn_launch_reduce_slabs(sl, grads, g.cov.d, ncov, s, g.h_cov.data());
+    if (rc == WN_E_UNSUPPORTED) {
+      rc = wn_launch_reduce_table(ws + L.bslab, B * L.bsplits, p->nparams, grads, g.cov.d + cov0, cov1 - cov0, s, g.h_cov.data() + cov0);
+      if (rc) return rc;
+      if (tp.in_split && (rc = wn_launch_reduce_table(ws + L.islab, B * L.isplits, (int64_t)(p->KS + 1) * p->R, grads, g.cov.d, 2, s, g.h_cov.data())))
+        return rc;
+      if (cov1 < ncov) rc = wn_launch_reduce_table(ws + L.hslab - L.head_base, B * L.hsplits, L.head_span, grads, g.cov.d + cov1, ncov - cov1,
+                                                   s, g.h_cov.data() + cov1);
+    }
+    if (rc) return rc;
     if (!p->c.use_skip && p->S > 0) {
       for (const BlockInfo& bi : p->blocks) {
         rc = wn_launch_fill(grads + p->tensors[bi.conv_skip.kernel_t].off, 0.f, p->tensors[bi.conv_skip.kernel_t].len, s);
```

After: 22.07 million. -3.2%, worse.
